# AvalonEnjoyer/pytorch-ViT-paper-replication

Hardware: AMD Instinct MI355X
Metric: images/sec (whole node) ViT-B/16 224px bf16 at 1/2/4/8 MI355X (higher is better)
Workload: dtype bf16; 1 GPU; model=ViT-B/16, global_batch=256, per_gpu_batch=256, seq_len=197, image_size=224, parallelism=dp1, impl=fused, grad_transport=none, optimizer=Adam(wd=0.03 decay group) + clip 1.0 + warmup/linear-decay LR, dropout=0.1 (mlp, embedding)

## Files before the change

### pytorch_vit_paper_replication_amd/_ext.py

```python
from __future__ import annotations

import contextlib
import os

import torch

_C = None
_ERR: BaseException | None = None
_TRIED = False


class StaleExtensionError(RuntimeError):
    """The in-tree ``_C`` was built from other ``csrc/`` sources than the ones in the tree."""


def check_source_hash(so, csrc) -> str:
    from .build import embedded_hash, source_hash

    want = source_hash(csrc)
    have = embedded_hash(so)
    if have != want:
        raise StaleExtensionError(
            f"{so} was built from other sources (binary {have}, csrc/ {want}): rebuild with "
            "`python -m pytorch_vit_paper_replication_amd.build` (or set PVR_AUTOBUILD=1)")
    return want


def load():
    global _C, _ERR, _TRIED
    if _TRIED:
        return _C
    _TRIED = True
    debug = os.environ.get("PVR_DEBUG_KERNELS", "0") == "1"
    try:
        from .build import CSRC, ext_path

        if CSRC.is_dir() and ext_path(debug).exists():
            try:
                check_source_hash(ext_path(debug), CSRC)
            except StaleExtensionError:
                if os.environ.get("PVR_AUTOBUILD", "0") != "1":
                    raise
                from .build import build_extension

                build_extension(debug=debug)
                check_source_hash(ext_path(debug), CSRC)
        if debug:
            from . import _C_debug as mod
        else:
            from . import _C as mod

        _C = mod
    except BaseException as e:
        _ERR = e
        if os.environ.get("PVR_AUTOBUILD", "0") == "1":
            try:
                from .build import build_extension

                build_extension(debug=debug)
                if debug:
                    from . import _C_debug as mod2
                else:
                    from . import _C as mod2

                _C = mod2
                _ERR = None
            except BaseException as e2:
                _ERR = e2
    return _C


def available() -> bool:
    return load() is not None


_DETERMINISTIC_ENV = os.environ.get("PVR_DETERMINISTIC", "0") not in ("", "0")


def deterministic() -> bool:
    m = _C if _TRIED else load()
    on = torch.are_deterministic_algorithms_enabled() or _DETERMINISTIC_ENV
    if m is not None and bool(m.deterministic()) != on:
        m.set_deterministic(on)
    return on


@contextlib.contextmanager
def deterministic_mode(on: bool = True):
    global _DETERMINISTIC_ENV
    old = _DETERMINISTIC_ENV
    _DETERMINISTIC_ENV = on
    try:
        deterministic()
        yield
    finally:
        _DETERMINISTIC_ENV = old
        deterministic()


def ext():
    m = load()
    if m is None:
        raise RuntimeError(
            "pytorch_vit_paper_replication_amd: the gfx950 extension _C is not built or failed to load "
            f"({_ERR!r}). Build it with `python -m pytorch_vit_paper_replication_amd.build`."
        )
    return m


def fallback_allowed() -> bool:
    return os.environ.get("PVR_ALLOW_TORCH_FALLBACK", "0") == "1"


_FORCE_REFERENCE = 0


def fused_disabled() -> bool:
    return _FORCE_REFERENCE > 0 or os.environ.get("PVR_DISABLE_FUSED", "0") == "1"


@contextlib.contextmanager
def reference_path():
    global _FORCE_REFERENCE
    _FORCE_REFERENCE += 1
    try:
        yield
    finally:
        _FORCE_REFERENCE -= 1


def use_fused(t: torch.Tensor) -> bool:
    if not t.is_cuda:
        return False
    if fused_disabled():
        return False
    if available():
        return True
    if fallback_allowed():
        return False
    ext()
    return False


def free_scratch() -> None:
    m = _C if _TRIED else load()
    if m is None:
        return
    if torch.cuda.is_available():
        torch.cuda.synchronize()
    m.free_scratch()
    from .ops import gemm as _gemm

    _gemm._workspaces.clear()
```

### pytorch_vit_paper_replication_amd/csrc/bindings.cpp

```cpp
#include <cstdlib>
#include <algorithm>
#include <map>
#include <torch/extension.h>
#include <c10/hip/HIPStream.h>
#include <hip/hip_runtime.h>

#include "kernels.h"

namespace {

hipStream_t stream() { return c10::hip::getCurrentHIPStream().stream(); }
using ScratchKey = std::pair<int, int64_t>;
ScratchKey scratch_key(int dev) { return std::make_pair(dev, (int64_t)c10::hip::getCurrentHIPStream().id()); }
template <class T>
std::map<ScratchKey, T>& scratch_map() {
  static auto* m = new std::map<ScratchKey, T>();
  return *m;
}
struct SkCounters { torch::Tensor t; };
struct DetWs { torch::Tensor t; };
struct DqWs { torch::Tensor t; };
struct AttnWs { torch::Tensor t; };

int num_cus() {
  static std::map<int, int> cache;
  int dev = 0;
  if (hipGetDevice(&dev) != hipSuccess) return 256;
  auto it = cache.find(dev);
  if (it != cache.end()) return it->second;
  hipDeviceProp_t prop;
  int n = hipGetDeviceProperties(&prop, dev) == hipSuccess && prop.multiProcessorCount > 0 ? prop.multiProcessorCount : 256;
  cache[dev] = n;
  return n;
}

void check(hipError_t e, const char* what) {
  TORCH_CHECK(e == hipSuccess, "pvr kernel '", what, "' failed: ", hipGetErrorString(e));
}

const uint16_t* bf(const torch::Tensor& t, const char* name) {
  TORCH_CHECK(t.is_cuda(), name, " must be a GPU tensor");
  TORCH_CHECK(t.scalar_type() == torch::kBFloat16, name, " must be bfloat16, got ", t.scalar_type());
  return reinterpret_cast<const uint16_t*>(t.data_ptr());
}
uint16_t* bf_mut(torch::Tensor& t, const char* name) { return const_cast<uint16_t*>(bf(t, name)); }
const float* f32(const torch::Tensor& t, const char* name) {
  TORCH_CHECK(t.is_cuda(), name, " must be a GPU tensor");
  TORCH_CHECK(t.scalar_type() == torch::kFloat32, name, " must be float32, got ", t.scalar_type());
  return t.data_ptr<float>();
}
float* f32_mut(torch::Tensor& t, const char* name) { return const_cast<float*>(f32(t, name)); }

template <class T>
T* opt_ptr(const c10::optional<torch::Tensor>& t) {
  return t.has_value() && t->defined() ? reinterpret_cast<T*>(t->data_ptr()) : nullptr;
}

int64_t ld_of(const torch::Tensor& t, const char* name) {
  TORCH_CHECK(t.dim() == 2, name, " must be 2-D");
  TORCH_CHECK(t.stride(1) == 1, name, " must have unit stride in its last dim");
  TORCH_CHECK(t.stride(0) % 8 == 0 || t.size(0) == 1, name, " leading dimension must be a multiple of 8 elements");
  TORCH_CHECK(reinterpret_cast<uintptr_t>(t.data_ptr()) % 16 == 0, name, " must be 16-byte aligned");
  return t.size(0) == 1 ? t.size(1) : t.stride(0);
}

pvr::DropSite drop_args(const c10::optional<torch::Tensor>& seed, int64_t seed_offset, double drop_p, const char* what) {
  pvr::DropSite d;
  d.offset = (uint64_t)seed_offset;
  if (drop_p > 0.0) {
    TORCH_CHECK(seed.has_value() && seed->defined() && seed->is_cuda() && seed->scalar_type() == torch::kInt64 && seed->numel() >= 1,
                what, ": dropout needs an int64 seed tensor on the GPU");
    d.seed = reinterpret_cast<const uint64_t*>(seed->data_ptr());
    d.thr = (uint32_t)llround(drop_p * 65536.0);
    if (d.thr > 65535) d.thr = 65535;
    d.scale = (float)(65536.0 / (65536.0 - d.thr));
  }
  return d;
}
pvr::DropSite drop_path_args(const c10::optional<torch::Tensor>& seed, int64_t seed_offset, double dp_p, int64_t dp_rows,
                             const char* what) {
  TORCH_CHECK(dp_p >= 0.0 && dp_p <= 1.0, what, ": drop_path rate must be in [0, 1]");
  if (dp_p > 0.0) TORCH_CHECK(dp_rows >= 1 && dp_rows < (int64_t(1) << 31), what, ": drop_path needs rows per sample >= 1");
  return drop_args(seed, seed_offset, dp_p, what);
}
void set_drop(pvr::GemmParams& p, const pvr::DropSite& d) {
  if (!d.seed) return;
  p.seed_ptr = d.seed; p.seed_offset = d.offset; p.drop_thr = d.thr; p.drop_scale = d.scale;
}

pvr::Fp8Copy fp8_copy(const c10::optional<torch::Tensor>& q_out, const c10::optional<torch::Tensor>& q_scale,
                      const c10::optional<torch::Tensor>& q_amax, int64_t q_fmt, int64_t rows, int64_t cols, int64_t align,
                      const char* what) {
  pvr::Fp8Copy q;
  q.fmt = (int)q_fmt;
  if (!q_out.has_value() || !q_out->defined()) return q;
  TORCH_CHECK(q_out->is_cuda() && q_out->scalar_type() == torch::kUInt8 && q_out->dim() == 2 && q_out->stride(1) == 1 &&
                  q_out->size(0) >= rows && q_out->size(1) >= cols && q_out->stride(0) % align == 0 &&
                  reinterpret_cast<uintptr_t>(q_out->data_ptr()) % align == 0,
              what, ": q_out must be uint8 [>= ", rows, "][>= ", cols, "] with unit column stride, row stride and base multiples of ", align);
  TORCH_CHECK(q_scale.has_value() && q_scale->defined() && q_amax.has_value() && q_amax->defined() && q_amax->is_cuda() &&
                  q_amax->scalar_type() == torch::kInt32 && (q_fmt == 0 || q_fmt == 1),
              what, ": q_out needs q_scale (f32), q_amax (int32 on the GPU) and q_fmt 0 / 1");
  q.out = q_out->data_ptr<uint8_t>();
  q.ld = q_out->stride(0);
  q.scale = f32(*q_scale, "q_scale");
  q.amax = reinterpret_cast<unsigned*>(q_amax->data_ptr());
  return q;
}

bool g_gemm_tail = true;
struct TailBufs {
  torch::Tensor ws, cnt;
};
void attach_tail(pvr::GemmParams& p, const torch::Tensor& like) {
  if (!g_gemm_tail) return;
  auto& bufs = scratch_map<TailBufs>();
  const auto key = scratch_key((int)like.get_device());
  auto it = bufs.find(key);
  if (it == bufs.end()) {
    const int64_t cus = num_cus();
    TailBufs b;
    b.ws = torch::empty({cus * 65536}, like.options().dtype(torch::kFloat32));
    b.cnt = torch::zeros({cus}, like.options().dtype(torch::kInt32));
    it = bufs.emplace(key, b).first;
  }
  p.tail_ws = it->second.ws.data_ptr<float>();
  p.tail_cnt = reinterpret_cast<unsigned*>(it->second.cnt.data_ptr<int32_t>());
  p.tail_ws_elems = it->second.ws.numel();
  p.tail_cnt_elems = (int)it->second.cnt.numel();
}
void set_gemm_tail(bool on) { g_gemm_tail = on; }

constexpr int g_sk_tiles = 4096;
torch::Tensor& splitk_counters(const torch::Tensor& like) {
  auto& bufs = scratch_map<SkCounters>();
  const auto key = scratch_key((int)like.get_device());
  auto it = bufs.find(key);
  if (it == bufs.end()) it = bufs.emplace(key, SkCounters{torch::zeros({2 * g_sk_tiles + 4}, like.options().dtype(torch::kInt32))}).first;
  return it->second.t;
}
int64_t splitk_timeouts(torch::Tensor like, bool reset) {
  torch::Tensor& c = splitk_counters(like);
  const int64_t v = c[2 * g_sk_tiles].item<int32_t>();
  if (reset) c[2 * g_sk_tiles].zero_();
  return v;
}
constexpr int g_tail_min_kt = 12;

bool g_deterministic = [] {
  const char* e = std::getenv("PVR_DETERMINISTIC");
  return e && std::atoi(e) != 0;
}();
void set_deterministic(bool on) { g_deterministic = on; }
bool deterministic() { return g_deterministic; }
float* det_scratch(int64_t numel, const torch::TensorOptions& opts) {
  DetWs& d = scratch_map<DetWs>()[scratch_key((int)opts.device().index())];
  if (!d.t.defined() || d.t.numel() < numel) d.t = torch::empty({numel}, opts.dtype(torch::kFloat32));
  return d.t.data_ptr<float>();
}

void gemm(torch::Tensor A, bool a_kcontig, torch::Tensor B, bool b_kcontig, torch::Tensor C, int64_t M, int64_t N, int64_t K,
          int64_t epi, c10::optional<torch::Tensor> bias, c10::optional<torch::Tensor> resid, c10::optional<torch::Tensor> addend,
          int64_t addend_period, c10::optional<torch::Tensor> aux, int64_t row_group, int64_t row_stride_group,
          int64_t row_offset, c10::optional<torch::Tensor> seed, int64_t seed_offset, double drop_p, int64_t k_split,
          int64_t tile_cfg, c10::optional<torch::Tensor> dbg, c10::optional<torch::Tensor> colsum,
          int64_t epi_staged, int64_t tail_limit, c10::optional<torch::Tensor> reduce_out, bool reduce_acc,
          int64_t drop_row_mul, c10::optional<torch::Tensor> dp_seed, int64_t dp_offset, double dp_p, int64_t dp_rows) {
  pvr::GemmParams p{};
  TORCH_CHECK(drop_row_mul >= 0 && (drop_row_mul == 0 || (tile_cfg == 0 && row_group == 0)) && M * std::max<int64_t>(drop_row_mul, 1) < (int64_t(1) << 31),
              "gemm: drop_row_mul (mask of every drop_row_mul-th row of a larger tensor) needs tile 0 and no row remap");
  p.drop_row_mul = (int)drop_row_mul;
  p.epi_staged = (int)epi_staged;
  if (colsum.has_value() && colsum->defined()) p.colsum = f32_mut(*colsum, "colsum");
  if (dbg.has_value() && dbg->defined()) p.dbg = reinterpret_cast<uint64_t*>(dbg->data_ptr());
  p.drop_scale = 1.f;
  p.M = (int)M; p.N = (int)N; p.K = (int)K;
  p.A = bf(A, "A"); p.lda = ld_of(A, "A"); p.a_kcontig = a_kcontig;
  p.B = bf(B, "B"); p.ldb = ld_of(B, "B"); p.b_kcontig = b_kcontig;
  TORCH_CHECK(N % 8 == 0, "gemm: N must be a multiple of 8");
  if (a_kcontig) TORCH_CHECK(K % 64 == 0, "gemm: K must be a multiple of 64 for a k-contiguous A");
  if (b_kcontig) TORCH_CHECK(K % 64 == 0, "gemm: K must be a multiple of 64 for a k-contiguous B");
  if (a_kcontig) {
    TORCH_CHECK(A.size(0) >= M && A.size(1) >= K, "gemm: A too small");
  } else {
    TORCH_CHECK(A.size(0) >= K && A.size(1) >= M, "gemm: A too small");
  }
  if (b_kcontig) {
    TORCH_CHECK(B.size(0) >= N && B.size(1) >= K, "gemm: B too small");
  } else {
    TORCH_CHECK(B.size(0) >= K && B.size(1) >= N, "gemm: B too small");
  }
  const bool f32out = epi >= 3;
  TORCH_CHECK(C.is_cuda() && C.scalar_type() == (f32out ? torch::kFloat32 : torch::kBFloat16), "gemm: C dtype mismatch for epilogue");
  if (C.dim() == 3) {
    TORCH_CHECK(epi == 4 && tile_cfg == 14, "gemm: a 3-D C is the split-K workspace of EPI_F32_STORE / tile 14");
    TORCH_CHECK(C.stride(2) == 1 && C.size(1) >= M && C.size(2) >= N, "gemm: workspace shape");
    const int64_t ks = k_split > 0 ? ((k_split + 63) / 64) * 64 : ((K + 63) / 64) * 64;
    TORCH_CHECK(C.size(0) >= (K + ks - 1) / ks, "gemm: workspace has fewer slices than K splits");
    p.C = C.data_ptr(); p.ldc = C.stride(1); p.split_stride = C.stride(0);
  } else {
    p.C = C.data_ptr(); p.ldc = ld_of(C, "C");
  }
  if (bias.has_value() && bias->defined()) { TORCH_CHECK(bias->numel() >= N && bias->is_contiguous(), "bias"); p.bias = f32(*bias, "bias"); }
  if (resid.has_value() && resid->defined()) { p.resid = bf(*resid, "resid"); p.ld_resid = ld_of(*resid, "resid"); }
  if (addend.has_value() && addend->defined()) { p.addend = f32(*addend, "addend"); p.addend_period = (int)addend_period; TORCH_CHECK(addend_period > 0, "addend_period"); }
  if (aux.has_value() && aux->defined()) { p.aux = const_cast<uint16_t*>(bf(*aux, "aux")); p.ld_aux = ld_of(*aux, "aux"); }
  if (epi == 2) TORCH_CHECK(p.aux != nullptr, "gemm: the dGELU epilogue needs aux");
  p.row_group = (int)row_group; p.row_stride_group = (int)row_stride_group; p.row_offset = (int)row_offset;
  set_drop(p, drop_args(seed, seed_offset, drop_p, "gemm"));
  p.k_split_len = k_split > 0 ? (int)(((k_split + 63) / 64) * 64) : (int)(((K + 63) / 64) * 64);
  if (dp_p > 0.0) {
    const pvr::DropSite dp = drop_path_args(dp_seed, dp_offset, dp_p, dp_rows, "gemm: drop_path");
    TORCH_CHECK(epi == 0 && p.resid != nullptr, "gemm: drop_path needs the residual epilogue (EPI_BF16 with resid)");
    TORCH_CHECK(a_kcontig && b_kcontig && row_group == 0 && p.addend == nullptr && p.k_split_len >= K,
                "gemm: drop_path does not combine with row_group / addend / split-K / transposed operands");
    TORCH_CHECK(tile_cfg == 0 || tile_cfg == 6 || tile_cfg == 12 || tile_cfg == 13,
                "gemm: drop_path runs on tiles 0, 6, 12 and 13 (not the wave-specialised tile 15 or the split-K tile 14)");
    TORCH_CHECK(p.seed_ptr == nullptr || p.seed_ptr == dp.seed, "gemm: drop_path and dropout must share the seed tensor");
    TORCH_CHECK(M / dp_rows + 1 < (int64_t(1) << 31), "gemm: drop_path sample index");
    p.seed_ptr = dp.seed;
    p.dp_thr = dp.thr; p.dp_scale = dp.scale; p.dp_seed_offset = dp.offset; p.dp_rows = (int)dp_rows;
  }
  p.epi = (int)epi;
  p.tile_cfg = (int)tile_cfg;
  if (epi <= 2 && p.k_split_len >= K && tail_limit >= 0) {
    attach_tail(p, C);
    p.tail_max_units = (int)tail_limit;
    p.tail_min_kt = g_tail_min_kt;
  }
  if (reduce_out.has_value() && reduce_out->defined()) {
    const torch::Tensor& o = *reduce_out;
    TORCH_CHECK(C.dim() == 3 && epi == 4 && tile_cfg == 14, "gemm: reduce_out needs the split-K workspace form");
    TORCH_CHECK(o.is_cuda() && o.scalar_type() == torch::kFloat32 && o.dim() == 2 && o.stride(1) == 1 && o.size(0) >= M && o.size(1) >= N &&
                    o.stride(0) % 4 == 0 && reinterpret_cast<uintptr_t>(o.data_ptr()) % 16 == 0,
                "gemm: reduce_out must be a 16-B aligned fp32 [M, N] tensor with unit column stride");
    const int64_t splits = (K + p.k_split_len - 1) / p.k_split_len;
    const int64_t tiles = ((M + 255) / 256) * ((N + 255) / 256);
    TORCH_CHECK(N % 4 == 0 && tiles <= g_sk_tiles && tiles * splits <= num_cus(), "gemm: reduce_out: too many workgroups to be co-resident");
    TORCH_CHECK(p.split_stride * 4 * (2 * splits + 16) < (int64_t(1) << 32) && M * p.ldc * 4 < (int64_t(1) << 31),
                "gemm: reduce_out: workspace too large for 32-bit buffer offsets");
    torch::Tensor& cnt = splitk_counters(o);
    p.sk_out = o.data_ptr<float>();
    p.sk_ldo = o.stride(0);
    p.sk_acc = reduce_acc ? 1 : 0;
    p.sk_cnt = reinterpret_cast<unsigned*>(cnt.data_ptr<int32_t>());
    p.sk_cnt_tiles = g_sk_tiles;
  }
  check(pvr_gemm(&p, stream()), "gemm");
}

std::vector<torch::Tensor> layernorm_fwd(torch::Tensor x, torch::Tensor w, torch::Tensor b, double eps, int64_t rows,
                                         int64_t x_row_stride) {
  const int64_t D = w.numel();
  auto y = torch::empty({rows, D}, x.options());
  auto mean = torch::empty({rows}, x.options().dtype(torch::kFloat32));
  auto rstd = torch::empty({rows}, x.options().dtype(torch::kFloat32));
  TORCH_CHECK(x.stride(-1) == 1, "layernorm: x last dim must be contiguous");
  check(pvr_layernorm_fwd(bf(x, "x"), x_row_stride, f32(w, "w"), f32(b, "b"), bf_mut(y, "y"), D, f32_mut(mean, "mean"),
                          f32_mut(rstd, "rstd"), (int)rows, (int)D, (float)eps, stream()),
        "layernorm_fwd");
  return {y, mean, rstd};
}

std::vector<torch::Tensor> layernorm_fwd_q8(torch::Tensor x, torch::Tensor w, torch::Tensor b, double eps, int64_t rows,
                                            int64_t x_row_stride, torch::Tensor q_out, torch::Tensor q_scale, torch::Tensor q_amax,
                                            bool skip_y) {
  const int64_t D = w.numel();
  auto y = torch::empty({rows, D}, x.options());
  auto mean = torch::empty({rows}, x.options().dtype(torch::kFloat32));
  auto rstd = torch::empty({rows}, x.options().dtype(torch::kFloat32));
  TORCH_CHECK(x.stride(-1) == 1, "layernorm: x last dim must be contiguous");
  TORCH_CHECK(q_out.defined(), "layernorm_fwd_q8: q_out is required");
  const pvr::Fp8Copy q = fp8_copy(q_out, q_scale, q_amax, 0, rows, D, 8, "layernorm_fwd_q8");
  check(pvr_layernorm_fwd_q8(bf(x, "x"), x_row_stride, f32(w, "w"), f32(b, "b"), skip_y ? nullptr : bf_mut(y, "y"), D, q,
                             f32_mut(mean, "mean"), f32_mut(rstd, "rstd"), (int)rows, (int)D, (float)eps, stream()),
        "layernorm_fwd_q8");
  return {y, mean, rstd};
}

void layernorm_bwd(torch::Tensor dy, int64_t dy_stride, torch::Tensor x, int64_t x_stride, torch::Tensor mean, torch::Tensor rstd,
                   torch::Tensor w, c10::optional<torch::Tensor> dres, int64_t dres_stride, torch::Tensor dx, int64_t dx_stride,
                   c10::optional<torch::Tensor> dw, c10::optional<torch::Tensor> db, int64_t rows,
                   c10::optional<torch::Tensor> dsum, c10::optional<torch::Tensor> dz, c10::optional<torch::Tensor> seed,
                   int64_t seed_offset, double drop_p, c10::optional<torch::Tensor> q_out,
                   c10::optional<torch::Tensor> q_scale, c10::optional<torch::Tensor> q_amax, bool dz_nostore,
                   int64_t q_fmt, int64_t dres_every, c10::optional<torch::Tensor> dp_seed, int64_t dp_offset, double dp_p,
                   int64_t dp_rows) {
  const int64_t D = w.numel();
  pvr::LnBwdParams p{};
  TORCH_CHECK(dres_every >= 0, "layernorm_bwd: dres_every >= 0");
  if (dres_every > 1) {
    TORCH_CHECK(dres.has_value() && dres->defined() && dres->numel() >= ((rows + dres_every - 1) / dres_every - 1) * dres_stride + D &&
                    !(q_out.has_value() && q_out->defined()),
                "layernorm_bwd: dres_every needs a compact dres [ceil(rows / dres_every)][D] and no fp8 copy");
  }
  p.dres_every = (int)dres_every;
  p.dy = bf(dy, "dy"); p.dy_stride = dy_stride;
  p.x = bf(x, "x"); p.x_stride = x_stride;
  p.mean = f32(mean, "mean"); p.rstd = f32(rstd, "rstd"); p.w = f32(w, "w");
  p.dres = opt_ptr<const uint16_t>(dres); p.dres_stride = dres_stride;
  p.dx = bf_mut(dx, "dx"); p.dx_stride = dx_stride;
  p.dw = opt_ptr<float>(dw); p.db = opt_ptr<float>(db); p.dsum = opt_ptr<float>(dsum);
  const bool has_dz = dz.has_value() && dz->defined();
  if (has_dz) {
    TORCH_CHECK(drop_p > 0.0 || dp_p > 0.0, "layernorm_bwd: dz is the dropout / drop_path backward, it needs drop_p > 0 or a drop_path rate > 0");
    p.dz = const_cast<uint16_t*>(bf(*dz, "dz"));
    p.dz_stride = ld_of(*dz, "dz");
  }
  p.drop = drop_args(seed, seed_offset, has_dz ? drop_p : 0.0, "layernorm_bwd");
  if (dp_p > 0.0) {
    TORCH_CHECK(has_dz, "layernorm_bwd: drop_path scales the dz output, it needs dz");
    TORCH_CHECK(!(q_out.has_value() && q_out->defined()), "layernorm_bwd: drop_path does not combine with the fp8 copy (q_out)");
    p.dpath = drop_path_args(dp_seed, dp_offset, dp_p, dp_rows, "layernorm_bwd: drop_path");
    p.dp_rows = (int)dp_rows;
  }
  p.dz_nostore = dz_nostore ? 1 : 0;
  p.q = fp8_copy(q_out, q_scale, q_amax, q_fmt, rows, D, 8, "layernorm_bwd");
  p.rows = (int)rows; p.D = (int)D;
  if (g_deterministic && (p.dw || p.db || p.dsum))
    p.part = det_scratch((int64_t)pvr_layernorm_bwd_blocks((int)rows, (int)D) * 3 * D, x.options());
  check(pvr_layernorm_bwd(&p, stream()), "layernorm_bwd");
}

void splitk_reduce(torch::Tensor ws, int64_t S, torch::Tensor out, bool accumulate) {
  TORCH_CHECK(ws.dim() == 3 && ws.size(0) >= S && S >= 1, "splitk_reduce: ws must be [S, rows, cols]");
  TORCH_CHECK(out.is_contiguous() && ws.stride(2) == 1 && ws.stride(1) == ws.size(2), "splitk_reduce: layouts");
  const int64_t rows = ws.size(1), wcols = ws.size(2);
  TORCH_CHECK(out.numel() % rows == 0, "splitk_reduce: out must hold [rows, ocols]");
  const int64_t ocols = out.numel() / rows;
  TORCH_CHECK(ocols <= wcols && ocols % 4 == 0 && wcols % 4 == 0, "splitk_reduce: out columns must be a 4-aligned prefix of ws columns");
  check(pvr_splitk_reduce(f32(ws, "ws"), (int)S, ws.stride(0), f32_mut(out, "out"), out.numel(), (int)ocols, (int)wcols,
                          accumulate ? 1 : 0, stream()),
        "splitk_reduce");
}

void pad_cols_bf16(torch::Tensor src, torch::Tensor dst) {
  TORCH_CHECK(src.is_contiguous() && dst.is_contiguous() && src.dim() == 2 && dst.dim() == 2 && src.size(0) == dst.size(0) &&
                  src.size(1) <= dst.size(1) && src.size(1) % 4 == 0 && dst.size(1) % 4 == 0,
              "pad_cols_bf16: src [rows, cols], dst [rows, ld >= cols], contiguous, 4-aligned");
  check(pvr_pad_cols_bf16(bf(src, "src"), (int)src.size(0), (int)src.size(1), bf_mut(dst, "dst"), (int)dst.size(1), stream()),
        "pad_cols_bf16");
}

void splitk_epilogue(torch::Tensor ws, int64_t S, torch::Tensor out, c10::optional<torch::Tensor> bias,
                     c10::optional<torch::Tensor> resid, bool gelu) {
  TORCH_CHECK(ws.dim() == 3 && ws.size(0) >= S && S >= 1 && ws.stride(2) == 1 && ws.stride(1) == ws.size(2),
              "splitk_epilogue: ws must be [S, M, N] with contiguous rows");
  const int64_t M = ws.size(1), N = ws.size(2);
  TORCH_CHECK(out.dim() == 2 && out.size(0) == M && out.size(1) == N && N % 4 == 0, "splitk_epilogue: out shape");
  const int64_t ldc = ld_of(out, "out");
  const float* bp = nullptr;
  if (bias.has_value() && bias->defined()) {
    TORCH_CHECK(bias->numel() >= N && bias->is_contiguous(), "splitk_epilogue: bias");
    bp = f32(*bias, "bias");
  }
  const uint16_t* rp = nullptr;
  int64_t ldr = 0;
  if (resid.has_value() && resid->defined()) {
    TORCH_CHECK(resid->dim() == 2 && resid->size(0) >= M && resid->size(1) >= N, "splitk_epilogue: resid must cover [M, N]");
    rp = bf(*resid, "resid");
    ldr = ld_of(*resid, "resid");
  }
  check(pvr_splitk_epilogue(f32(ws, "ws"), (int)S, ws.stride(0), (int)M, (int)N, bp, rp, ldr, gelu ? 1 : 0, bf_mut(out, "out"), ldc,
                            stream()),
        "splitk_epilogue");
}

void cast_f32_bf16(torch::Tensor in, torch::Tensor out) {
  TORCH_CHECK(in.is_contiguous() && out.is_contiguous() && in.numel() == out.numel(), "cast: shape/contiguity");
  TORCH_CHECK(in.device() == out.device() && reinterpret_cast<uintptr_t>(in.data_ptr()) % 16 == 0 &&
                  reinterpret_cast<uintptr_t>(out.data_ptr()) % 8 == 0,
              "cast: in (16-byte aligned) and out (8-byte aligned) on one GPU");
  check(pvr_cast_f32_bf16(f32(in, "in"), bf_mut(out, "out"), in.numel(), stream()), "cast_f32_bf16");
}

void transpose_batched(torch::Tensor src, torch::Tensor dst, torch::Tensor meta, int64_t total_tiles) {
  TORCH_CHECK(meta.scalar_type() == torch::kInt64 && meta.is_cuda() && meta.dim() == 2 && meta.size(1) == 5, "meta");
  check(pvr_transpose_batched(bf(src, "src"), bf_mut(dst, "dst"), meta.data_ptr<int64_t>(), (int)meta.size(0), (int)total_tiles,
                              stream()),
        "transpose_batched");
}

void colsum(torch::Tensor dy, int64_t rows, int64_t N, c10::optional<torch::Tensor> db, c10::optional<torch::Tensor> dz,
            c10::optional<torch::Tensor> seed, int64_t seed_offset, double drop_p, c10::optional<torch::Tensor> q_out,
            c10::optional<torch::Tensor> q_scale, c10::optional<torch::Tensor> q_amax, int64_t q_fmt, int64_t row_mul,
            c10::optional<torch::Tensor> dp_seed, int64_t dp_offset, double dp_p, int64_t dp_rows) {
  TORCH_CHECK(row_mul >= 1 && rows * row_mul < (int64_t(1) << 31), "colsum: row_mul >= 1 and rows * row_mul < 2^31");
  const pvr::DropSite d = drop_args(seed, seed_offset, drop_p, "colsum");
  pvr::DropSite dp;
  if (dp_p > 0.0) {
    TORCH_CHECK(!(q_out.has_value() && q_out->defined()), "colsum: drop_path does not combine with the fp8 copy (q_out)");
    dp = drop_path_args(dp_seed, dp_offset, dp_p, dp_rows, "colsum: drop_path");
  }
  int64_t ldz = 0;
  uint16_t* dzp = nullptr;
  if (dz.has_value() && dz->defined()) { dzp = const_cast<uint16_t*>(bf(*dz, "dz")); ldz = ld_of(*dz, "dz"); }
  const pvr::Fp8Copy q = fp8_copy(q_out, q_scale, q_amax, q_fmt, rows, N, 8, "colsum");
  check(pvr_colsum(bf(dy, "dy"), ld_of(dy, "dy"), (int)rows, (int)N, opt_ptr<float>(db), dzp, ldz, d, q,
                   g_deterministic && opt_ptr<float>(db) ? det_scratch((int64_t)pvr_colsum_part_rows((int)rows) * N, dy.options()) : nullptr,
                   (int)row_mul, dp, (int)std::max<int64_t>(dp_rows, 1), stream()),
        "colsum");
}

torch::Tensor drop_path_scale(torch::Tensor seed, int64_t site_offset, double p, int64_t B) {
  TORCH_CHECK(B >= 0 && B < (int64_t(1) << 31), "drop_path_scale: B");
  auto out = torch::ones({B}, seed.options().dtype(torch::kFloat32));
  if (p <= 0.0 || B == 0) return out;
  const pvr::DropSite dp = drop_path_args(seed, site_offset, p, 1, "drop_path_scale");
  check(pvr_drop_path_scale(dp, out.data_ptr<float>(), (int)B, stream()), "drop_path_scale");
  return out;
}

const pvr::MixRow* mix_rows(const c10::optional<torch::Tensor>& mix, const c10::optional<torch::Tensor>& host, int64_t B, int64_t H,
                            int64_t W, const torch::Tensor& img, const char* what) {
  if (!mix.has_value() || !mix->defined()) {
    TORCH_CHECK(!host.has_value() || !host->defined(), what, ": mix_host without mix");
    return nullptr;
  }
  TORCH_CHECK(mix->is_cuda() && mix->device() == img.device(), what, ": mix must be on the image's device");
  TORCH_CHECK(mix->scalar_type() == torch::kInt32 && mix->dim() == 2 && mix->size(0) == B && mix->size(1) == 8 && mix->is_contiguous(),
              what, ": mix must be contiguous int32 [", B, ", 8]");
  TORCH_CHECK(reinterpret_cast<uintptr_t>(mix->data_ptr()) % 16 == 0, what, ": mix must be 16-byte aligned");
  torch::Tensor h;
  if (host.has_value() && host->defined()) {
    TORCH_CHECK(!host->is_cuda() && host->scalar_type() == torch::kInt32 && host->dim() == 2 && host->size(0) == B &&
                    host->size(1) == 8 && host->is_contiguous(),
                what, ": mix_host must be a contiguous CPU int32 [", B, ", 8] tensor");
    h = *host;
  } else {
    h = mix->cpu();
  }
  const auto* rows = reinterpret_cast<const pvr::MixRow*>(h.data_ptr());
  for (int64_t b = 0; b < B; ++b) {
    const pvr::MixRow& r = rows[b];
// ... 676 lines not shown
}

void fp8_transpose(torch::Tensor x8, torch::Tensor yt) {
  TORCH_CHECK(x8.is_cuda() && x8.scalar_type() == torch::kUInt8 && x8.dim() == 2 && x8.stride(1) == 1 && x8.stride(0) % 16 == 0 &&
                  x8.size(1) % 16 == 0 && reinterpret_cast<uintptr_t>(x8.data_ptr()) % 16 == 0,
              "fp8_transpose: x8 uint8 [rows][cols], cols and row stride multiples of 16, 16-byte aligned");
  TORCH_CHECK(yt.is_cuda() && yt.scalar_type() == torch::kUInt8 && yt.dim() == 2 && yt.size(0) == x8.size(1) &&
                  yt.size(1) >= x8.size(0) && yt.stride(1) == 1 && yt.stride(0) % 64 == 0 && yt.size(1) == yt.stride(0) &&
                  reinterpret_cast<uintptr_t>(yt.data_ptr()) % 16 == 0,
              "fp8_transpose: yT uint8 [cols][>= rows], row stride a multiple of 64");
  check(pvr_fp8_transpose(x8.data_ptr<uint8_t>(), x8.stride(0), yt.data_ptr<uint8_t>(), yt.stride(0), (int)x8.size(0), (int)x8.size(1),
                          stream()),
        "fp8_transpose");
}

void gemm_fp8_wgrad_mn(torch::Tensor dy8, torch::Tensor x8, torch::Tensor ws, int64_t N, int64_t K, int64_t T, torch::Tensor scale_a,
                       torch::Tensor scale_b, int64_t ksplit, int64_t fmt_a) {
  TORCH_CHECK((fmt_a == 0 || fmt_a == 1), "gemm_fp8_wgrad_mn: fmt_a 0 (e4m3) / 1 (e5m2)");
  TORCH_CHECK(dy8.dim() == 2 && x8.dim() == 2 && dy8.size(0) >= T && x8.size(0) >= T && dy8.size(1) >= N && x8.size(1) >= K &&
                  dy8.stride(1) == 1 && x8.stride(1) == 1,
              "gemm_fp8_wgrad_mn: dy8 [T][N], x8 [T][K] row-major");
  TORCH_CHECK(N % 16 == 0 && K % 16 == 0 && dy8.stride(0) % 16 == 0 && x8.stride(0) % 16 == 0 && ksplit % 128 == 0 &&
                  reinterpret_cast<uintptr_t>(dy8.data_ptr()) % 16 == 0 && reinterpret_cast<uintptr_t>(x8.data_ptr()) % 16 == 0,
              "gemm_fp8_wgrad_mn: 16-byte rows and bases, ksplit a multiple of 128");
  TORCH_CHECK(T * std::max(dy8.stride(0), x8.stride(0)) < (1ll << 31), "gemm_fp8_wgrad_mn: 31-bit operand offsets");
  TORCH_CHECK(ws.is_cuda() && ws.scalar_type() == torch::kFloat32 && ws.dim() == 3 && ws.stride(2) == 1 && ws.size(1) >= N &&
                  ws.size(2) >= K && ws.size(0) >= (T + ksplit - 1) / ksplit,
              "gemm_fp8_wgrad_mn: workspace [splits][N][K] f32");
  pvr::GemmParams p{};
  p.drop_scale = 1.f;
  p.M = (int)N; p.N = (int)K; p.K = (int)T;
  p.A = reinterpret_cast<const uint16_t*>(u8(dy8, "dy8")); p.lda = dy8.stride(0); p.a_kcontig = 0;
  p.B = reinterpret_cast<const uint16_t*>(u8(x8, "x8")); p.ldb = x8.stride(0); p.b_kcontig = 0;
  p.C = ws.data_ptr(); p.ldc = ws.stride(1); p.split_stride = ws.stride(0);
  p.scale_a = f32(scale_a, "scale_a"); p.scale_b = f32(scale_b, "scale_b");
  p.elem8 = 1; p.fmt_a = (int)fmt_a; p.fmt_b = 0;
  p.k_split_len = (int)ksplit;
  p.epi = 4;
  p.tile_cfg = 14;
  check(pvr_gemm(&p, stream()), "gemm_fp8_wgrad_mn");
}

void gemm_fp8_wgrad(torch::Tensor A8, torch::Tensor B8, torch::Tensor ws, int64_t N, int64_t K, int64_t Tp, torch::Tensor scale_a,
                    torch::Tensor scale_b, int64_t ksplit, int64_t fmt_a) {
  TORCH_CHECK((fmt_a == 0 || fmt_a == 1), "gemm_fp8_wgrad: fmt_a 0 (e4m3) / 1 (e5m2)");
  pvr::GemmParams p{};
  p.drop_scale = 1.f;
  p.M = (int)N; p.N = (int)K; p.K = (int)Tp;
  p.A = reinterpret_cast<const uint16_t*>(u8(A8, "A8")); p.lda = A8.stride(0); p.a_kcontig = 1;
  p.B = reinterpret_cast<const uint16_t*>(u8(B8, "B8")); p.ldb = B8.stride(0); p.b_kcontig = 1;
  TORCH_CHECK(A8.size(0) >= N && A8.size(1) >= Tp && B8.size(0) >= K && B8.size(1) >= Tp, "gemm_fp8_wgrad: operand too small");
  TORCH_CHECK(Tp % 128 == 0 && ksplit % 128 == 0 && K % 8 == 0, "gemm_fp8_wgrad: Tp, ksplit multiples of 128");
  TORCH_CHECK(ws.is_cuda() && ws.scalar_type() == torch::kFloat32 && ws.dim() == 3 && ws.stride(2) == 1 && ws.size(1) >= N &&
                  ws.size(2) >= K && ws.size(0) >= (Tp + ksplit - 1) / ksplit,
              "gemm_fp8_wgrad: workspace [splits][N][K] f32");
  p.C = ws.data_ptr(); p.ldc = ws.stride(1); p.split_stride = ws.stride(0);
  p.scale_a = f32(scale_a, "scale_a"); p.scale_b = f32(scale_b, "scale_b");
  p.elem8 = 1; p.fmt_a = (int)fmt_a; p.fmt_b = 0;
  p.k_split_len = (int)ksplit;
  p.epi = 4;
  p.tile_cfg = 14;
  check(pvr_gemm(&p, stream()), "gemm_fp8_wgrad");
}

void fp8_quant(torch::Tensor x, c10::optional<torch::Tensor> y, c10::optional<torch::Tensor> qscale, torch::Tensor amax, int64_t fmt) {
  const uint16_t* xp = bf(x, "x");
  const int64_t ldx = ld_of(x, "x");
  uint8_t* yp = nullptr;
  int64_t ldy = 0;
  if (y.has_value() && y->defined()) {
    yp = const_cast<uint8_t*>(u8(*y, "y"));
    ldy = y->stride(0);
    TORCH_CHECK(y->size(0) == x.size(0) && y->size(1) == x.size(1), "fp8_quant: shape mismatch");
  }
  TORCH_CHECK(amax.is_cuda() && amax.scalar_type() == torch::kInt32 && amax.numel() >= 1, "fp8_quant: amax int32");
  const float* qs = nullptr;
  if (qscale.has_value() && qscale->defined()) qs = f32(*qscale, "qscale");
  TORCH_CHECK(yp == nullptr || qs != nullptr, "fp8_quant: y needs qscale");
  check(pvr_fp8_quant(xp, ldx, yp, ldy, x.size(0), (int)x.size(1), qs, reinterpret_cast<unsigned*>(amax.data_ptr()), (int)fmt, stream()),
        "fp8_quant");
}

torch::Tensor fp8_dequant(torch::Tensor x, c10::optional<torch::Tensor> dscale, int64_t fmt) {
  TORCH_CHECK(x.is_cuda() && x.scalar_type() == torch::kUInt8 && x.is_contiguous(), "fp8_dequant: contiguous uint8");
  auto y = torch::empty(x.sizes(), x.options().dtype(torch::kFloat32));
  const float* ds = nullptr;
  if (dscale.has_value() && dscale->defined()) ds = f32(*dscale, "dscale");
  check(pvr_fp8_dequant(x.data_ptr<uint8_t>(), y.data_ptr<float>(), x.numel(), ds, (int)fmt, stream()), "fp8_dequant");
  return y;
}

void fp8_quant_multi(torch::Tensor segs, int64_t nchunks, c10::optional<torch::Tensor> qscale, torch::Tensor amax, int64_t fmt,
                     bool amax_only) {
  TORCH_CHECK(segs.is_cuda() && segs.scalar_type() == torch::kInt64 && segs.dim() == 2 && segs.size(1) == 5 && segs.is_contiguous(),
              "fp8_quant_multi: segs int64 [n][5]");
  TORCH_CHECK(amax.is_cuda() && amax.scalar_type() == torch::kInt32, "fp8_quant_multi: amax int32");
  const float* qs = qscale.has_value() && qscale->defined() ? f32(*qscale, "qscale") : nullptr;
  TORCH_CHECK(amax_only || qs != nullptr, "fp8_quant_multi: quantizing needs qscale");
  check(pvr_fp8_quant_multi(segs.data_ptr<int64_t>(), (int)segs.size(0), nchunks, qs, reinterpret_cast<unsigned*>(amax.data_ptr()),
                            (int)fmt, amax_only ? 1 : 0, stream()),
        "fp8_quant_multi");
}

void fp8_scale_update(torch::Tensor hist, torch::Tensor amax, torch::Tensor qscale, torch::Tensor dscale, torch::Tensor fmax, int64_t s0,
                      int64_t s1, double margin_mul) {
  TORCH_CHECK(hist.dim() == 2 && hist.is_contiguous(), "hist [n][H]");
  TORCH_CHECK(amax.scalar_type() == torch::kInt32, "amax int32");
  TORCH_CHECK(s0 >= 0 && s1 <= hist.size(0), "slot range");
  check(pvr_fp8_scale_update(f32_mut(hist, "hist"), (int)hist.size(1), reinterpret_cast<unsigned*>(amax.data_ptr()), f32_mut(qscale, "qscale"),
                             f32_mut(dscale, "dscale"), f32(fmax, "fmax"), (int)s0, (int)s1, (float)margin_mul, stream()),
        "fp8_scale_update");
}

std::vector<torch::Tensor> attn_fwd(torch::Tensor qkv, int64_t B, int64_t N, int64_t H, double scale, c10::optional<torch::Tensor> seed,
                                    int64_t seed_offset, double drop_p, c10::optional<torch::Tensor> q_out,
                                    c10::optional<torch::Tensor> q_scale, c10::optional<torch::Tensor> q_amax, bool q_only) {
  const int64_t D = qkv.size(1) / 3;
  auto out = torch::empty({B * N, D}, qkv.options());
  auto lse = torch::empty({B * H, N}, qkv.options().dtype(torch::kFloat32));
  TORCH_CHECK(!q_only || (q_out.has_value() && q_out->defined()), "attn_fwd: q_only needs q_out");
  TORCH_CHECK(qkv.size(0) == B * N, "attn_fwd: qkv rows != B*N");
  const pvr::DropSite d = drop_args(seed, seed_offset, drop_p, "attn_fwd");
  const pvr::Fp8Copy q8 = fp8_copy(q_out, q_scale, q_amax, 0, B * N, D, 4, "attn_fwd");
  check(pvr_attn_fwd(bf(qkv, "qkv"), ld_of(qkv, "qkv"), bf_mut(out, "out"), D, f32_mut(lse, "lse"), (int)B, (int)N, (int)H, (int)D,
                     (float)scale, d, q8, q_only ? 1 : 0, stream()),
        "attn_fwd");
  return {out, lse};
}

void attn_dbias_reduce(torch::Tensor part, int64_t B, int64_t H, torch::Tensor dbias) {
  TORCH_CHECK(dbias.is_cuda() && dbias.scalar_type() == torch::kFloat32 && dbias.is_contiguous() && dbias.numel() % (3 * H) == 0,
              "attn_dbias_reduce: f32 [3D] bias gradient");
  const int64_t DH = dbias.numel() / (3 * H);
  TORCH_CHECK(part.is_cuda() && part.scalar_type() == torch::kFloat32 && part.is_contiguous() && part.numel() % (B * H * 3 * DH) == 0,
              "attn_dbias_reduce: f32 [B*H][R][3 * head dim] partials");
  const int64_t NQ = part.numel() / (B * H * 3 * DH);
  auto ws = torch::empty({(int64_t)pvr_attn_dbias_splits((int)B, (int)NQ) * H * 2 * DH}, part.options());
  check(pvr_attn_dbias_reduce(part.data_ptr<float>(), ws.data_ptr<float>(), dbias.data_ptr<float>(), (int)B, (int)H, (int)NQ,
                              (int)(DH * H), stream()),
        "attn_dbias_reduce");
}

torch::Tensor dq_workspace(int64_t numel, const torch::TensorOptions& opts, bool drop = false) {
  DqWs& d = scratch_map<DqWs>()[scratch_key((int)opts.device().index())];
  if (drop) {
    d.t = torch::Tensor();
    return torch::Tensor();
  }
  if (!d.t.defined() || d.t.numel() < numel) d.t = torch::zeros({numel}, opts.dtype(torch::kFloat32));
  return d.t;
}

torch::Tensor attn_scratch(int64_t numel, const torch::TensorOptions& opts) {
  AttnWs& d = scratch_map<AttnWs>()[scratch_key((int)opts.device().index())];
  if (!d.t.defined() || d.t.numel() < numel) d.t = torch::empty({numel}, opts.dtype(torch::kFloat32));
  return d.t;
}

void free_scratch() {
  scratch_map<TailBufs>().clear();
  scratch_map<SkCounters>().clear();
  scratch_map<DetWs>().clear();
  scratch_map<DqWs>().clear();
  scratch_map<AttnWs>().clear();
}

int64_t attn_bwd_bias_rows(int64_t B, int64_t N, int64_t H, int64_t D, bool drop) {
  return pvr_attn_bwd_part_rows((int)B, (int)N, (int)H, (int)D, 3 * D, D, D, 3 * D, drop ? 1 : 0);
}

bool attn_bwd_q8_ok(int64_t B, int64_t N, int64_t H, int64_t D, bool drop) {
  return pvr_attn_bwd_q8_ok((int)N, drop ? 1 : 0) && !pvr_attn_bwd_uses_pipe((int)B, (int)N, (int)H, (int)D, 3 * D, D, D, 3 * D, drop ? 1 : 0);
}

torch::Tensor attn_bwd(torch::Tensor dout, torch::Tensor qkv, torch::Tensor out, torch::Tensor lse, int64_t B, int64_t N, int64_t H,
                       double scale, c10::optional<torch::Tensor> dbias, c10::optional<torch::Tensor> dbias_part_out,
                       c10::optional<torch::Tensor> seed, int64_t seed_offset, double drop_p, c10::optional<torch::Tensor> q_out,
                       c10::optional<torch::Tensor> q_scale, c10::optional<torch::Tensor> q_amax, bool q_only,
                       int64_t q_fmt) {
  const int64_t D = qkv.size(1) / 3;
  auto dqkv = torch::empty_like(qkv);
  torch::Tensor dq_acc;
  int dq_rezero = 0;
  const pvr::DropSite drop = drop_args(seed, seed_offset, drop_p, "attn_bwd");
  const int has_drop = drop.seed ? 1 : 0;
  const int64_t dh = D / H;
  torch::Tensor dbias_part, old_part;
  const bool want_db = dbias.has_value() && dbias->defined();
  const int64_t lds[4] = {ld_of(qkv, "qkv"), ld_of(dout, "dout"), ld_of(out, "out"), ld_of(dqkv, "dqkv")};
  const int prow = pvr_attn_bwd_part_rows((int)B, (int)N, (int)H, (int)D, lds[0], lds[1], lds[2], lds[3], has_drop);
  const bool parts = prow > 0;
  const bool pipe = pvr_attn_bwd_uses_pipe((int)B, (int)N, (int)H, (int)D, lds[0], lds[1], lds[2], lds[3], has_drop) != 0;
  const bool part_out = dbias_part_out.has_value() && dbias_part_out->defined();
  if (part_out) {
    TORCH_CHECK(parts && !want_db, "dbias_part: shapes with attn_bwd_bias_rows > 0 only, and not together with dbias");
    TORCH_CHECK(dbias_part_out->is_cuda() && dbias_part_out->scalar_type() == torch::kFloat32 && dbias_part_out->is_contiguous() &&
                    dbias_part_out->numel() == B * H * prow * 3 * dh,
                "dbias_part [B*H][attn_bwd_bias_rows][3 * head dim] f32");
    dbias_part = *dbias_part_out;
  }
  if (want_db) {
    TORCH_CHECK(dbias->numel() == 3 * D && dbias->scalar_type() == torch::kFloat32 && dbias->is_contiguous(), "dbias [3D] f32");
    if (parts)
      dbias_part = torch::empty({B * H, (int64_t)prow, 3 * dh}, qkv.options().dtype(torch::kFloat32));
    else if (2 * (dh / 16) <= 2 * pvr_attn_bwd_waves((int)N))
      old_part = torch::empty({B * pvr_attn_bwd_key_blocks((int)N), 3 * D}, qkv.options().dtype(torch::kFloat32));
  }
  const int old_db = old_part.defined() ? 1 : 0;
  if (pvr_attn_bwd_needs_dq_acc((int)N, (int)dh, old_db, has_drop, g_deterministic ? 1 : 0)) {
    dq_acc = dq_workspace(B * N * D, qkv.options());
    dq_rezero = dq_acc.defined() ? 1 : 0;
    if (!dq_acc.defined()) dq_acc = torch::zeros({B * N, D}, qkv.options().dtype(torch::kFloat32));
  }
  const pvr::Fp8Copy q8 = fp8_copy(q_out, q_scale, q_amax, q_fmt, B * N, 3 * D, 4, "attn_bwd");
  if (q8.out)
    TORCH_CHECK(pvr_attn_bwd_q8_ok((int)N, has_drop) && !old_db && !pipe, "attn_bwd: no e5m2 dQKV copy for this shape (see attn_bwd_q8_ok)");
  auto ws = attn_scratch(pvr_attn_bwd_ws_floats((int)B, (int)N, (int)H, (int)D, old_db, has_drop, g_deterministic ? 1 : 0), qkv.options());
  pvr::AttnBwdParams p{};
  p.qkv = bf(qkv, "qkv"); p.ld = lds[0];
  p.out = bf(out, "out"); p.ld_o = lds[2];
  p.dout = bf(dout, "dout"); p.ld_do = lds[1];
  p.dqkv = bf_mut(dqkv, "dqkv"); p.ld_dq = lds[3];
  p.lse = f32(lse, "lse"); p.ws = ws.data_ptr<float>();
  p.dq_acc = dq_acc.defined() ? dq_acc.data_ptr<float>() : nullptr; p.dq_rezero = dq_rezero;
  p.dbias = pipe && dbias_part.defined() ? dbias_part.data_ptr<float>() : old_db ? old_part.data_ptr<float>() : nullptr;
  p.bpart = !pipe && dbias_part.defined() ? dbias_part.data_ptr<float>() : nullptr;
  p.B = (int)B; p.N = (int)N; p.H = (int)H; p.D = (int)D; p.scale = (float)scale;
  p.drop = drop; p.q8 = q8; p.q8_only = q_only && q8.out ? 1 : 0;
  const hipError_t err = pvr_attn_bwd(&p, stream());
  if (err != hipSuccess && dq_rezero) dq_workspace(0, qkv.options(), true);
  check(err, "attn_bwd");
  if (want_db) {
    if (parts)
      attn_dbias_reduce(dbias_part, B, H, *dbias);
    else if (old_db)
      dbias->add_(old_part.sum(0));
    else
      dbias->add_(dqkv.sum(0, false, torch::kFloat32));
  }
  return dqkv;
}

std::vector<torch::Tensor> attn_cls_fwd(torch::Tensor qkv, int64_t B, int64_t N, int64_t H, double scale) {
  TORCH_CHECK(qkv.dim() == 2 && qkv.size(0) == B * N && qkv.size(1) % 3 == 0 && H > 0, "attn_cls_fwd: qkv [B*N][3D]");
  const int64_t D = qkv.size(1) / 3;
  TORCH_CHECK(D % H == 0 && pvr_attn_cls_ok((int)N, (int)(D / H)), "attn_cls_fwd: unsupported N / head dim (attn_cls_ok)");
  auto out = torch::empty({B, D}, qkv.options());
  auto lse = torch::empty({B * H}, qkv.options().dtype(torch::kFloat32));
  check(pvr_attn_cls_fwd(bf(qkv, "qkv"), ld_of(qkv, "qkv"), bf_mut(out, "out"), D, f32_mut(lse, "lse"), (int)B, (int)N, (int)H, (int)D,
                         (float)scale, stream()),
        "attn_cls_fwd");
  return {out, lse};
}

std::vector<torch::Tensor> attn_cls_bwd(torch::Tensor dout, torch::Tensor qkv, torch::Tensor out, torch::Tensor lse, int64_t B, int64_t N,
                                        int64_t H, double scale) {
  TORCH_CHECK(qkv.dim() == 2 && qkv.size(0) == B * N && qkv.size(1) % 3 == 0 && H > 0, "attn_cls_bwd: qkv [B*N][3D]");
  const int64_t D = qkv.size(1) / 3;
  TORCH_CHECK(D % H == 0 && pvr_attn_cls_ok((int)N, (int)(D / H)), "attn_cls_bwd: unsupported N / head dim (attn_cls_ok)");
  TORCH_CHECK(dout.dim() == 2 && dout.size(0) == B && dout.size(1) == D && out.dim() == 2 && out.size(0) == B && out.size(1) == D &&
                  lse.numel() == B * H && lse.is_contiguous(),
              "attn_cls_bwd: dout / out [B][D], lse [B*H]");
  auto dqkv = torch::empty({B * N, 3 * D}, qkv.options());
  auto dq0 = torch::empty({B, D}, qkv.options().dtype(torch::kFloat32));
  check(pvr_attn_cls_bwd(bf(qkv, "qkv"), ld_of(qkv, "qkv"), bf(out, "out"), ld_of(out, "out"), bf(dout, "dout"), ld_of(dout, "dout"),
                         f32(lse, "lse"), bf_mut(dqkv, "dqkv"), 3 * D, f32_mut(dq0, "dq0"), (int)B, (int)N, (int)H, (int)D, (float)scale,
                         stream()),
        "attn_cls_bwd");
  return {dqkv, dq0};
}

void attn_cls_dbias(torch::Tensor dq0, torch::Tensor dout, torch::Tensor dbias) {
  TORCH_CHECK(dq0.dim() == 2 && dq0.is_contiguous() && dout.dim() == 2 && dout.size(0) == dq0.size(0) && dout.size(1) == dq0.size(1) &&
                  dbias.is_contiguous() && dbias.numel() == 3 * dq0.size(1),
              "attn_cls_dbias: dq0 f32 [B][D] contiguous, dout bf16 [B][D], dbias f32 [3D]");
  check(pvr_attn_cls_dbias(f32(dq0, "dq0"), bf(dout, "dout"), ld_of(dout, "dout"), f32_mut(dbias, "dbias"), (int)dq0.size(0),
                           (int)dq0.size(1), stream()),
        "attn_cls_dbias");
}

}

extern "C" const char* pvr_src_hash(void);

PYBIND11_MODULE(TORCH_EXTENSION_NAME, m) {
  m.doc() = "MI355X (gfx950) HIP kernels for pytorch_vit_paper_replication_amd";
  m.def("source_hash", []() { return std::string(pvr_src_hash()); },
        "content hash of the csrc/ sources this binary was built from (build.source_hash())");
  m.def("gemm_tail_split", [](int64_t M, int64_t N, int64_t K, int64_t elem_bytes, int64_t max_units) {
    return pvr_gemm_tail_split((int)M, (int)N, (int)K, (int)elem_bytes, (int)max_units); },
    py::arg("M"), py::arg("N"), py::arg("K"), py::arg("elem_bytes"), py::arg("max_units") = 0,
    "K-parts of the split tail round this GEMM shape gets (0: none)");
  m.def("set_attn_dbg", [](torch::Tensor t) { pvr_set_attn_dbg(t.defined() && t.numel() ? t.data_ptr() : nullptr); },
        "diagnostic builds (-DPVR_ATTN_STAMPS): int64 buffer for the attention backward's phase stamps "
        "[workgroup * waves + wave][8] (scripts/attn_stamps.py); a no-op otherwise");
  m.def("set_attn_prep_xcd", &pvr_set_attn_prep_xcd, "attention backward pre-pass: XCD-contiguous (batch, head) pairs (1) or round-robin (0, default); A/B");
  m.def("set_ln_fwd_q8_grid", &pvr_set_ln_fwd_q8_grid, "LayerNorm forward with the e4m3 copy: grid cap in workgroups per CU (A/B)");
  m.def("set_attn_fwd_head_qf", &pvr_set_attn_fwd_head_qf, "whole-head attention forward (dh 64, N <= 256): 16-query fragments per wave (1 = default, 2 = half the LDS reads with 7 waves; A/B)");
  m.def("set_attn_fwd_qg", &pvr_set_attn_fwd_qg, "tiled attention forward: 16-query groups per wave (0 = auto by query padding, 1 = round-3 form, 2 = forced; A/B)");
  m.def("set_fp8_persistent", &pvr_set_fp8_persistent, "fp8 fwd/dgrad GEMMs on the persistent ping-pong: 1 when the epilogue has no per-row input (default), 0 never (A/B)");
  m.def("set_deterministic", &set_deterministic, "deterministic reductions (partial rows + ordered sum) instead of float atomics");
  m.def("deterministic", &deterministic);
  m.def("set_gemm_tail", &set_gemm_tail, "split-K tail of the last dispatch round on (True, default) / off (A/B)");
  m.def("gemm", &gemm,py::arg("A"), py::arg("a_kcontig"), py::arg("B"), py::arg("b_kcontig"), py::arg("C"),
        py::arg("M"), py::arg("N"), py::arg("K"), py::arg("epi"), py::arg("bias"), py::arg("resid"), py::arg("addend"),
        py::arg("addend_period"), py::arg("aux"), py::arg("row_group"), py::arg("row_stride_group"),
        py::arg("row_offset"), py::arg("seed"), py::arg("seed_offset"), py::arg("drop_p"), py::arg("k_split"),
        py::arg("tile_cfg"), py::arg("dbg") = py::none(), py::arg("colsum") = py::none(),
        py::arg("epi_staged") = 0, py::arg("tail_limit") = 0, py::arg("reduce_out") = py::none(), py::arg("reduce_acc") = true,
        py::arg("drop_row_mul") = 0, py::arg("dp_seed") = py::none(), py::arg("dp_offset") = 0, py::arg("dp_p") = 0.0,
        py::arg("dp_rows") = 1);
  m.def("drop_path_scale", &drop_path_scale, py::arg("seed"), py::arg("site_offset"), py::arg("p"), py::arg("B"));
  m.def("splitk_timeouts", &splitk_timeouts, py::arg("like"), py::arg("reset") = false);
  m.def("num_cus", &num_cus);
  m.def("layernorm_fwd", &layernorm_fwd);
  m.def("free_scratch", &free_scratch);
  m.def("layernorm_fwd_q8", &layernorm_fwd_q8);
  m.def("layernorm_bwd", &layernorm_bwd, py::arg("dy"), py::arg("dy_stride"), py::arg("x"), py::arg("x_stride"),
        py::arg("mean"), py::arg("rstd"), py::arg("w"), py::arg("dres"), py::arg("dres_stride"), py::arg("dx"),
        py::arg("dx_stride"), py::arg("dw"), py::arg("db"), py::arg("rows"), py::arg("dsum") = py::none(),
        py::arg("dz") = py::none(), py::arg("seed") = py::none(), py::arg("seed_offset") = 0, py::arg("drop_p") = 0.0,
        py::arg("q_out") = py::none(), py::arg("q_scale") = py::none(), py::arg("q_amax") = py::none(),
        py::arg("dz_nostore") = false, py::arg("q_fmt") = 1, py::arg("dres_every") = 0, py::arg("dp_seed") = py::none(),
        py::arg("dp_offset") = 0, py::arg("dp_p") = 0.0, py::arg("dp_rows") = 1);
  m.def("cast_f32_bf16", &cast_f32_bf16);
  m.def("splitk_epilogue", &splitk_epilogue);
  m.def("attn_bwd_bias_rows", &attn_bwd_bias_rows, py::arg("B"), py::arg("N"), py::arg("H"), py::arg("D"), py::arg("drop") = false);
  m.def("attn_dbias_reduce", &attn_dbias_reduce);
  m.def("splitk_reduce", &splitk_reduce);
  m.def("pad_cols_bf16", &pad_cols_bf16);
  m.def("transpose_batched", &transpose_batched);
  m.def("colsum", &colsum, py::arg("dy"), py::arg("rows"), py::arg("N"), py::arg("db"), py::arg("dz"), py::arg("seed"),
        py::arg("seed_offset"), py::arg("drop_p"), py::arg("q_out") = py::none(), py::arg("q_scale") = py::none(),
        py::arg("q_amax") = py::none(), py::arg("q_fmt") = 1, py::arg("row_mul") = 1, py::arg("dp_seed") = py::none(),
        py::arg("dp_offset") = 0, py::arg("dp_p") = 0.0, py::arg("dp_rows") = 1);
  m.def("im2col", &im2col, py::arg("img"), py::arg("out"), py::arg("P"), py::arg("Kp"), py::arg("mix") = py::none(),
        py::arg("mix_host") = py::none(), py::arg("keep") = py::none(), py::arg("erase") = py::none(),
        py::arg("erase_host") = py::none(), py::arg("erase_mode") = "const", py::arg("erase_value") = std::vector<double>{0.0},
        py::arg("erase_seed") = py::none(), py::arg("erase_offset") = 0);
  m.def("im2col_u8", &im2col_u8, py::arg("img"), py::arg("out"), py::arg("mean"), py::arg("std"), py::arg("geom"), py::arg("H"),
        py::arg("W"), py::arg("P"), py::arg("Kp"), py::arg("mix") = py::none(), py::arg("mix_host") = py::none(),
        py::arg("keep") = py::none(), py::arg("erase") = py::none(), py::arg("erase_host") = py::none(),
        py::arg("erase_mode") = "const", py::arg("erase_value") = std::vector<double>{0.0}, py::arg("erase_seed") = py::none(),
        py::arg("erase_offset") = 0);
  m.def("color_u8", &color_u8, py::arg("img"), py::arg("plan"), py::arg("plan_host") = py::none());
  m.def("erase_noise", &erase_noise, py::arg("seed"), py::arg("site_offset"), py::arg("B"), py::arg("C"), py::arg("H"), py::arg("W"));
  m.def("patch_keep_table", &patch_keep_table, py::arg("seed"), py::arg("site_offset"), py::arg("B"), py::arg("n_p"), py::arg("n_keep"));
  m.def("pos_gather", &pos_gather, py::arg("pos"), py::arg("keep"));
  m.def("cls_rows", &cls_rows);
  m.def("patch_bwd", &patch_bwd, py::arg("dE"), py::arg("B"), py::arg("ntok"), py::arg("D"), py::arg("dpos"), py::arg("dcls"),
        py::arg("dconv"), py::arg("dbias"), py::arg("seed"), py::arg("seed_offset"), py::arg("drop_p"), py::arg("inv") = py::none(),
        py::arg("n_keep") = 0);
  m.def("xent", &xent, py::arg("logits"), py::arg("labels"), py::arg("dlogits"), py::arg("correct"), py::arg("grad_scale"),
        py::arg("mean") = py::none());
  m.def("xent_soft", &xent_soft, py::arg("logits"), py::arg("ya"), py::arg("yb"), py::arg("lam"), py::arg("eps"),
        py::arg("dlogits"), py::arg("correct"), py::arg("grad_scale"), py::arg("mean") = py::none());
  m.def("grad_norm", &grad_norm);
  m.def("norm_partial_blocks", []() { return pvr_norm_partial_blocks(); });
  m.def("adam", &adam, py::arg("p"), py::arg("g"), py::arg("m"), py::arg("v"), py::arg("shadow"), py::arg("seg_start"),
        py::arg("seg_group"), py::arg("groups"), py::arg("clip"), py::arg("skip_nonfinite"), py::arg("ema") = py::none(),
        py::arg("ema_pair") = py::none());
  m.def("adam_t", &adam_t, py::arg("p"), py::arg("g"), py::arg("m"), py::arg("v"), py::arg("shadow"), py::arg("shadow_t"),
        py::arg("tmeta"), py::arg("ntiles"), py::arg("fmeta"), py::arg("flat4"), py::arg("groups"), py::arg("clip"),
        py::arg("skip_nonfinite"), py::arg("ema") = py::none(), py::arg("ema_pair") = py::none());
  m.def("lamb_chunk", []() { return (int)pvr::LAMB_CHUNK; });
  m.def("lamb_moments", &lamb_moments, py::arg("p"), py::arg("g"), py::arg("m"), py::arg("v"), py::arg("chunks"), py::arg("seg_group"),
        py::arg("partial"), py::arg("groups"), py::arg("clip"), py::arg("skip_nonfinite"));
  m.def("lamb_ratio", &lamb_ratio, py::arg("partial"), py::arg("seg_chunks"), py::arg("seg_group"), py::arg("trust"), py::arg("groups"),
        py::arg("clip"), py::arg("skip_nonfinite"));
  m.def("lamb_update", &lamb_update, py::arg("p"), py::arg("m"), py::arg("v"), py::arg("shadow"), py::arg("trust"), py::arg("groups"),
        py::arg("clip"), py::arg("skip_nonfinite"), py::arg("seg_start") = py::none(), py::arg("seg_group") = py::none(),
        py::arg("shadow_t") = py::none(), py::arg("tmeta") = py::none(), py::arg("ntiles") = 0, py::arg("fmeta") = py::none(),
        py::arg("flat4") = 0, py::arg("ema") = py::none(), py::arg("ema_pair") = py::none());
  m.def("scale_by_clip", &scale_by_clip);
  m.def("head_fwd", &head_fwd);
  m.def("head_bwd", &head_bwd, py::arg("dlogits"), py::arg("xhat"), py::arg("rstd"), py::arg("gamma"), py::arg("beta"), py::arg("W"),
        py::arg("B"), py::arg("N"), py::arg("dW") = py::none(), py::arg("db") = py::none(), py::arg("dgamma") = py::none(),
        py::arg("dbeta") = py::none());
  m.def("scale_by", &scale_by);
  m.def("metrics_accum", &metrics_accum);
  m.def("rng_next", &rng_next);
  m.def("zero_f32", &zero_f32);
  m.def("gemm_fp8", &gemm_fp8, py::arg("A"), py::arg("fmt_a"), py::arg("B"), py::arg("fmt_b"), py::arg("C"), py::arg("M"),
        py::arg("N"), py::arg("K"), py::arg("epi"), py::arg("scale_a"), py::arg("scale_b"), py::arg("bias") = py::none(),
        py::arg("resid") = py::none(), py::arg("aux") = py::none(), py::arg("seed") = py::none(), py::arg("seed_offset") = 0,
        py::arg("drop_p") = 0.0, py::arg("colsum") = py::none(), py::arg("q_out") = py::none(), py::arg("q_scale") = py::none(),
        py::arg("q_amax") = py::none(), py::arg("q_fmt") = 0, py::arg("c_skip") = false, py::arg("tail_limit") = 0);
  m.def("fp8_transpose", &fp8_transpose);
  m.def("gemm_fp8_wgrad_mn", &gemm_fp8_wgrad_mn, py::arg("dy8"), py::arg("x8"), py::arg("ws"), py::arg("N"), py::arg("K"),
        py::arg("T"), py::arg("scale_a"), py::arg("scale_b"), py::arg("ksplit"), py::arg("fmt_a") = 1);
  m.def("fp8_quant", &fp8_quant, py::arg("x"), py::arg("y"), py::arg("qscale"), py::arg("amax"), py::arg("fmt"));
  m.def("fp8_dequant", &fp8_dequant, py::arg("x"), py::arg("dscale") = py::none(), py::arg("fmt") = 0);
  m.def("fp8_scale_update", &fp8_scale_update);
  m.def("fp8_quant_t", &fp8_quant_t);
  m.def("gemm_fp8_wgrad", &gemm_fp8_wgrad, py::arg("A8"), py::arg("B8"), py::arg("ws"), py::arg("N"), py::arg("K"), py::arg("Tp"),
        py::arg("scale_a"), py::arg("scale_b"), py::arg("ksplit"), py::arg("fmt_a") = 1);
  m.def("fp8_quant_multi", &fp8_quant_multi, py::arg("segs"), py::arg("nchunks"), py::arg("qscale"), py::arg("amax"), py::arg("fmt"),
        py::arg("amax_only"));
  m.def("attn_fwd", &attn_fwd, py::arg("qkv"), py::arg("B"), py::arg("N"), py::arg("H"), py::arg("scale"),
        py::arg("seed") = py::none(), py::arg("seed_offset") = 0, py::arg("drop_p") = 0.0, py::arg("q_out") = py::none(),
        py::arg("q_scale") = py::none(), py::arg("q_amax") = py::none(), py::arg("q_only") = false);
  m.def("attn_bwd", &attn_bwd, py::arg("dout"), py::arg("qkv"), py::arg("out"), py::arg("lse"), py::arg("B"), py::arg("N"),
        py::arg("H"), py::arg("scale"), py::arg("dbias") = py::none(), py::arg("dbias_part") = py::none(),
        py::arg("seed") = py::none(), py::arg("seed_offset") = 0, py::arg("drop_p") = 0.0, py::arg("q_out") = py::none(),
        py::arg("q_scale") = py::none(), py::arg("q_amax") = py::none(), py::arg("q_only") = false,
        py::arg("q_fmt") = 1);
  m.def("attn_cls_ok", [](int64_t N, int64_t dh) { return pvr_attn_cls_ok((int)N, (int)dh) != 0; },
        "the class-token attention kernels take this token count and head dim");
  m.def("attn_cls_fwd", &attn_cls_fwd, py::arg("qkv"), py::arg("B"), py::arg("N"), py::arg("H"), py::arg("scale"));
  m.def("attn_cls_bwd", &attn_cls_bwd, py::arg("dout"), py::arg("qkv"), py::arg("out"), py::arg("lse"), py::arg("B"), py::arg("N"),
        py::arg("H"), py::arg("scale"));
  m.def("attn_cls_dbias", &attn_cls_dbias);
  m.def("attn_bwd_q8_ok", &attn_bwd_q8_ok, "attn_bwd can write dQKV's e5m2 copy for this shape");
  m.def("arch", []() { return std::string("gfx950"); });
}
```

### pytorch_vit_paper_replication_amd/csrc/gemm.hip

```cpp
#include "common.h"
#include "kernels.h"
#include <type_traits>

namespace pvr {

enum GemmEpi : int {
  EPI_BF16 = 0,
  EPI_GELU = 1,
  EPI_DGELU = 2,
  EPI_F32_ATOMIC = 3,
  EPI_F32_STORE = 4,
  EPI_BF16_DP = 5,
};
constexpr bool epi_bf16(int e) { return e == EPI_BF16 || e == EPI_BF16_DP; }

struct DpRowScale {
  uint32_t key, b0, r0;
  int row0;
  float fkeep;
  PVR_DEV void init(const GemmParams& p, int first_row) {
    key = rng_key(*p.seed_ptr + p.dp_seed_offset);
    fkeep = p.drop_scale * p.dp_scale;
    row0 = __builtin_amdgcn_readfirstlane(first_row);
    b0 = (uint32_t)row0 / (uint32_t)p.dp_rows;
    r0 = (uint32_t)row0 - b0 * (uint32_t)p.dp_rows;
  }
  PVR_DEV float factor(const GemmParams& p, int row) const {
    const uint32_t d = (uint32_t)p.dp_rows;
    uint32_t b;
    if (d >= 128u) {
      const uint32_t r = r0 + (uint32_t)(row - row0);
      b = b0 + (r >= d ? 1u : 0u) + (r >= 2u * d ? 1u : 0u);
    } else {
      b = (uint32_t)row / d;
    }
    return rng_keep_32(key, b, p.dp_thr) ? fkeep : 0.f;
  }
};



namespace {

PVR_DEV void stamp(const GemmParams& p, int slot) {
#ifdef PVR_GEMM_PHASE_STAMPS
  return;
#endif
  if (p.dbg && threadIdx.x == 0) {
    const int b = blockIdx.x + gridDim.x * blockIdx.z;
    p.dbg[(int64_t)b * 8 + slot] = __builtin_amdgcn_s_memtime();
  }
}

constexpr int TK = 64;

#ifndef PVR_PP_PRE
#define PVR_PP_PRE 1
#endif

PVR_DEV int swz_k(int row) { return (row >> 1) & 7; }
PVR_DEV int swz_mn(int row) { return ((row & 3) | (((row >> 3) & 1) << 2)) << 1; }
PVR_DEV int swz8(int row) { return ((row >> 1) & 3) | (((row >> 5) & 1) << 2); }

template <int R, bool KC, int NW>
PVR_DEV void stage_tile(__amdgpu_buffer_rsrc_t rs, char* lds, int64_t ld, int k0, int wave, int lane) {
  if constexpr (KC) {
    constexpr int NI = R / 8;
#pragma unroll
    for (int i = 0; i < NI / NW; ++i) {
      const int s = wave + NW * i;
      const int row = s * 8 + (lane >> 3);
      const int c = (lane & 7) ^ swz_k(row);
      const uint32_t voff = (uint32_t)(row * ld * 2 + (int64_t)(k0 + c * 8) * 2);
      dma16(rs, to_lds(lds + s * 1024), voff);
    }
  } else {
    constexpr int CPR = R / 8, RPI = 64 / CPR, NI = TK / RPI;
#pragma unroll
    for (int i = 0; i < NI / NW; ++i) {
      const int s = wave + NW * i;
      const int row = s * RPI + lane / CPR;
      const int pc = lane % CPR;
      const int c = (pc & ~15) | ((pc & 15) ^ swz_mn(row));
      const uint32_t voff = (uint32_t)((int64_t)(k0 + row) * ld * 2 + c * 16);
      dma16(rs, to_lds(lds + s * 1024), voff);
    }
  }
}

template <int R, bool KC>
PVR_DEV v8s read_frag(const char* lds, int r0, int ks, int lane) {
  if constexpr (KC) {
    const int row = r0 + (lane & 15);
    const int c = ks * 4 + (lane >> 4);
    return ds_read_b128(lds + row * 128 + ((c ^ swz_k(row)) << 4));
  } else {
    const int g = lane >> 4, q = (lane >> 2) & 3, p = lane & 3;
    const int c = (r0 >> 3) + (p >> 1);
    const int kr0 = ks * 32 + 8 * g + q;
    const int kr1 = kr0 + 4;
    const int pc0 = (c & ~15) | ((c & 15) ^ swz_mn(kr0));
    const int pc1 = (c & ~15) | ((c & 15) ^ swz_mn(kr1));
    v4s lo = ds_read_tr(lds + kr0 * (R * 2) + pc0 * 16 + 8 * (p & 1));
    v4s hi = ds_read_tr(lds + kr1 * (R * 2) + pc1 * 16 + 8 * (p & 1));
    return cat44(lo, hi);
  }
}

template <int R>
PVR_DEV void read_frag_mn_async(const char* lds, int r0, int ks, int lane, v4s& lo, v4s& hi) {
  const int g = lane >> 4, q = (lane >> 2) & 3, p = lane & 3;
  const int c = (r0 >> 3) + (p >> 1);
  const int kr0 = ks * 32 + 8 * g + q;
  const int kr1 = kr0 + 4;
  const int pc0 = (c & ~15) | ((c & 15) ^ swz_mn(kr0));
  const int pc1 = (c & ~15) | ((c & 15) ^ swz_mn(kr1));
  lo = ds_read_tr_async(lds + kr0 * (R * 2) + pc0 * 16 + 8 * (p & 1));
  hi = ds_read_tr_async(lds + kr1 * (R * 2) + pc1 * 16 + 8 * (p & 1));
}

PVR_DEV uint32_t rsrc_bytes(int64_t extent_elems, int64_t base_elems) {
  int64_t b = (extent_elems - base_elems) * 2;
  if (b < 0) b = 0;
  if (b > 0xFFFFFFFFll) b = 0xFFFFFFFFll;
  return (uint32_t)b;
}

template <int FN, int EPI>
struct RowIn {
  uint2 r[FN];
  float4 a[FN];
};

template <int FN, int EPI>
PVR_DEV void load_row(const GemmParams& p, int m, int64_t orow, int nb, int g, RowIn<FN, EPI>& in) {
  if (m >= p.M) return;
#pragma unroll
  for (int j = 0; j < FN; ++j) {
    const int n = nb + 16 * j + 4 * g;
    if (n >= p.N) continue;
    if constexpr (epi_bf16(EPI)) {
      if (p.resid) in.r[j] = *(const uint2*)(p.resid + (int64_t)m * p.ld_resid + n);
      if (p.addend) in.a[j] = *(const float4*)(p.addend + (orow % p.addend_period) * p.N + n);
    } else if constexpr (EPI == EPI_DGELU) {
      in.r[j] = *(const uint2*)(p.aux + (int64_t)m * p.ld_aux + n);
    }
  }
}

PVR_DEV int64_t out_row(const GemmParams& p, int m) {
  return p.row_group ? (int64_t)(m / p.row_group) * p.row_stride_group + p.row_offset + m % p.row_group : (int64_t)m;
}

template <int FM, int FN, bool SWAP, int EPI>
PVR_DEV void epilogue(const GemmParams& p, v4f (&acc)[FM][FN], int mb, int nb, int lane) {
  const int g = lane >> 4, li = lane & 15;
  if constexpr (SWAP) {
    const uint64_t seed = (p.drop_thr ? *p.seed_ptr : 0ull) + p.seed_offset;
    const float deq = p.scale_a ? (*p.scale_a) * (*p.scale_b) : 1.f;
    DpRowScale dps{};
    if constexpr (EPI == EPI_BF16_DP) dps.init(p, mb);
    float4 bias[FN];
#pragma unroll
    for (int j = 0; j < FN; ++j) {
      bias[j] = make_float4(0.f, 0.f, 0.f, 0.f);
      if constexpr (epi_bf16(EPI) || EPI == EPI_GELU) {
        const int n = nb + 16 * j + 4 * g;
        if (p.bias && n < p.N) bias[j] = *(const float4*)(p.bias + n);
      }
    }
    float csum[FN][4];
#pragma unroll
    for (int j = 0; j < FN; ++j) csum[j][0] = csum[j][1] = csum[j][2] = csum[j][3] = 0.f;
    RowIn<FN, EPI> cur, nxt;
    load_row<FN, EPI>(p, mb + li, out_row(p, mb + li), nb, g, cur);
#pragma unroll
    for (int i = 0; i < FM; ++i) {
      const int m = mb + 16 * i + li;
      const int64_t orow = out_row(p, m);
      if (i + 1 < FM) load_row<FN, EPI>(p, m + 16, out_row(p, m + 16), nb, g, nxt);
      if (m < p.M) {
        float rf = 1.f;
        if constexpr (EPI == EPI_BF16_DP) rf = dps.factor(p, m);
#pragma unroll
        for (int j = 0; j < FN; ++j) {
          const int n = nb + 16 * j + 4 * g;
          if (n >= p.N) continue;
          float v[4] = {acc[i][j][0] * deq, acc[i][j][1] * deq, acc[i][j][2] * deq, acc[i][j][3] * deq};
          bool keep[4] = {true, true, true, true};
          if constexpr (epi_bf16(EPI) || EPI == EPI_GELU) {
            if (p.drop_thr) {
              const uint64_t idx = (uint64_t)(p.drop_row_mul ? (int64_t)m * p.drop_row_mul : orow) * p.N + n;
              rng_keep2(seed, idx, p.drop_thr, keep[0], keep[1]);
              rng_keep2(seed, idx + 2, p.drop_thr, keep[2], keep[3]);
            }
          }
          if constexpr (epi_bf16(EPI) || EPI == EPI_GELU) {
            v[0] += bias[j].x; v[1] += bias[j].y; v[2] += bias[j].z; v[3] += bias[j].w;
          }
          if constexpr (epi_bf16(EPI)) {
            if (p.addend) {
              v[0] += cur.a[j].x; v[1] += cur.a[j].y; v[2] += cur.a[j].z; v[3] += cur.a[j].w;
            }
            if constexpr (EPI == EPI_BF16_DP) {
              const bool rk = rf != 0.f;
              const float zero = rk ? 0.f : -0.f;
#pragma unroll
              for (int r = 0; r < 4; ++r) v[r] = keep[r] && rk ? v[r] * rf : zero;
            } else if (p.drop_thr) {
#pragma unroll
              for (int r = 0; r < 4; ++r) v[r] = keep[r] ? v[r] * p.drop_scale : 0.f;
            }
            if (p.resid) {
              const uint2 rr = cur.r[j];
              v[0] += bf2f(rr.x & 0xFFFF); v[1] += bf2f(rr.x >> 16);
              v[2] += bf2f(rr.y & 0xFFFF); v[3] += bf2f(rr.y >> 16);
            }
            uint2 o; o.x = pack2bf(v[0], v[1]); o.y = pack2bf(v[2], v[3]);
            *(uint2*)((uint16_t*)p.C + orow * p.ldc + n) = o;
          } else if constexpr (EPI == EPI_GELU) {
            float gp[4];
#pragma unroll
            for (int r = 0; r < 4; ++r) {
              float gv, gd;
              gelu_and_grad(v[r], gv, gd);
              const float sc = keep[r] ? p.drop_scale : 0.f;
              v[r] = gv * sc;
              gp[r] = gd * sc;
            }
            if (p.aux) {
              uint2 a; a.x = pack2bf(gp[0], gp[1]); a.y = pack2bf(gp[2], gp[3]);
              *(uint2*)(p.aux + (int64_t)m * p.ld_aux + n) = a;
            }
            uint2 o; o.x = pack2bf(v[0], v[1]); o.y = pack2bf(v[2], v[3]);
            *(uint2*)((uint16_t*)p.C + orow * p.ldc + n) = o;
          } else if constexpr (EPI == EPI_DGELU) {
            const uint2 gg = cur.r[j];
            v[0] *= bf2f(gg.x & 0xFFFF); v[1] *= bf2f(gg.x >> 16);
            v[2] *= bf2f(gg.y & 0xFFFF); v[3] *= bf2f(gg.y >> 16);
            csum[j][0] += v[0]; csum[j][1] += v[1]; csum[j][2] += v[2]; csum[j][3] += v[3];
            uint2 o; o.x = pack2bf(v[0], v[1]); o.y = pack2bf(v[2], v[3]);
            *(uint2*)((uint16_t*)p.C + orow * p.ldc + n) = o;
          } else if constexpr (EPI == EPI_F32_STORE) {
            *(float4*)((float*)p.C + orow * p.ldc + n) = make_float4(v[0], v[1], v[2], v[3]);
          } else {
#pragma unroll
            for (int r = 0; r < 4; ++r) atomicAdd((float*)p.C + orow * p.ldc + n + r, v[r]);
          }
        }
      }
      cur = nxt;
    }
    if constexpr (EPI == EPI_DGELU) {
      if (p.colsum) {
#pragma unroll
        for (int j = 0; j < FN; ++j)
#pragma unroll
          for (int r = 0; r < 4; ++r) {
            float c = csum[j][r];
            c += __shfl_xor(c, 1, 64);
            c += __shfl_xor(c, 2, 64);
            c += __shfl_xor(c, 4, 64);
            c += __shfl_xor(c, 8, 64);
            csum[j][r] = c;
          }
        if (li == 0) {
#pragma unroll
          for (int j = 0; j < FN; ++j) {
            const int n = nb + 16 * j + 4 * g;
            if (n < p.N)
#pragma unroll
              for (int r = 0; r < 4; ++r) atomicAdd(p.colsum + n + r, csum[j][r]);
          }
        }
      }
    }
  } else {
#pragma unroll
    for (int i = 0; i < FM; ++i)
#pragma unroll
      for (int j = 0; j < FN; ++j) {
        const int n = nb + 16 * j + li;
        if (n >= p.N) continue;
#pragma unroll
        for (int r = 0; r < 4; ++r) {
          const int m = mb + 16 * i + 4 * g + r;
          if (m >= p.M) continue;
          float* dst = (float*)p.C + (int64_t)m * p.ldc + n;
          if constexpr (EPI == EPI_F32_ATOMIC)
            atomicAdd(dst, acc[i][j][r]);
          else
            *dst = acc[i][j][r];
        }
      }
  }
}

template <int BM, int BN, int WM, int WN, bool AK, bool BKC, bool SWAP, int EPI>
__global__ void __launch_bounds__(WM* WN * 64) gemm_kernel(GemmParams p) {
  constexpr int NW = WM * WN;
  constexpr int A_BYTES = BM * TK * 2, B_BYTES = BN * TK * 2, STAGE = A_BYTES + B_BYTES;
  constexpr int WTM = BM / WM, WTN = BN / WN, FM = WTM / 16, FN = WTN / 16;
  extern __shared__ __attribute__((aligned(16))) char smem[];

// ... 286 lines not shown
    char* dst = smem + s * STAGE_BYTES;
    stage32<BM, AK, NW>(pick_rsrc(s < nk, ars, nul), dst, p.lda, s * BK32, wave, lane);
    stage32<BN, BKC, NW>(pick_rsrc(s < nk, brs, nul), dst + A_BYTES, p.ldb, s * BK32, wave, lane);
  }
  wait_barrier<INFL>();
  v8s a0[FM], b0[FN], a1[FM], b1[FN];
  load_frags<FM, FN, BM, BN, AK, BKC>(smem, wm, wn, lane, a0, b0);
  wait_barrier_lds<INFL>();
  stamp(p, 1);

  int kt = 0;
  for (; kt + 1 < nk; kt += 2) {
    v3_stage<BM, BN, WM, WN, AK, BKC, SWAP>(acc, a0, b0, a1, b1, smem + ((kt + 1) % STAGES) * STAGE_BYTES,
                                    smem + (kt % STAGES) * STAGE_BYTES, pick_rsrc(kt + STAGES < nk, ars, nul),
                                    pick_rsrc(kt + STAGES < nk, brs, nul), p.lda, p.ldb, (kt + STAGES) * BK32, wave, lane,
                                    wm, wn);
    wait_barrier_lds<INFL>();
    v3_stage<BM, BN, WM, WN, AK, BKC, SWAP>(acc, a1, b1, a0, b0, smem + ((kt + 2) % STAGES) * STAGE_BYTES,
                                    smem + ((kt + 1) % STAGES) * STAGE_BYTES, pick_rsrc(kt + 1 + STAGES < nk, ars, nul),
                                    pick_rsrc(kt + 1 + STAGES < nk, brs, nul), p.lda, p.ldb, (kt + 1 + STAGES) * BK32, wave,
                                    lane, wm, wn);
    wait_barrier_lds<INFL>();
  }
  if (kt < nk) mfma_block<FM, FN, SWAP>(acc, a0, b0);
  asm volatile("s_waitcnt vmcnt(0)" ::: "memory");
  stamp(p, 2);
  epilogue<FM, FN, SWAP, EPI>(p, acc, m0 + wm * (16 * FM), n0 + wn * (16 * FN), lane);
  if (p.dbg) asm volatile("s_waitcnt vmcnt(0)" ::: "memory");
  stamp(p, 3);
}

template <int BM, int BN, int WM, int WN, int STAGES, int WPE, bool AK, bool BKC, bool SWAP, int EPI>
hipError_t launch_v3(const GemmParams& p, hipStream_t s) {
  constexpr int SMEM = STAGES * (BM + BN) * BK32 * 2;
  auto kern = gemm_v3_kernel<BM, BN, WM, WN, STAGES, WPE, AK, BKC, SWAP, EPI>;
  static bool attr_set = false;
  if (!attr_set) {
    hipError_t e = hipFuncSetAttribute((const void*)kern, hipFuncAttributeMaxDynamicSharedMemorySize, SMEM);
    if (e != hipSuccess) return e;
    attr_set = true;
  }
  const int ntm = (p.M + BM - 1) / BM, ntn = (p.N + BN - 1) / BN;
  const int nsplit = (p.K + p.k_split_len - 1) / p.k_split_len;
  hipLaunchKernelGGL(kern, dim3(ntm * ntn, 1, nsplit), dim3(WM * WN * 64), SMEM, s, p);
  return hipGetLastError();
}

constexpr int PP_BK = 64;
constexpr int PP_BUF = 2 * 256 * 128;

template <int W, bool AK, bool BKC, int ES>
PVR_DEV void pp_issue(__amdgpu_buffer_rsrc_t ars, __amdgpu_buffer_rsrc_t brs, __amdgpu_buffer_rsrc_t nul, char* smem,
                      int64_t lda, int64_t ldb, int t, int nk, int wave, int lane) {
  static_assert(ES == 2 || ES == 1, "bf16 or fp8 operands");
  char* buf = smem + (t & 1) * PP_BUF;
  const int k0 = t * PP_BK;
  const int kb = t * 128;
  const bool live = t < nk;
#pragma unroll
  for (int x = 0; x < 2; ++x) {
    const int d = wave + 8 * x;
    if constexpr (W == 0 || W == 3) {
      constexpr int hh = W == 3;
      if constexpr (AK) {
        const int rowb = (2 * (d >> 3) + hh) * 64 + (d & 7) * 8;
        const int row = rowb + (lane >> 3);
        const int c = (lane & 7) ^ swz_k(row);
        dma16(live ? ars : nul, to_lds(buf + rowb * 128), (uint32_t)(row * lda * ES + kb + c * 16));
      } else if constexpr (ES == 1) {
        const int kr = 8 * d + (lane >> 3), cl = (lane & 7) ^ swz8(kr);
        const int m = (cl >> 2) * 128 + hh * 64 + (cl & 3) * 16;
        dma16(live ? ars : nul, to_lds(buf + hh * 16384 + d * 1024), (uint32_t)((int64_t)(t * 128 + kr) * lda + m));
      } else {
        const int kr = 4 * d + (lane >> 4);
        const int cl = (lane & 15) ^ swz_mn(kr);
        const int m = (cl >> 3) * 128 + hh * 64 + (cl & 7) * 8;
        dma16(live ? ars : nul, to_lds(buf + hh * 16384 + d * 1024), (uint32_t)(((int64_t)(k0 + kr) * lda + m) * 2));
      }
    } else {
      constexpr int hh = W == 2;
      if constexpr (BKC) {
        const int rowb = (2 * (d >> 2) + hh) * 32 + (d & 3) * 8;
        const int row = rowb + (lane >> 3);
        const int c = (lane & 7) ^ swz_k(row);
        dma16(live ? brs : nul, to_lds(buf + 256 * 128 + rowb * 128), (uint32_t)(row * ldb * ES + kb + c * 16));
      } else if constexpr (ES == 1) {
        const int kr = 8 * d + (lane >> 3), cl = (lane & 7) ^ swz8(kr);
        const int n = (cl >> 1) * 64 + hh * 32 + (cl & 1) * 16;
        dma16(live ? brs : nul, to_lds(buf + 256 * 128 + hh * 16384 + d * 1024), (uint32_t)((int64_t)(t * 128 + kr) * ldb + n));
      } else {
        const int kr = 4 * d + (lane >> 4);
        const int cl = (lane & 15) ^ swz_mn(kr);
        const int n = (cl >> 2) * 64 + hh * 32 + (cl & 3) * 8;
        dma16(live ? brs : nul, to_lds(buf + 256 * 128 + hh * 16384 + d * 1024), (uint32_t)(((int64_t)(k0 + kr) * ldb + n) * 2));
      }
    }
  }
}

PVR_DEV void pp_barrier() {
  asm volatile("" ::: "memory");
  __builtin_amdgcn_s_barrier();
  asm volatile("" ::: "memory");
}

PVR_DEV v8s frag_fp8(const char* img, int r0, int h, int lane) {
  const int row = r0 + (lane & 15);
  const int c = (lane >> 4) + 4 * h;
  return ds_read_b128(img + row * 128 + ((c ^ swz_k(row)) << 4));
}

typedef uint32_t v2u8 __attribute__((ext_vector_type(2)));
PVR_DEV void read_frag_mn8_async(const char* img, int c0, int lane, v2u8 (&r)[4]) {
  const int g = lane >> 4, i = lane & 15;
  const int row = 32 * g + (i >> 1);
  const uint32_t a = (uint32_t)(uintptr_t)(const __attribute__((address_space(3))) char*)(
      img + row * 128 + ((((c0 >> 4) ^ swz8(row)) << 4) | 8 * (i & 1)));
  asm volatile("ds_read_b64_tr_b8 %0, %1" : "=v"(r[0]) : "v"(a));
  asm volatile("ds_read_b64_tr_b8 %0, %1 offset:1024" : "=v"(r[1]) : "v"(a));
  asm volatile("ds_read_b64_tr_b8 %0, %1 offset:2048" : "=v"(r[2]) : "v"(a));
  asm volatile("ds_read_b64_tr_b8 %0, %1 offset:3072" : "=v"(r[3]) : "v"(a));
}
PVR_DEV v8s cat8_fp8(v2u8 lo, v2u8 hi) {
  typedef uint32_t v4u_ __attribute__((ext_vector_type(4)));
  return __builtin_bit_cast(v8s, (v4u_){lo.x, lo.y, hi.x, hi.y});
}

template <int FA, int FB>
PVR_DEV v4f mfma_fp8(const v8s& a0, const v8s& a1, const v8s& b0, const v8s& b1, v4f c) {
  typedef int v8i __attribute__((ext_vector_type(8)));
  typedef int v4i __attribute__((ext_vector_type(4)));
  const v4i x0 = __builtin_bit_cast(v4i, a0), x1 = __builtin_bit_cast(v4i, a1);
  const v4i y0 = __builtin_bit_cast(v4i, b0), y1 = __builtin_bit_cast(v4i, b1);
  const v8i a = {x0[0], x0[1], x0[2], x0[3], x1[0], x1[1], x1[2], x1[3]};
  const v8i b = {y0[0], y0[1], y0[2], y0[3], y1[0], y1[1], y1[2], y1[3]};
  return __builtin_amdgcn_mfma_scale_f32_16x16x128_f8f6f4(a, b, c, FA, FB, 0, 127, 0, 127);
}

struct PpStamps {
#ifdef PVR_GEMM_PHASE_STAMPS
  uint64_t acc[8] = {0, 0, 0, 0, 0, 0, 0, 0};
  uint64_t last = 0;
  uint64_t t0 = 0;
#endif
  PVR_DEV void at(int k, int pt) {
#if defined(PVR_GEMM_PHASE_STAMPS) && !defined(PVR_GEMM_PHASE_BY_TYPE)
    const uint64_t t = __builtin_amdgcn_s_memtime();
#ifdef PVR_GEMM_PHASE_ONLY_TYPE
    if (pt == PVR_GEMM_PHASE_ONLY_TYPE) acc[k] += t - last;
#else
    (void)pt;
    acc[k] += t - last;
#endif
    last = t;
#else
    (void)k;
    (void)pt;
#endif
  }
  PVR_DEV void type_mark(int pt, int what) {
#if defined(PVR_GEMM_PHASE_STAMPS) && defined(PVR_GEMM_PHASE_BY_TYPE)
    const uint64_t t = __builtin_amdgcn_s_memtime();
    if (what == 0) t0 = t;
    else if (what == 1) acc[4 + pt] += t - t0;
    else acc[pt] += t - t0;
#else
    (void)pt;
    (void)what;
#endif
  }
  PVR_DEV void begin() {
#ifdef PVR_GEMM_PHASE_STAMPS
    last = __builtin_amdgcn_s_memtime();
#endif
  }
};

template <int QM, int QN, int RD_A, int RD_B, int KIND, bool AK, bool BKC, bool SWAP, int ES = 2, int FA = 0, int FB = 0, int PR = 0>
PVR_DEV void pp_phase(v4f (&acc)[8][4], v8s (&af)[4][2], v8s (&bf)[2][2][2], v8s (&pre)[4], const char* buf, const char* nbuf,
                      __amdgpu_buffer_rsrc_t ars, __amdgpu_buffer_rsrc_t brs, __amdgpu_buffer_rsrc_t nul, char* smem, int64_t lda,
                      int64_t ldb, int t_issue, int nk, int wave, int lane, int wm, int wn, PpStamps& pst) {
  static_assert(PR == 0 || (AK && ES == 2), "A0 read-ahead: bf16 k-contiguous A only");
  constexpr int PT_ = QM == 0 ? QN : 3 - QN;
  pst.type_mark(PT_, 0);

  v4s alo[4][2], ahi[4][2], blo[2][2], bhi[2][2];
  constexpr bool MN8A = ES == 1 && !AK, MN8B = ES == 1 && !BKC;
  v2u8 a8r[MN8A ? 4 : 1][4], b8r[MN8B ? 2 : 1][4];
  if constexpr (RD_A && MN8A) {
#pragma unroll
    for (int ii = 0; ii < 4; ++ii) read_frag_mn8_async(buf + QM * 16384, wm * 64 + 16 * ii, lane, a8r[ii]);
  } else if constexpr (RD_A) {
#pragma unroll
    for (int ii = 0; ii < 4; ++ii)
#pragma unroll
      for (int ks = 0; ks < 2; ++ks) {
        if constexpr (ES == 1)
          af[ii][ks] = frag_fp8(buf, wm * 128 + QM * 64 + 16 * ii, ks, lane);
        else if constexpr (AK && PR == 1)
          af[ii][ks] = ks == 0 ? pre[ii] : read_frag<256, true>(buf, wm * 128 + QM * 64 + 16 * ii, ks, lane);
        else if constexpr (AK)
          af[ii][ks] = read_frag<256, true>(buf, wm * 128 + QM * 64 + 16 * ii, ks, lane);
        else
          read_frag_mn_async<128>(buf + QM * 16384, wm * 64 + 16 * ii, ks, lane, alo[ii][ks], ahi[ii][ks]);
      }
  }
  if constexpr (PR == 2) {
#pragma unroll
    for (int ii = 0; ii < 4; ++ii) pre[ii] = read_frag<256, true>(nbuf, wm * 128 + 16 * ii, 0, lane);
  }
  if constexpr (RD_B && MN8B) {
#pragma unroll
    for (int jj = 0; jj < 2; ++jj) read_frag_mn8_async(buf + 256 * 128 + QN * 16384, wn * 32 + 16 * jj, lane, b8r[jj]);
  } else if constexpr (RD_B) {
#pragma unroll
    for (int jj = 0; jj < 2; ++jj)
#pragma unroll
      for (int ks = 0; ks < 2; ++ks) {
        if constexpr (ES == 1)
          bf[QN][jj][ks] = frag_fp8(buf + 256 * 128, wn * 64 + QN * 32 + 16 * jj, ks, lane);
        else if constexpr (BKC)
          bf[QN][jj][ks] = read_frag<256, true>(buf + 256 * 128, wn * 64 + QN * 32 + 16 * jj, ks, lane);
        else
          read_frag_mn_async<128>(buf + 256 * 128 + QN * 16384, wn * 32 + 16 * jj, ks, lane, blo[jj][ks], bhi[jj][ks]);
      }
  }
  pst.at(0, PT_);
  pp_issue<KIND, AK, BKC, ES>(ars, brs, nul, smem, lda, ldb, t_issue, nk, wave, lane);
  pst.at(1, PT_);
  asm volatile("s_waitcnt vmcnt(8)" ::: "memory");
  pst.type_mark(PT_, 1);
  pst.at(2, PT_);
  pp_barrier();
  pst.at(3, PT_);
  if constexpr (AK && BKC)
    asm volatile("s_waitcnt lgkmcnt(0)" ::: "memory");
  else
    lds_wait();
  if constexpr (RD_A && MN8A) {
#pragma unroll
    for (int ii = 0; ii < 4; ++ii) {
      af[ii][0] = cat8_fp8(a8r[ii][0], a8r[ii][1]);
      af[ii][1] = cat8_fp8(a8r[ii][2], a8r[ii][3]);
    }
  }
  if constexpr (RD_B && MN8B) {
#pragma unroll
    for (int jj = 0; jj < 2; ++jj) {
      bf[QN][jj][0] = cat8_fp8(b8r[jj][0], b8r[jj][1]);
      bf[QN][jj][1] = cat8_fp8(b8r[jj][2], b8r[jj][3]);
    }
  }
  if constexpr (RD_A && !AK && ES == 2) {
#pragma unroll
    for (int ii = 0; ii < 4; ++ii)
#pragma unroll
      for (int ks = 0; ks < 2; ++ks) af[ii][ks] = cat44(alo[ii][ks], ahi[ii][ks]);
  }
  if constexpr (RD_B && !BKC && ES == 2) {
#pragma unroll
    for (int jj = 0; jj < 2; ++jj)
#pragma unroll
      for (int ks = 0; ks < 2; ++ks) bf[QN][jj][ks] = cat44(blo[jj][ks], bhi[jj][ks]);
  }
  pst.at(4, PT_);
  __builtin_amdgcn_s_setprio(1);
  if constexpr (ES == 1) {
#pragma unroll
    for (int ii = 0; ii < 4; ++ii)
#pragma unroll
      for (int jj = 0; jj < 2; ++jj) {
        v4f& c = acc[QM * 4 + ii][QN * 2 + jj];
        if constexpr (SWAP)
          c = mfma_fp8<FB, FA>(bf[QN][jj][0], bf[QN][jj][1], af[ii][0], af[ii][1], c);
        else
          c = mfma_fp8<FA, FB>(af[ii][0], af[ii][1], bf[QN][jj][0], bf[QN][jj][1], c);
      }
    __builtin_amdgcn_s_setprio(0);
    pst.at(5, PT_);
    pp_barrier();
    pst.at(6, PT_);
    pst.type_mark(PT_, 2);
    return;
  }
#pragma unroll
  for (int ks = 0; ks < 2; ++ks)
#pragma unroll
    for (int ii = 0; ii < 4; ++ii)
#pragma unroll
      for (int jj = 0; jj < 2; ++jj) {
        v4f& c = acc[QM * 4 + ii][QN * 2 + jj];
        if constexpr (SWAP)
          c = mfma16(bf[QN][jj][ks], af[ii][ks], c);
        else
          c = mfma16(af[ii][ks], bf[QN][jj][ks], c);
      }
  __builtin_amdgcn_s_setprio(0);
  pst.at(5, PT_);
  pp_barrier();
  pst.at(6, PT_);
  pst.type_mark(PT_, 2);
}

__host__ __device__ inline bool direct_ok(const GemmParams& p) {
  const int64_t l1 = p.ldc > p.ld_resid ? p.ldc : p.ld_resid;
  const int64_t ld = l1 > p.ld_aux ? l1 : p.ld_aux;
  return !p.addend && !p.row_group && (p.N & 7) == 0 && (int64_t)p.M * ld * 2 < (1ll << 31);
}

template <int EPI, bool RES, bool SCALED = false>
PVR_DEV void epilogue_direct(const GemmParams& p, v4f (&acc)[8][4], char* smem, int mb, int nb, int wm, int wn, int lane) {
  typedef uint32_t v4u __attribute__((ext_vector_type(4)));
  typedef uint32_t v2u_q __attribute__((ext_vector_type(2)));
  const int li = lane & 15, g = lane >> 4;
  const float deq = SCALED ? (*p.scale_a) * (*p.scale_b) : 1.f;
  const int rows = max(0, min(128, p.M - mb));
  const uint32_t OOB = 0x80000000u;
  const __amdgpu_buffer_rsrc_t crs =
      make_rsrc((const uint16_t*)p.C + (int64_t)mb * p.ldc, rows && !p.c_skip ? (uint32_t)(((int64_t)(rows - 1) * p.ldc + p.N) * 2) : 0);
  __amdgpu_buffer_rsrc_t xrs = crs;
  int64_t ldx = p.ldc;
  if constexpr (epi_bf16(EPI) && RES) {
    xrs = make_rsrc(p.resid + (int64_t)mb * p.ld_resid, rows ? (uint32_t)(((int64_t)(rows - 1) * p.ld_resid + p.N) * 2) : 0);
    ldx = p.ld_resid;
  } else if constexpr (EPI == EPI_GELU || EPI == EPI_DGELU) {
    const bool has = p.aux != nullptr;
    xrs = make_rsrc(has ? p.aux + (int64_t)mb * p.ld_aux : p.aux, has && rows ? (uint32_t)(((int64_t)(rows - 1) * p.ld_aux + p.N) * 2) : 0);
    ldx = p.ld_aux;
  }
  const __amdgpu_buffer_rsrc_t brs = make_rsrc(p.bias, p.bias ? (uint32_t)p.N * 4 : 0);
  int c0[2];
  uint32_t vc[2], vx[2];
  float bias[2][8];
#pragma unroll
  for (int jp = 0; jp < 2; ++jp) {
    c0[jp] = nb + 32 * jp + ((g & 1) << 4) + ((g & 2) << 2);
    const bool okc = c0[jp] < p.N;
    vc[jp] = okc ? (uint32_t)((li * p.ldc + c0[jp]) * 2) : OOB;
    vx[jp] = okc ? (uint32_t)((li * ldx + c0[jp]) * 2) : OOB;
#pragma unroll
    for (int e = 0; e < 8; ++e) bias[jp][e] = 0.f;
    if constexpr (epi_bf16(EPI) || EPI == EPI_GELU) {
      const uint32_t vb = okc ? (uint32_t)(c0[jp] * 4) : OOB;
      const v4f b0 = __builtin_bit_cast(v4f, __builtin_amdgcn_raw_buffer_load_b128(brs, vb, 0, 0));
      const v4f b1 = __builtin_bit_cast(v4f, __builtin_amdgcn_raw_buffer_load_b128(brs, vb + 16, 0, 0));
#pragma unroll
      for (int e = 0; e < 4; ++e) { bias[jp][e] = b0[e]; bias[jp][4 + e] = b1[e]; }
    }
  }
  const uint64_t seed = (p.drop_thr ? *p.seed_ptr : 0ull) + p.seed_offset;
  const uint32_t key = p.drop_thr ? rng_key(seed) : 0u;
  const bool idx32 = (uint64_t)p.M * (uint64_t)p.N + 8 <= 0xFFFFFFFFull;
  DpRowScale dps{};
  if constexpr (EPI == EPI_BF16_DP) dps.init(p, mb);
  float csum[2][8];
#pragma unroll
  for (int jp = 0; jp < 2; ++jp)
#pragma unroll
    for (int e = 0; e < 8; ++e) csum[jp][e] = 0.f;
  constexpr bool HAS_IN = (epi_bf16(EPI) && RES) || EPI == EPI_DGELU;
  constexpr int RING = 4;
  constexpr bool QOK = SCALED && (EPI == EPI_GELU || EPI == EPI_DGELU);
  const bool qon = QOK && p.q_out != nullptr;
  const __amdgpu_buffer_rsrc_t qrs = make_rsrc(qon ? p.q_out + (int64_t)mb * p.ld_q : p.q_out,
                                               qon && rows ? (uint32_t)((int64_t)(rows - 1) * p.ld_q + p.N) : 0u);
  const float qsc = qon ? *p.q_scale : 1.f;
  float qam = 0.f;
  v4u xring[HAS_IN ? RING : 1][2];
  if constexpr (HAS_IN) {
#pragma unroll
    for (int i = 0; i < RING; ++i)
#pragma unroll
      for (int jp = 0; jp < 2; ++jp)
        xring[i][jp] = __builtin_amdgcn_raw_buffer_load_b128(xrs, vx[jp] + (uint32_t)(i * 16 * (int)ldx * 2), 0, 0);
  }
#pragma unroll
  for (int i = 0; i < 8; ++i) {
    if (i == 1) stamp(p, 4);
    const uint32_t so_c = (uint32_t)(i * 16 * (int)p.ldc * 2), so_x = (uint32_t)(i * 16 * (int)ldx * 2);
    const int m = mb + 16 * i + li;
    float rf = 1.f;
    if constexpr (EPI == EPI_BF16_DP) rf = dps.factor(p, m);
#pragma unroll
    for (int jp = 0; jp < 2; ++jp) {
      v4u xin = {0u, 0u, 0u, 0u};
      if constexpr (HAS_IN) {
        xin = xring[i % RING][jp];
        if (i + RING < 8)
          xring[i % RING][jp] = __builtin_amdgcn_raw_buffer_load_b128(xrs, vx[jp] + (uint32_t)((i + RING) * 16 * (int)ldx * 2), 0, 0);
      }
      float v[8];
#pragma unroll
      for (int r = 0; r < 4; ++r) {
        float a = acc[i][2 * jp][r], b = acc[i][2 * jp + 1][r];
        asm volatile("s_nop 1\n\tv_permlane16_swap_b32 %0, %1" : "+v"(a), "+v"(b));
        v[r] = SCALED ? a * deq : a;
        v[4 + r] = SCALED ? b * deq : b;
      }
      bool keep[8] = {true, true, true, true, true, true, true, true};
      if constexpr (epi_bf16(EPI) || EPI == EPI_GELU) {
#pragma unroll
        for (int e = 0; e < 8; ++e) v[e] += bias[jp][e];
        if (p.drop_thr) {
          const uint64_t idx = (uint64_t)m * p.N + c0[jp];
          if (idx32) {
            bool k0[4], k1[4];
            rng_keep4_32(key, (uint32_t)idx, p.drop_thr, k0);
            rng_keep4_32(key, (uint32_t)idx + 4, p.drop_thr, k1);
#pragma unroll
            for (int e = 0; e < 4; ++e) { keep[e] = k0[e]; keep[4 + e] = k1[e]; }
          } else {
#pragma unroll
            for (int e = 0; e < 8; e += 2) rng_keep2(seed, idx + e, p.drop_thr, keep[e], keep[e + 1]);
          }
        }
      }
      v4u out;
      if constexpr (epi_bf16(EPI)) {
        if constexpr (EPI == EPI_BF16_DP) {
          const bool rk = rf != 0.f;
          const float zero = rk ? 0.f : -0.f;
#pragma unroll
          for (int e = 0; e < 8; ++e) v[e] = keep[e] && rk ? v[e] * rf : zero;
        } else if (p.drop_thr) {
#pragma unroll
          for (int e = 0; e < 8; ++e) v[e] = keep[e] ? v[e] * p.drop_scale : 0.f;
        }
        if constexpr (RES) {
#pragma unroll
          for (int q = 0; q < 4; ++q) {
            v[2 * q] += bf2f(xin[q] & 0xFFFF);
            v[2 * q + 1] += bf2f(xin[q] >> 16);
          }
        }
#pragma unroll
        for (int q = 0; q < 4; ++q) out[q] = pack2bf(v[2 * q], v[2 * q + 1]);
      } else if constexpr (EPI == EPI_GELU) {
        v4u ax;
#pragma unroll
        for (int q = 0; q < 4; ++q) {
          const v2f s2 = {keep[2 * q] ? p.drop_scale : 0.f, keep[2 * q + 1] ? p.drop_scale : 0.f};
          v2f g2, d2;
          gelu_and_grad2((v2f){v[2 * q], v[2 * q + 1]}, g2, d2);
          g2 *= s2;
          d2 *= s2;
          ax[q] = pack2bf(d2.x, d2.y);
          v[2 * q] = g2.x;
          v[2 * q + 1] = g2.y;
        }
        if (!p.c_skip) {
#pragma unroll
          for (int q = 0; q < 4; ++q) out[q] = pack2bf(v[2 * q], v[2 * q + 1]);
        } else {
          out = v4u{0u, 0u, 0u, 0u};
        }
        __builtin_amdgcn_raw_buffer_store_b128(ax, xrs, vx[jp] + so_x, 0, 0);
      } else {
#pragma unroll
        for (int q = 0; q < 4; ++q) {
          v[2 * q] *= bf2f(xin[q] & 0xFFFF);
          v[2 * q + 1] *= bf2f(xin[q] >> 16);
        }
#pragma unroll
        for (int e = 0; e < 8; ++e) csum[jp][e] += v[e];
        if (!p.c_skip) {
#pragma unroll
          for (int q = 0; q < 4; ++q) out[q] = pack2bf(v[2 * q], v[2 * q + 1]);
        } else {
          out = v4u{0u, 0u, 0u, 0u};
        }
      }
      __builtin_amdgcn_raw_buffer_store_b128(out, crs, vc[jp] + so_c, 0, 0);
      if constexpr (QOK) {
        if (qon) {
          const uint32_t vq = c0[jp] < p.N ? (uint32_t)((int64_t)(16 * i + li) * p.ld_q + c0[jp]) : OOB;
          float vm = 0.f;
#pragma unroll
          for (int e = 0; e < 8; ++e) vm = nan_max(vm, fabsf(v[e]));
          qam = nan_max(qam, vm);
          const uint2 q8 = p.q_fmt ? pack8_fp8_fast<1>(v, qsc, vm) : pack8_fp8_fast<0>(v, qsc, vm);
          __builtin_amdgcn_raw_buffer_store_b64((v2u_q){q8.x, q8.y}, qrs, vq, 0, 0);
        }
      }
    }
  }
  stamp(p, 5);
  if constexpr (EPI == EPI_DGELU) {
    {
#pragma unroll
      for (int jp = 0; jp < 2; ++jp)
#pragma unroll
        for (int e = 0; e < 8; ++e) csum[jp][e] = row16_sum(csum[jp][e]);
      float* red = (float*)smem;
      if (li == 0) {
#pragma unroll
        for (int e = 0; e < 8; ++e) {
          const float give = wm == 0 ? csum[1][e] : csum[0][e];
          red[(1 - wm) * 128 + wn * 32 + (c0[1 - wm] - nb - 32 * (1 - wm)) + e] = give;
        }
      }
      asm volatile("s_waitcnt lgkmcnt(0)" ::: "memory");
      __builtin_amdgcn_s_barrier();
      asm volatile("" ::: "memory");
      const __amdgpu_buffer_rsrc_t srs = make_rsrc(p.colsum, p.colsum ? (uint32_t)p.N * 4 : 0);
      if (li == 0) {
        const int jp = wm;
        const uint32_t vo = c0[jp] < p.N ? (uint32_t)c0[jp] * 4 : OOB;
#pragma unroll
        for (int e = 0; e < 8; ++e) {
          const float mine = wm == 0 ? csum[0][e] : csum[1][e];
          __builtin_amdgcn_raw_ptr_buffer_atomic_fadd_f32(mine + red[jp * 128 + wn * 32 + (c0[jp] - nb - 32 * jp) + e], srs, vo + 4 * e, 0, 0);
        }
      }
    }
  }
  if constexpr (QOK) {
    if (qon) {
      qam = wave_max_nan(qam);
      float* qred = (float*)(smem + 2048);
      const int w = (int)(threadIdx.x >> 6);
      if (lane == 0) qred[w] = qam;
      asm volatile("s_waitcnt lgkmcnt(0)" ::: "memory");
      __builtin_amdgcn_s_barrier();
      asm volatile("" ::: "memory");
      if (threadIdx.x == 0) {
        float b = qred[0];
#pragma unroll
        for (int k = 1; k < 8; ++k) b = nan_max(b, qred[k]);
        if (!(b <= 0.f)) atomicMax(p.q_amax, __float_as_uint(b));
      }
    }
  }
}

constexpr int CPOL_SC1 = 16;

template <int EPI, int RP = 128, bool RES = false>
PVR_DEV void epilogue_staged(const GemmParams& p, v4f (&acc)[8][4], char* smem, int m0, int n0, int wm, int wn, int lane) {
  static_assert(RP == 128 || RP == 64 || RP == 32, "rows per pass");
  const int tid = threadIdx.x;
  const int g = lane >> 4, li = lane & 15;
  const int cq = tid & 63;
  const int n = n0 + 4 * cq;
  const bool ncol = n < p.N;
  float4 bias = make_float4(0.f, 0.f, 0.f, 0.f);
  if constexpr (epi_bf16(EPI) || EPI == EPI_GELU) {
    if (p.bias && ncol) bias = *(const float4*)(p.bias + n);
  }
  const uint64_t seed = (p.drop_thr ? *p.seed_ptr : 0ull) + p.seed_offset;
  const uint32_t key = p.drop_thr ? rng_key(seed) : 0u;
  const bool idx32 = (uint64_t)p.M * (uint64_t)p.N + 4 <= 0xFFFFFFFFull;
  const float deq = p.scale_a ? (*p.scale_a) * (*p.scale_b) : 1.f;
  DpRowScale dps{};
  if constexpr (EPI == EPI_BF16_DP) dps.init(p, m0);
  float csum[4] = {0.f, 0.f, 0.f, 0.f};
  constexpr int NPASS = 256 / RP, FPP = RP / 16;
#pragma unroll
  for (int half = 0; half < NPASS; ++half) {
    if constexpr (EPI == EPI_F32_ATOMIC) {
      __syncthreads();
      if (wm == (half * RP) / 128) {
        const int i0 = ((half * RP) % 128) / 16;
#pragma unroll
        for (int ii = 0; ii < FPP; ++ii)
#pragma unroll
          for (int j = 0; j < 4; ++j) {
            const int r = 16 * ii + li;
            const int ch = wn * 16 + 4 * j + g;
            *(v4f*)(smem + r * 1024 + ((ch ^ (r & 63)) << 4)) = acc[i0 + ii][j];
          }
      }
      __syncthreads();
      const int c = tid & 255;
      const bool okc = n0 + c < p.N;
#pragma unroll 8
      for (int k = 0; k < RP / 2; ++k) {
        const int r = (tid >> 8) + 2 * k;
        const int m = m0 + half * RP + r;
        const float a = *(const float*)(smem + r * 1024 + (((c >> 2) ^ (r & 63)) << 4) + 4 * (c & 3));
        if (okc && m < p.M) atomicAdd((float*)p.C + (int64_t)m * p.ldc + n0 + c, a * deq);
      }
      continue;
    }
    __syncthreads();
    if (wm == (half * RP) / 128) {
      const int i0 = ((half * RP) % 128) / 16;
#pragma unroll
      for (int ii = 0; ii < FPP; ++ii)
#pragma unroll
        for (int j = 0; j < 4; ++j) {
          const int r = 16 * ii + li;
          const int ch = wn * 16 + 4 * j + g;
          *(v4f*)(smem + r * 1024 + ((ch ^ (r & 63)) << 4)) = acc[i0 + ii][j];
        }
    }
    __syncthreads();
    constexpr int RPT = RP / 8;
    constexpr bool HAS_IN = EPI == EPI_DGELU || (epi_bf16(EPI) && RES);
    const int mrow0 = m0 + half * RP + (tid >> 6);
    const int nn = ncol ? n : 0;
    const bool rows_in = m0 + half * RP + RP <= p.M;
    uint2 pin[HAS_IN ? RPT : 1];
    if constexpr (HAS_IN) {
      const uint16_t* src = EPI == EPI_DGELU ? p.aux : p.resid;
      const int64_t lsrc = EPI == EPI_DGELU ? p.ld_aux : p.ld_resid;
      const uint16_t* s0 = src + (int64_t)mrow0 * lsrc + nn;
      if (rows_in) {
#pragma unroll
        for (int k = 0; k < RPT; ++k) pin[k] = *(const uint2*)(s0 + (int64_t)k * (8 * lsrc));
      } else {
#pragma unroll
        for (int k = 0; k < RPT; ++k) pin[k] = *(const uint2*)(src + (int64_t)min(mrow0 + 8 * k, p.M - 1) * lsrc + nn);
      }
    }
    const uint64_t idx0 = (uint64_t)mrow0 * p.N + n, idx_step = 8ull * p.N;
    uint16_t* c0 = (uint16_t*)p.C + (int64_t)mrow0 * p.ldc + n;
    uint16_t* x0 = EPI == EPI_GELU && p.aux ? p.aux + (int64_t)mrow0 * p.ld_aux + n : nullptr;
#pragma unroll
    for (int k = 0; k < RPT; ++k) {
      const int r = (tid >> 6) + 8 * k;
      const int m = mrow0 + 8 * k;
      const v4f a = *(const v4f*)(smem + r * 1024 + ((cq ^ (r & 63)) << 4));
      const bool ok = m < p.M && ncol;
      float v[4] = {a[0] * deq, a[1] * deq, a[2] * deq, a[3] * deq};
      if constexpr (epi_bf16(EPI) || EPI == EPI_GELU) {
        v[0] += bias.x; v[1] += bias.y; v[2] += bias.z; v[3] += bias.w;
        bool keep[4] = {true, true, true, true};
        if (p.drop_thr) {
          const uint64_t idx = idx0 + (uint64_t)k * idx_step;
          if (EPI == EPI_GELU && idx32) {
            rng_keep4_32(key, (uint32_t)idx, p.drop_thr, keep);
          } else {
            rng_keep2(seed, idx, p.drop_thr, keep[0], keep[1]);
            rng_keep2(seed, idx + 2, p.drop_thr, keep[2], keep[3]);
          }
        }
        if constexpr (epi_bf16(EPI)) {
          if constexpr (EPI == EPI_BF16_DP) {
            const float rf = dps.factor(p, m);
            const bool rk = rf != 0.f;
            const float zero = rk ? 0.f : -0.f;
#pragma unroll
            for (int q = 0; q < 4; ++q) v[q] = keep[q] && rk ? v[q] * rf : zero;
          } else if (p.drop_thr) {
#pragma unroll
            for (int q = 0; q < 4; ++q) v[q] = keep[q] ? v[q] * p.drop_scale : 0.f;
          }
          if constexpr (RES) {
            const uint2 rr = pin[k];
            v[0] += bf2f(rr.x & 0xFFFF); v[1] += bf2f(rr.x >> 16);
            v[2] += bf2f(rr.y & 0xFFFF); v[3] += bf2f(rr.y >> 16);
          }
        } else {
          const v2f s01 = {keep[0] ? p.drop_scale : 0.f, keep[1] ? p.drop_scale : 0.f};
          const v2f s23 = {keep[2] ? p.drop_scale : 0.f, keep[3] ? p.drop_scale : 0.f};
          v2f g01, d01, g23, d23;
          gelu_and_grad2((v2f){v[0], v[1]}, g01, d01);
          gelu_and_grad2((v2f){v[2], v[3]}, g23, d23);
          g01 *= s01; g23 *= s23; d01 *= s01; d23 *= s23;
          v[0] = g01.x; v[1] = g01.y; v[2] = g23.x; v[3] = g23.y;
          uint2 ax; ax.x = pack2bf(d01.x, d01.y); ax.y = pack2bf(d23.x, d23.y);
          if (ok && p.aux) *(uint2*)(x0 + (int64_t)k * (8 * p.ld_aux)) = ax;
        }
      } else if constexpr (EPI == EPI_DGELU) {
        const uint2 gg = pin[k];
        v[0] *= bf2f(gg.x & 0xFFFF); v[1] *= bf2f(gg.x >> 16);
        v[2] *= bf2f(gg.y & 0xFFFF); v[3] *= bf2f(gg.y >> 16);
        if (ok) {
          csum[0] += v[0]; csum[1] += v[1]; csum[2] += v[2]; csum[3] += v[3];
        }
      }
      if constexpr (EPI == EPI_F32_STORE) {
        if (p.sk_out) {
          typedef uint32_t v4u_t __attribute__((ext_vector_type(4)));
          const __amdgpu_buffer_rsrc_t srs = make_rsrc((float*)p.C + (int64_t)blockIdx.z * p.split_stride, (uint32_t)(p.split_stride * 4));
          if (ok)
            __builtin_amdgcn_raw_buffer_store_b128(__builtin_bit_cast(v4u_t, make_float4(v[0], v[1], v[2], v[3])), srs,
                                                   (uint32_t)(((int64_t)m * p.ldc + n) * 4), 0, CPOL_SC1);
        } else if (ok) {
          *(float4*)((float*)p.C + (int64_t)blockIdx.z * p.split_stride + (int64_t)m * p.ldc + n) = make_float4(v[0], v[1], v[2], v[3]);
        }
      } else {
        uint2 o; o.x = pack2bf(v[0], v[1]); o.y = pack2bf(v[2], v[3]);
        if (ok) *(uint2*)(c0 + (int64_t)k * (8 * p.ldc)) = o;
      }
    }
  }
  if constexpr (EPI == EPI_DGELU) {
    if (p.colsum) {
      __syncthreads();
      float* red = (float*)smem;
      *(float4*)(red + (tid >> 6) * 256 + 4 * cq) = make_float4(csum[0], csum[1], csum[2], csum[3]);
      __syncthreads();
      if (tid < 256 && n0 + tid < p.N) {
        float t = 0.f;
#pragma unroll
        for (int w = 0; w < 8; ++w) t += red[w * 256 + tid];
        atomicAdd(p.colsum + n0 + tid, t);
      }
    }
  }
}


template <int S>
PVR_DEV void tail_sum(v4f (&acc)[8][4], __amdgpu_buffer_rsrc_t rs, int tid) {
  constexpr int SLAB_BYTES = 256 * 256 * 4;
#pragma unroll
  for (int i = 0; i < 8; ++i)
#pragma unroll
    for (int j = 0; j < 4; ++j) {
      const uint32_t off = (uint32_t)(((i * 4 + j) * 512 + tid) * 16);
      v4f s = __builtin_bit_cast(v4f, __builtin_amdgcn_raw_buffer_load_b128(rs, off, 0, CPOL_SC1));
#pragma unroll
      for (int q = 1; q < S; ++q)
        s += __builtin_bit_cast(v4f, __builtin_amdgcn_raw_buffer_load_b128(rs, off, q * SLAB_BYTES, CPOL_SC1));
      acc[i][j] = s;
    }
}

PVR_DEV bool tail_gather(const GemmParams& p, v4f (&acc)[8][4], char* smem, int tloc, int tpart) {
  typedef uint32_t v4u_t __attribute__((ext_vector_type(4)));
  constexpr int SLAB = 256 * 256;
  const int tid = threadIdx.x;
  const int S = p.tail_split;
  float* base = p.tail_ws + (int64_t)tloc * S * SLAB;
  const __amdgpu_buffer_rsrc_t rs = make_rsrc(base, (uint32_t)S * SLAB * 4);
#pragma unroll
  for (int i = 0; i < 8; ++i)
#pragma unroll
    for (int j = 0; j < 4; ++j)
      __builtin_amdgcn_raw_buffer_store_b128(__builtin_bit_cast(v4u_t, acc[i][j]), rs, (uint32_t)(((i * 4 + j) * 512 + tid) * 16),
                                             tpart * SLAB * 4, CPOL_SC1);
  asm volatile("s_waitcnt vmcnt(0)" ::: "memory");
  __syncthreads();
  unsigned* flag = (unsigned*)smem;
  if (tid == 0) {
    const unsigned old = __hip_atomic_fetch_add(p.tail_cnt + tloc, 1u, __ATOMIC_RELAXED, __HIP_MEMORY_SCOPE_AGENT);
    const unsigned last = old == (unsigned)(S - 1) ? 1u : 0u;
    if (last) __hip_atomic_store(p.tail_cnt + tloc, 0u, __ATOMIC_RELAXED, __HIP_MEMORY_SCOPE_AGENT);
    *(volatile unsigned*)flag = last;
  }
  __syncthreads();
  const unsigned last = *(volatile unsigned*)flag;
  if (!last) return false;
  switch (S) {
    case 2: tail_sum<2>(acc, rs, tid); break;
    case 3: tail_sum<3>(acc, rs, tid); break;
    default: tail_sum<4>(acc, rs, tid); break;
  }
  __syncthreads();
  return true;
}

template <int RPT, int U>
PVR_DEV void splitk_rows(const GemmParams& p, __amdgpu_buffer_rsrc_t wrs, int S, int rb, int nrow, int n0, int tid) {
  const int n = n0 + 4 * (tid & 63);
  const uint32_t far = (uint32_t)(p.split_stride * 4 * S);
  uint32_t off[RPT];
  v4f a[RPT];
#pragma unroll
  for (int i = 0; i < RPT; ++i) {
    const int r = (tid >> 6) + 8 * i, m = rb + r;
    off[i] = r < nrow && m < p.M && n < p.N ? (uint32_t)(((int64_t)m * p.ldc + n) * 4) : far;
    a[i] = v4f{0.f, 0.f, 0.f, 0.f};
  }
  for (int q0 = 0; q0 < S; q0 += U) {
    v4f l[U][RPT];
#pragma unroll
    for (int u = 0; u < U; ++u)
#pragma unroll
      for (int i = 0; i < RPT; ++i)
        l[u][i] = __builtin_bit_cast(v4f, __builtin_amdgcn_raw_buffer_load_b128(wrs, off[i], (uint32_t)((q0 + u) * p.split_stride * 4), CPOL_SC1));
#pragma unroll
    for (int u = 0; u < U; ++u)
#pragma unroll
      for (int i = 0; i < RPT; ++i) a[i] += l[u][i];
  }
#pragma unroll
  for (int i = 0; i < RPT; ++i) {
    if (off[i] == far) continue;
    const int m = rb + (tid >> 6) + 8 * i;
    float4* dst = (float4*)(p.sk_out + (int64_t)m * p.sk_ldo + n);
    const v4f prev = p.sk_acc ? __builtin_bit_cast(v4f, *dst) : v4f{0.f, 0.f, 0.f, 0.f};
    *dst = __builtin_bit_cast(float4, prev + a[i]);
  }
}

PVR_DEV void splitk_fixup(const GemmParams& p, char* smem, int tile, int m0, int n0) {
  typedef uint32_t v4u_t __attribute__((ext_vector_type(4)));
  const int S = gridDim.z, z = blockIdx.z, tid = threadIdx.x;
  unsigned* arrive = p.sk_cnt + 2 * tile;
  unsigned* done = arrive + 1;
  asm volatile("s_waitcnt vmcnt(0)" ::: "memory");
  __syncthreads();
  if (tid == 0) {
    __hip_atomic_fetch_add(arrive, 1u, __ATOMIC_RELAXED, __HIP_MEMORY_SCOPE_AGENT);
    unsigned spins = 0;
    while (__hip_atomic_load(arrive, __ATOMIC_RELAXED, __HIP_MEMORY_SCOPE_AGENT) < (unsigned)S) {
      __builtin_amdgcn_s_sleep(4);
      if (++spins == (1u << 24)) {
        __hip_atomic_fetch_add(p.sk_cnt + 2 * p.sk_cnt_tiles, 1u, __ATOMIC_RELAXED, __HIP_MEMORY_SCOPE_AGENT);
        break;
      }
    }
  }
  __syncthreads();
  __builtin_amdgcn_fence(__ATOMIC_ACQUIRE, "wavefront");
  const __amdgpu_buffer_rsrc_t wrs = make_rsrc(p.C, (uint32_t)(p.split_stride * 4 * S));
  const int r0 = 256 * z / S, nrow = 256 * (z + 1) / S - r0;
  const int rpt = (nrow + 7) / 8;
  if (rpt <= 1) splitk_rows<1, 16>(p, wrs, S, m0 + r0, nrow, n0, tid);
  else if (rpt <= 2) splitk_rows<2, 8>(p, wrs, S, m0 + r0, nrow, n0, tid);
  else if (rpt <= 4) splitk_rows<4, 4>(p, wrs, S, m0 + r0, nrow, n0, tid);
  else if (rpt <= 8) splitk_rows<8, 2>(p, wrs, S, m0 + r0, nrow, n0, tid);
  else splitk_rows<16, 1>(p, wrs, S, m0 + r0, nrow, n0, tid);
  asm volatile("s_waitcnt vmcnt(0)" ::: "memory");
  __syncthreads();
  if (tid == 0) {
    const unsigned old = __hip_atomic_fetch_add(done, 1u, __ATOMIC_RELAXED, __HIP_MEMORY_SCOPE_AGENT);
    if (old == (unsigned)(S - 1)) {
      __hip_atomic_store(arrive, 0u, __ATOMIC_RELAXED, __HIP_MEMORY_SCOPE_AGENT);
      __hip_atomic_store(done, 0u, __ATOMIC_RELAXED, __HIP_MEMORY_SCOPE_AGENT);
    }
  }
  (void)smem;
}

template <bool AK, bool BKC, bool SWAP, int EPI, int ES = 2, int FA = 0, int FB = 0>
__global__ void __launch_bounds__(512, 2) gemm_pp_kernel(GemmParams p) {
  extern __shared__ __attribute__((aligned(16))) char smem[];
  const int lane = threadIdx.x & 63;
  const int wave = __builtin_amdgcn_readfirstlane(threadIdx.x >> 6);
  const int wm = wave >> 2, wn = wave & 3;

  const int ntm = (p.M + 255) / 256, ntn = (p.N + 255) / 256;
  constexpr int BKE = 128 / ES;
  PVR_ASSERT(blockDim.x == 512);
  PVR_ASSERT(ES == 2 || (p.K % 128 == 0 && p.scale_a && p.scale_b));
  int tt, kbeg, kend, tloc = 0, tpart = -1;
  const TailPlan tp{p.tail_from, p.tail_split};
  PVR_ASSERT((int)blockIdx.x < tail_grid(tp, ntm * ntn));
  const TailUnit tu = tail_unit_c(tp, ntm * ntn, (int)blockIdx.x);
  tt = tu.tile;
  if (tu.part >= 0) {
    tpart = tu.part;
    tloc = tt - p.tail_from;
    const int nkt = p.K / BKE;
    kbeg = tail_kbeg(tpart, p.tail_split, nkt) * BKE;
    kend = tail_kbeg(tpart + 1, p.tail_split, nkt) * BKE;
  } else {
    kbeg = blockIdx.z * p.k_split_len;
    kend = min(p.K, kbeg + p.k_split_len);
  }
  const int m0 = (tt / ntn) * 256, n0 = (tt % ntn) * 256;
  const int nk = (kend - kbeg + BKE - 1) / BKE;
  PVR_ASSERT(!(AK || BKC) || (p.K % BKE == 0 && kbeg % BKE == 0));

  const void* abase;
  uint32_t abytes;
  if constexpr (ES == 1 && !AK) {
    const uint8_t* a8 = (const uint8_t*)p.A;
    abase = a8 + (int64_t)kbeg * p.lda + m0;
    abytes = rsrc_bytes((int64_t)(kend - 1) * p.lda + p.M, (int64_t)kbeg * p.lda + m0) / 2;
  } else if constexpr (ES == 1) {
    const uint8_t* a8 = (const uint8_t*)p.A;
    abase = a8 + (int64_t)m0 * p.lda + kbeg;
    abytes = rsrc_bytes((int64_t)(p.M - 1) * p.lda + p.K, (int64_t)m0 * p.lda + kbeg) / 2;
  } else if constexpr (AK) {
    abase = p.A + (int64_t)m0 * p.lda + kbeg;
    abytes = rsrc_bytes((int64_t)(p.M - 1) * p.lda + p.K, (int64_t)m0 * p.lda + kbeg);
  } else {
    abase = p.A + (int64_t)kbeg * p.lda + m0;
    abytes = rsrc_bytes((int64_t)(kend - 1) * p.lda + p.M, (int64_t)kbeg * p.lda + m0);
  }
  const void* bbase;
  uint32_t bbytes;
  if constexpr (ES == 1 && !BKC) {
    const uint8_t* b8 = (const uint8_t*)p.B;
    bbase = b8 + (int64_t)kbeg * p.ldb + n0;
    bbytes = rsrc_bytes((int64_t)(kend - 1) * p.ldb + p.N, (int64_t)kbeg * p.ldb + n0) / 2;
  } else if constexpr (ES == 1) {
    const uint8_t* b8 = (const uint8_t*)p.B;
    bbase = b8 + (int64_t)n0 * p.ldb + kbeg;
    bbytes = rsrc_bytes((int64_t)(p.N - 1) * p.ldb + p.K, (int64_t)n0 * p.ldb + kbeg) / 2;
  } else if constexpr (BKC) {
    bbase = p.B + (int64_t)n0 * p.ldb + kbeg;
    bbytes = rsrc_bytes((int64_t)(p.N - 1) * p.ldb + p.K, (int64_t)n0 * p.ldb + kbeg);
  } else {
    bbase = p.B + (int64_t)kbeg * p.ldb + n0;
    bbytes = rsrc_bytes((int64_t)(kend - 1) * p.ldb + p.N, (int64_t)kbeg * p.ldb + n0);
  }
  const __amdgpu_buffer_rsrc_t ars = make_rsrc(abase, abytes);
  const __amdgpu_buffer_rsrc_t brs = make_rsrc(bbase, bbytes);
  const __amdgpu_buffer_rsrc_t nul = make_rsrc(abase, 0);

  v4f acc[8][4];
#pragma unroll
  for (int i = 0; i < 8; ++i)
#pragma unroll
    for (int j = 0; j < 4; ++j) acc[i][j] = v4f{0.f, 0.f, 0.f, 0.f};
  v8s af[4][2], bf[2][2][2];
  PpStamps pst;

  stamp(p, 0);
  pp_issue<0, AK, BKC, ES>(ars, brs, nul, smem, p.lda, p.ldb, 0, nk, wave, lane);
  pp_issue<1, AK, BKC, ES>(ars, brs, nul, smem, p.lda, p.ldb, 0, nk, wave, lane);
  pp_issue<2, AK, BKC, ES>(ars, brs, nul, smem, p.lda, p.ldb, 0, nk, wave, lane);
  pp_issue<3, AK, BKC, ES>(ars, brs, nul, smem, p.lda, p.ldb, 0, nk, wave, lane);
  pp_issue<0, AK, BKC, ES>(ars, brs, nul, smem, p.lda, p.ldb, 1, nk, wave, lane);
  pp_issue<1, AK, BKC, ES>(ars, brs, nul, smem, p.lda, p.ldb, 1, nk, wave, lane);
  asm volatile("s_waitcnt vmcnt(8)" ::: "memory");
  pp_barrier();
  if (wm == 1) pp_barrier();
  stamp(p, 1);
  pst.begin();
#ifdef PVR_GEMM_PHASE_STAMPS
  const uint64_t pst0 = pst.last;
#endif

  constexpr int PRE = (PVR_PP_PRE && AK && ES == 2) ? 1 : 0;
  v8s pre[4];
  if constexpr (PRE) {
#pragma unroll
    for (int ii = 0; ii < 4; ++ii) pre[ii] = read_frag<256, true>(smem, wm * 128 + 16 * ii, 0, lane);
  }
  for (int t = 0; t < nk; ++t) {
    const char* buf = smem + (t & 1) * PP_BUF;
    const char* nbuf = smem + ((t + 1) & 1) * PP_BUF;
    pp_phase<0, 0, 1, 1, 2, AK, BKC, SWAP, ES, FA, FB, PRE>(acc, af, bf, pre, buf, nbuf, ars, brs, nul, smem, p.lda, p.ldb, t + 1, nk, wave, lane, wm, wn, pst);
    pp_phase<0, 1, 0, 1, 3, AK, BKC, SWAP, ES, FA, FB>(acc, af, bf, pre, buf, nbuf, ars, brs, nul, smem, p.lda, p.ldb, t + 1, nk, wave, lane, wm, wn, pst);
    pp_phase<1, 1, 1, 0, 0, AK, BKC, SWAP, ES, FA, FB>(acc, af, bf, pre, buf, nbuf, ars, brs, nul, smem, p.lda, p.ldb, t + 2, nk, wave, lane, wm, wn, pst);
    pp_phase<1, 0, 0, 0, 1, AK, BKC, SWAP, ES, FA, FB, 2 * PRE>(acc, af, bf, pre, buf, nbuf, ars, brs, nul, smem, p.lda, p.ldb, t + 2, nk, wave, lane, wm, wn, pst);
  }
  asm volatile("s_waitcnt vmcnt(0)" ::: "memory");
  if (wm == 0) pp_barrier();
  stamp(p, 2);
#ifdef PVR_GEMM_PHASE_STAMPS
  pst.acc[7] = __builtin_amdgcn_s_memtime() - pst0;
  if (p.dbg && lane == 0) {
    const int64_t b = blockIdx.x + (int64_t)gridDim.x * blockIdx.z;
#pragma unroll
    for (int k = 0; k < 8; ++k) p.dbg[(b * 8 + wave) * 8 + k] = pst.acc[k];
  }
#endif
  if constexpr (epi_bf16(EPI) || EPI == EPI_GELU || EPI == EPI_DGELU) {
    if (tpart >= 0 && !tail_gather(p, acc, smem, tloc, tpart)) return;
  }
  if constexpr (SWAP && (EPI == EPI_F32_ATOMIC || EPI == EPI_F32_STORE)) {
    if ((p.N & 3) == 0 && !p.row_group)
      epilogue_staged<EPI, 128, false>(p, acc, smem, m0, n0, wm, wn, lane);
    else
      epilogue<8, 4, SWAP, EPI>(p, acc, m0 + wm * 128, n0 + wn * 64, lane);
    if constexpr (EPI == EPI_F32_STORE) {
      if (p.sk_out) splitk_fixup(p, smem, tt, m0, n0);
    }
  } else if constexpr (SWAP && (epi_bf16(EPI) || EPI == EPI_GELU || EPI == EPI_DGELU)) {
    if (!p.epi_staged && direct_ok(p)) {
      if (EPI == EPI_BF16_DP || (epi_bf16(EPI) && p.resid))
        epilogue_direct<EPI, epi_bf16(EPI), ES == 1>(p, acc, smem, m0 + wm * 128, n0 + wn * 64, wm, wn, lane);
      else
        epilogue_direct<EPI, false, ES == 1>(p, acc, smem, m0 + wm * 128, n0 + wn * 64, wm, wn, lane);
    } else if (EPI == EPI_BF16_DP || (!p.addend && !p.row_group && (p.N & 3) == 0)) {
      if (EPI == EPI_BF16_DP || (epi_bf16(EPI) && p.resid))
        epilogue_staged<EPI, 128, epi_bf16(EPI)>(p, acc, smem, m0, n0, wm, wn, lane);
      else
        epilogue_staged<EPI, 128, false>(p, acc, smem, m0, n0, wm, wn, lane);
    }
    else
      epilogue<8, 4, SWAP, EPI>(p, acc, m0 + wm * 128, n0 + wn * 64, lane);
  } else {
    epilogue<8, 4, SWAP, EPI>(p, acc, m0 + wm * 128, n0 + wn * 64, lane);
  }
  if (p.dbg) asm volatile("s_waitcnt vmcnt(0)" ::: "memory");
  stamp(p, 3);
}

int device_cus() {
  static int cache[64] = {0};
  int dev = 0;
  if (hipGetDevice(&dev) != hipSuccess || dev < 0 || dev >= 64) return 256;
  if (!cache[dev]) {
    hipDeviceProp_t prop;
    const int n = hipGetDeviceProperties(&prop, dev) == hipSuccess ? prop.multiProcessorCount : 0;
    cache[dev] = n > 0 ? n : 256;
  }
  return cache[dev];
}

void plan_tail(GemmParams& q, int ntiles, int bke) {
  q.tail_from = 0;
  q.tail_split = 0;
  if (!q.tail_ws || !q.tail_cnt) return;
  const TailPlan t = plan_tail_c(ntiles, q.K / bke, device_cus(), q.tail_ws_elems, q.tail_cnt_elems, q.tail_max_units,
                                    q.tail_min_kt > 0 ? q.tail_min_kt : 12);
  q.tail_from = t.from;
  q.tail_split = t.split;
}

template <bool AK, bool BKC, bool SWAP, int EPI, int ES = 2, int FA = 0, int FB = 0>
hipError_t launch_pp(const GemmParams& p, hipStream_t s) {
  constexpr int SMEM = 2 * PP_BUF;
  auto kern = gemm_pp_kernel<AK, BKC, SWAP, EPI, ES, FA, FB>;
  static bool attr_set = false;
  if (!attr_set) {
    hipError_t e = hipFuncSetAttribute((const void*)kern, hipFuncAttributeMaxDynamicSharedMemorySize, SMEM);
    if (e != hipSuccess) return e;
    attr_set = true;
  }
  const int ntm = (p.M + 255) / 256, ntn = (p.N + 255) / 256;
  const int nsplit = (p.K + p.k_split_len - 1) / p.k_split_len;
  GemmParams q = p;
  q.tail_from = q.tail_split = 0;
  int grid = ntm * ntn;
  if constexpr (AK && BKC && (epi_bf16(EPI) || EPI == EPI_GELU || EPI == EPI_DGELU)) {
    if (nsplit == 1) {
      plan_tail(q, ntm * ntn, 128 / ES);
      grid = tail_grid(TailPlan{q.tail_from, q.tail_split}, ntm * ntn);
    }
  }
  hipLaunchKernelGGL(kern, dim3(grid, 1, nsplit), dim3(512), SMEM, s, q);
  return hipGetLastError();
}

template <int ES = 2>
PVR_DEV void ppp_issue_kind(int kind, __amdgpu_buffer_rsrc_t ars, __amdgpu_buffer_rsrc_t brs, char* buf, int64_t lda, int64_t ldb,
                            int kb, int wave, int lane) {
#pragma unroll
  for (int x = 0; x < 2; ++x) {
    const int d = wave + 8 * x;
    if (kind == 0 || kind == 3) {
      const int hh = kind == 3;
      const int rowb = (2 * (d >> 3) + hh) * 64 + (d & 7) * 8;
      const int row = rowb + (lane >> 3);
      const int c = (lane & 7) ^ swz_k(row);
      dma16(ars, to_lds(buf + rowb * 128), (uint32_t)(row * lda * ES + kb + c * 16));
    } else {
      const int hh = kind == 2;
      const int rowb = (2 * (d >> 2) + hh) * 32 + (d & 3) * 8;
      const int row = rowb + (lane >> 3);
      const int c = (lane & 7) ^ swz_k(row);
      dma16(brs, to_lds(buf + 256 * 128 + rowb * 128), (uint32_t)(row * ldb * ES + kb + c * 16));
    }
  }
}

struct PppTile {
  int m0, n0;
  __amdgpu_buffer_rsrc_t ars, brs;
};

template <int ES = 2>
PVR_DEV PppTile ppp_tile(const GemmParams& p, int v, int ntiles, int ntn) {
  PppTile t;
  if (v >= ntiles) {
    t.m0 = t.n0 = 0;
    t.ars = make_rsrc(p.A, 0);
    t.brs = make_rsrc(p.B, 0);
    return t;
  }
  const int tt = xcd_remap(v, ntiles);
  t.m0 = (tt / ntn) * 256;
  t.n0 = (tt % ntn) * 256;
  if constexpr (ES == 1) {
    t.ars = make_rsrc((const uint8_t*)p.A + (int64_t)t.m0 * p.lda, rsrc_bytes((int64_t)(p.M - 1) * p.lda + p.K, (int64_t)t.m0 * p.lda) / 2);
    t.brs = make_rsrc((const uint8_t*)p.B + (int64_t)t.n0 * p.ldb, rsrc_bytes((int64_t)(p.N - 1) * p.ldb + p.K, (int64_t)t.n0 * p.ldb) / 2);
  } else {
    t.ars = make_rsrc(p.A + (int64_t)t.m0 * p.lda, rsrc_bytes((int64_t)(p.M - 1) * p.lda + p.K, (int64_t)t.m0 * p.lda));
    t.brs = make_rsrc(p.B + (int64_t)t.n0 * p.ldb, rsrc_bytes((int64_t)(p.N - 1) * p.ldb + p.K, (int64_t)t.n0 * p.ldb));
  }
  return t;
}

template <int QM, int QN, int RD_A, int RD_B, bool SWAP, int VM = 8, int ES = 2, int FA = 0, int FB = 0, int PR = 0>
PVR_DEV void ppp_phase(v4f (&acc)[8][4], v8s (&af)[4][2], v8s (&bf)[2][2][2], v8s (&pre)[4], const char* buf, char* smem,
                       const PppTile& cur, const PppTile& nxt, int G_issue, int kind, int tile_first_G, int nk, const GemmParams& p,
                       int wave, int lane, int wm, int wn) {
  static_assert(PR == 0 || ES == 2, "A0 read-ahead: bf16 only");
  if constexpr (RD_A) {
#pragma unroll
    for (int ii = 0; ii < 4; ++ii)
#pragma unroll
      for (int ks = 0; ks < 2; ++ks)
        af[ii][ks] = ES == 1 ? frag_fp8(buf, wm * 128 + QM * 64 + 16 * ii, ks, lane)
                     : (PR == 1 && ks == 0) ? pre[ii]
                                            : read_frag<256, true>(buf, wm * 128 + QM * 64 + 16 * ii, ks, lane);
  }
  if constexpr (PR == 2) {
    const char* nbuf = smem + (((buf - smem) / PP_BUF) ^ 1) * PP_BUF;
#pragma unroll
    for (int ii = 0; ii < 4; ++ii) pre[ii] = read_frag<256, true>(nbuf, wm * 128 + 16 * ii, 0, lane);
  }
  if constexpr (RD_B) {
#pragma unroll
    for (int jj = 0; jj < 2; ++jj)
#pragma unroll
      for (int ks = 0; ks < 2; ++ks)
        bf[QN][jj][ks] = ES == 1 ? frag_fp8(buf + 256 * 128, wn * 64 + QN * 32 + 16 * jj, ks, lane)
                                 : read_frag<256, true>(buf + 256 * 128, wn * 64 + QN * 32 + 16 * jj, ks, lane);
  }
  {
    const int rel = G_issue - tile_first_G;
    const bool same = rel < nk;
    const PppTile& t = same ? cur : nxt;
    const int kt = same ? rel : rel - nk;
    ppp_issue_kind<ES>(kind, t.ars, t.brs, smem + (G_issue & 1) * PP_BUF, p.lda, p.ldb, kt * 128, wave, lane);
  }
  asm volatile("s_waitcnt vmcnt(%0)" ::"n"(VM) : "memory");
  pp_barrier();
  asm volatile("s_waitcnt lgkmcnt(0)" ::: "memory");
  __builtin_amdgcn_s_setprio(1);
  if constexpr (ES == 1) {
#pragma unroll
    for (int ii = 0; ii < 4; ++ii)
#pragma unroll
      for (int jj = 0; jj < 2; ++jj) {
        v4f& c = acc[QM * 4 + ii][QN * 2 + jj];
        if constexpr (SWAP)
          c = mfma_fp8<FB, FA>(bf[QN][jj][0], bf[QN][jj][1], af[ii][0], af[ii][1], c);
        else
          c = mfma_fp8<FA, FB>(af[ii][0], af[ii][1], bf[QN][jj][0], bf[QN][jj][1], c);
      }
    __builtin_amdgcn_s_setprio(0);
    pp_barrier();
    return;
  }
#pragma unroll
  for (int ks = 0; ks < 2; ++ks)
#pragma unroll
    for (int ii = 0; ii < 4; ++ii)
#pragma unroll
      for (int jj = 0; jj < 2; ++jj) {
        v4f& c = acc[QM * 4 + ii][QN * 2 + jj];
        if constexpr (SWAP)
          c = mfma16(bf[QN][jj][ks], af[ii][ks], c);
        else
          c = mfma16(af[ii][ks], bf[QN][jj][ks], c);
      }
  __builtin_amdgcn_s_setprio(0);
  pp_barrier();
}

template <bool SWAP, int EPI, bool DIRECT, int ES = 2, int FA = 0, int FB = 0>
__global__ void __launch_bounds__(512, 2) gemm_ppp_kernel(GemmParams p) {
  static_assert(ES == 2 || DIRECT, "fp8 persistent GEMM: register-direct epilogue");
  constexpr int INFL = !DIRECT ? 0 : epi_bf16(EPI) ? 16 : EPI == EPI_GELU ? 32 : 24;
  extern __shared__ __attribute__((aligned(16))) char smem[];
  const int lane = threadIdx.x & 63;
  const int wave = __builtin_amdgcn_readfirstlane(threadIdx.x >> 6);
  const int wm = wave >> 2, wn = wave & 3;
  const int ntm = (p.M + 255) / 256, ntn = (p.N + 255) / 256, ntiles = ntm * ntn;
  const int nk = p.K / (128 / ES);
  int v = blockIdx.x;
  if (v >= ntiles) return;

  PppTile cur = ppp_tile<ES>(p, v, ntiles, ntn);
  PppTile nxt = ppp_tile<ES>(p, v + gridDim.x, ntiles, ntn);
  ppp_issue_kind<ES>(0, cur.ars, cur.brs, smem, p.lda, p.ldb, 0, wave, lane);
  ppp_issue_kind<ES>(1, cur.ars, cur.brs, smem, p.lda, p.ldb, 0, wave, lane);
  ppp_issue_kind<ES>(2, cur.ars, cur.brs, smem, p.lda, p.ldb, 0, wave, lane);
  ppp_issue_kind<ES>(3, cur.ars, cur.brs, smem, p.lda, p.ldb, 0, wave, lane);
  ppp_issue_kind<ES>(0, cur.ars, cur.brs, smem + PP_BUF, p.lda, p.ldb, 128, wave, lane);
  ppp_issue_kind<ES>(1, cur.ars, cur.brs, smem + PP_BUF, p.lda, p.ldb, 128, wave, lane);
  asm volatile("s_waitcnt vmcnt(8)" ::: "memory");
  pp_barrier();
  constexpr int PRE = (PVR_PP_PRE && ES == 2) ? 1 : 0;
  v8s pre[4];
  if constexpr (PRE) {
#pragma unroll
    for (int ii = 0; ii < 4; ++ii) pre[ii] = read_frag<256, true>(smem, wm * 128 + 16 * ii, 0, lane);
  }

  const bool dstamp = p.dbg != nullptr;
  const uint64_t ts0 = dstamp ? __builtin_amdgcn_s_memtime() : 0;
  uint64_t ts_loop = 0, ts_epi = 0, ts_a = 0;
  int ntile_done = 0;
  int G0 = 0;
  for (;;) {
    if (dstamp) ts_a = __builtin_amdgcn_s_memtime();
    v4f acc[8][4];
#pragma unroll
    for (int i = 0; i < 8; ++i)
#pragma unroll
      for (int j = 0; j < 4; ++j) acc[i][j] = v4f{0.f, 0.f, 0.f, 0.f};
    v8s af[4][2], bf[2][2][2];
    if (wm == 1) pp_barrier();
    int kt = 0;
    if constexpr (INFL > 0) {
      if (G0 > 0) {
        const char* buf = smem + (G0 & 1) * PP_BUF;
        ppp_phase<0, 0, 1, 1, SWAP, 8 + INFL, ES, FA, FB, PRE>(acc, af, bf, pre, buf, smem, cur, nxt, G0 + 1, 2, G0, nk, p, wave, lane, wm, wn);
        ppp_phase<0, 1, 0, 1, SWAP, 8 + INFL, ES, FA, FB>(acc, af, bf, pre, buf, smem, cur, nxt, G0 + 1, 3, G0, nk, p, wave, lane, wm, wn);
        ppp_phase<1, 1, 1, 0, SWAP, 8 + INFL, ES, FA, FB>(acc, af, bf, pre, buf, smem, cur, nxt, G0 + 2, 0, G0, nk, p, wave, lane, wm, wn);
        ppp_phase<1, 0, 0, 0, SWAP, 8 + INFL, ES, FA, FB, 2 * PRE>(acc, af, bf, pre, buf, smem, cur, nxt, G0 + 2, 1, G0, nk, p, wave, lane, wm, wn);
        kt = 1;
      }
    }
    for (; kt < nk; ++kt) {
      const int G = G0 + kt;
      const char* buf = smem + (G & 1) * PP_BUF;
      ppp_phase<0, 0, 1, 1, SWAP, 8, ES, FA, FB, PRE>(acc, af, bf, pre, buf, smem, cur, nxt, G + 1, 2, G0, nk, p, wave, lane, wm, wn);
      ppp_phase<0, 1, 0, 1, SWAP, 8, ES, FA, FB>(acc, af, bf, pre, buf, smem, cur, nxt, G + 1, 3, G0, nk, p, wave, lane, wm, wn);
      ppp_phase<1, 1, 1, 0, SWAP, 8, ES, FA, FB>(acc, af, bf, pre, buf, smem, cur, nxt, G + 2, 0, G0, nk, p, wave, lane, wm, wn);
      ppp_phase<1, 0, 0, 0, SWAP, 8, ES, FA, FB, 2 * PRE>(acc, af, bf, pre, buf, smem, cur, nxt, G + 2, 1, G0, nk, p, wave, lane, wm, wn);
    }
    if (wm == 0) pp_barrier();
    uint64_t ts_b = 0;
    if (dstamp) {
      ts_b = __builtin_amdgcn_s_memtime();
      ts_loop += ts_b - ts_a;
    }
    if constexpr (DIRECT) {
      if (EPI == EPI_BF16_DP || (epi_bf16(EPI) && p.resid))
        epilogue_direct<EPI, epi_bf16(EPI), ES == 1>(p, acc, smem + 2 * PP_BUF, cur.m0 + wm * 128, cur.n0 + wn * 64, wm, wn, lane);
      else
        epilogue_direct<EPI, false, ES == 1>(p, acc, smem + 2 * PP_BUF, cur.m0 + wm * 128, cur.n0 + wn * 64, wm, wn, lane);
    } else if constexpr (ES == 2) {
      if (EPI == EPI_BF16_DP || (epi_bf16(EPI) && p.resid))
        epilogue_staged<EPI, 32, epi_bf16(EPI)>(p, acc, smem + 2 * PP_BUF, cur.m0, cur.n0, wm, wn, lane);
      else
        epilogue_staged<EPI, 32, false>(p, acc, smem + 2 * PP_BUF, cur.m0, cur.n0, wm, wn, lane);
    }
    if (dstamp) {
      ts_epi += __builtin_amdgcn_s_memtime() - ts_b;
      ++ntile_done;
    }
    v += gridDim.x;
    if (v >= ntiles) break;
    G0 += nk;
    cur = nxt;
    nxt = ppp_tile<ES>(p, v + gridDim.x, ntiles, ntn);
    if constexpr (INFL == 0) {
      asm volatile("s_waitcnt vmcnt(0)" ::: "memory");
      __syncthreads();
    }
  }
  asm volatile("s_waitcnt vmcnt(0)" ::: "memory");
  if (dstamp && threadIdx.x == 0) {
    uint64_t* d = p.dbg + (int64_t)blockIdx.x * 8;
    d[0] = __builtin_amdgcn_s_memtime() - ts0;
    d[1] = ts_loop;
    d[2] = ts_epi;
    d[3] = (uint64_t)ntile_done;
  }
}

template <bool SWAP, int EPI, int ES = 2, int FA = 0, int FB = 0>
hipError_t launch_ppp(const GemmParams& p, hipStream_t s) {
  constexpr int SMEM = 2 * PP_BUF + 32 * 1024;
  auto kd = gemm_ppp_kernel<SWAP, EPI, true, ES, FA, FB>;
  auto ks = gemm_ppp_kernel<SWAP, EPI, ES == 1, ES, FA, FB>;
  static bool attr_set = false;
  if (!attr_set) {
    hipError_t e = hipFuncSetAttribute((const void*)kd, hipFuncAttributeMaxDynamicSharedMemorySize, SMEM);
    if (e == hipSuccess) e = hipFuncSetAttribute((const void*)ks, hipFuncAttributeMaxDynamicSharedMemorySize, SMEM);
    if (e != hipSuccess) return e;
    attr_set = true;
  }
  const bool direct = !p.epi_staged && direct_ok(p);
  if (ES == 1 && !direct) return hipErrorInvalidValue;
  auto kern = direct ? kd : ks;
  const int ntiles = ((p.M + 255) / 256) * ((p.N + 255) / 256);
  const int cus = device_cus();
  const int grid = ntiles < cus ? ntiles : cus;
  hipLaunchKernelGGL(kern, dim3(grid), dim3(512), SMEM, s, p);
  return hipGetLastError();
}

template <bool AK, bool BKC, bool SWAP, int EPI>
hipError_t launch_tile(const GemmParams& p, hipStream_t s) {
  switch (p.tile_cfg) {
    case 6: return launch_v3<256, 256, 2, 4, 4, 2, AK, BKC, SWAP, EPI>(p, s);
    case 13:
      if constexpr (AK && BKC && SWAP && (epi_bf16(EPI) || EPI == EPI_GELU || EPI == EPI_DGELU)) {
        if (p.K % PP_BK == 0 && p.K >= 2 * PP_BK && p.k_split_len >= p.K && !p.addend && !p.row_group && (p.N & 3) == 0)
          return launch_ppp<SWAP, EPI>(p, s);
      }
      [[fallthrough]];
    case 12:
      if constexpr (AK || !BKC) {
        if ((!AK || (p.K % PP_BK == 0 && p.k_split_len % PP_BK == 0)) && (AK || p.k_split_len % PP_BK == 0))
          return launch_pp<AK, BKC, SWAP, EPI>(p, s);
      }
      return launch_v3<256, 256, 2, 4, 4, 2, AK, BKC, SWAP, EPI>(p, s);
    default: return launch_cfg<128, 128, 2, 2, AK, BKC, SWAP, EPI>(p, s);
  }
}

}

}

extern "C" int pvr_gemm_tail_split(int M, int N, int K, int elem_bytes, int max_units) {
  pvr::GemmParams q{};
  q.K = K;
  q.tail_max_units = max_units;
  q.tail_ws = reinterpret_cast<float*>(16);
  q.tail_cnt = reinterpret_cast<unsigned*>(16);
  q.tail_ws_elems = (int64_t)pvr::device_cus() * 65536;
  q.tail_cnt_elems = pvr::device_cus();
  pvr::plan_tail(q, ((M + 255) / 256) * ((N + 255) / 256), elem_bytes == 1 ? 128 : 64);
  return q.tail_split;
}

static int g_fp8_persistent = 1;
extern "C" void pvr_set_fp8_persistent(int mode) { g_fp8_persistent = mode ? 1 : 0; }

extern "C" int pvr_gemm_ws_takes(const pvr::GemmParams* pp) { return pvr_gemm_ws_ok(pp, pvr::device_cus()); }

extern "C" hipError_t pvr_gemm(const pvr::GemmParams* pp, hipStream_t s) {
  using namespace pvr;
  const GemmParams& p = *pp;
  if (p.M <= 0 || p.N <= 0 || p.K <= 0) return hipSuccess;
  if (p.drop_row_mul && (p.drop_row_mul < 0 || p.tile_cfg != 0 || p.row_group || p.elem8)) return hipErrorInvalidValue;
  if (p.epi < EPI_BF16 || p.epi > EPI_F32_STORE) return hipErrorInvalidValue;
  if (p.dp_thr) {
    const bool tile_ok = p.tile_cfg == 0 || p.tile_cfg == 6 || p.tile_cfg == 12 || p.tile_cfg == 13;
    if (p.epi != EPI_BF16 || !p.resid || !p.seed_ptr || p.dp_rows < 1 || p.dp_thr > 65535u || p.elem8 || p.row_group || p.addend ||
        (p.N & 7) || !tile_ok || !p.a_kcontig || !p.b_kcontig || p.k_split_len < p.K)
      return hipErrorInvalidValue;
    return launch_tile<true, true, true, EPI_BF16_DP>(p, s);
  }
  if (p.tile_cfg == 15) {
    if (pvr_gemm_ws_ok(pp, device_cus())) return pvr_gemm_ws(pp, device_cus(), s);
    GemmParams q = p;
    q.tile_cfg = 13;
    return pvr_gemm(&q, s);
  }
  const bool ak = p.a_kcontig, bk = p.b_kcontig;
  if (p.elem8) {
    const int f = p.fmt_a * 2 + p.fmt_b;
    if ((p.N & 3) || !p.scale_a || !p.scale_b) return hipErrorInvalidValue;
    if (!ak && !bk) {
      if (p.epi != EPI_F32_STORE || p.tile_cfg != 14 || p.k_split_len % 128 != 0 || (f != 2 && f != 0) || (p.M & 15) ||
          (p.N & 15) || (p.lda & 15) || (p.ldb & 15))
        return hipErrorInvalidValue;
      if (f == 0) return launch_pp<false, false, true, EPI_F32_STORE, 1, 0, 0>(p, s);
      return launch_pp<false, false, true, EPI_F32_STORE, 1, 1, 0>(p, s);
    }
    if (!ak || !bk || p.K % 128 != 0) return hipErrorInvalidValue;
    if (p.epi == EPI_F32_STORE) {
      if (p.tile_cfg != 14 || p.k_split_len % 128 != 0 || (f != 2 && f != 0)) return hipErrorInvalidValue;
      if (f == 0) return launch_pp<true, true, true, EPI_F32_STORE, 1, 0, 0>(p, s);
      return launch_pp<true, true, true, EPI_F32_STORE, 1, 1, 0>(p, s);
    }
    if (p.k_split_len < p.K) return hipErrorInvalidValue;
    const int ntiles8 = ((p.M + 255) / 256) * ((p.N + 255) / 256);
    const bool pers = g_fp8_persistent > 0 && ntiles8 >= 4 * device_cus() && p.K >= 256 && p.K <= 2048 && !p.epi_staged &&
                      direct_ok(p) && !p.resid;
    switch (p.epi) {
      case EPI_BF16:
        if (pers && f == 0) return launch_ppp<true, EPI_BF16, 1, 0, 0>(p, s);
        if (pers && f == 2) return launch_ppp<true, EPI_BF16, 1, 1, 0>(p, s);
        if (f == 0) return launch_pp<true, true, true, EPI_BF16, 1, 0, 0>(p, s);
        if (f == 2) return launch_pp<true, true, true, EPI_BF16, 1, 1, 0>(p, s);
        break;
      case EPI_GELU:
        if (pers && f == 0) return launch_ppp<true, EPI_GELU, 1, 0, 0>(p, s);
        if (f == 0) return launch_pp<true, true, true, EPI_GELU, 1, 0, 0>(p, s);
        break;
      case EPI_DGELU:
        if (f == 0) return launch_pp<true, true, true, EPI_DGELU, 1, 0, 0>(p, s);
        if (f == 2) return launch_pp<true, true, true, EPI_DGELU, 1, 1, 0>(p, s);
        break;
    }
    return hipErrorInvalidValue;
  }
  switch (p.epi) {
    case EPI_BF16:
      if (ak && bk) return launch_tile<true, true, true, EPI_BF16>(p, s);
      if (ak && !bk) return launch_tile<true, false, true, EPI_BF16>(p, s);
      break;
    case EPI_GELU:
      if (ak && bk) return launch_tile<true, true, true, EPI_GELU>(p, s);
      break;
    case EPI_DGELU:
      if (ak && bk) return launch_tile<true, true, true, EPI_DGELU>(p, s);
      if (ak && !bk) return launch_tile<true, false, true, EPI_DGELU>(p, s);
      break;
    case EPI_F32_ATOMIC:
      if (p.tile_cfg == 14 && ak == bk && p.k_split_len % PP_BK == 0 && (!ak || p.K % PP_BK == 0))
        return ak ? launch_pp<true, true, true, EPI_F32_ATOMIC>(p, s) : launch_pp<false, false, true, EPI_F32_ATOMIC>(p, s);
      if (!ak && !bk) return launch_tile<false, false, false, EPI_F32_ATOMIC>(p, s);
      if (ak && bk) return launch_tile<true, true, false, EPI_F32_ATOMIC>(p, s);
      break;
    case EPI_F32_STORE:
      if (p.tile_cfg == 14 && ak == bk && p.k_split_len % PP_BK == 0 && (!ak || p.K % PP_BK == 0))
        return ak ? launch_pp<true, true, true, EPI_F32_STORE>(p, s) : launch_pp<false, false, true, EPI_F32_STORE>(p, s);
      if (p.split_stride) return hipErrorInvalidValue;
      if (!ak && !bk) return launch_tile<false, false, false, EPI_F32_STORE>(p, s);
      if (ak && bk) return launch_tile<true, true, false, EPI_F32_STORE>(p, s);
      break;
  }
  return hipErrorInvalidValue;
}
```

### pytorch_vit_paper_replication_amd/csrc/kernels.h

```cpp
#pragma once
#include <stdint.h>

#include <hip/hip_runtime_api.h>

#include "gemm_params.h"

namespace pvr {

struct AdamGroup {
  float lr, beta1, beta2, eps, weight_decay;
  float bc1, bc2_sqrt;
  int decoupled;
  float one_minus_beta1, one_minus_beta2;
};
constexpr int ADAM_GROUP_COLS = 10;
static_assert(sizeof(AdamGroup) == ADAM_GROUP_COLS * sizeof(float), "AdamGroup is one float32 [10] row of the group table");

struct AdamEma {
  float* buf = nullptr; const float* pair = nullptr; float decay = 0.f, one_minus_decay = 1.f;
};

constexpr int LAMB_ALWAYS_ADAPT = 2;
constexpr int LAMB_CHUNK = 4096;

struct DropSite {
  const uint64_t* seed = nullptr; uint64_t offset = 0; uint32_t thr = 0; float scale = 1.f;
};


struct Fp8Copy {
  uint8_t* out = nullptr; int64_t ld = 0; const float* scale = nullptr; unsigned* amax = nullptr; int fmt = 0;
};

struct MixRow {
  int partner;
  float lam;
  int bx0, by0, bx1, by1;
  int pad[2];
};
static_assert(sizeof(MixRow) == 32, "MixRow is one int32 [8] row of the plan tensor");

struct EraseRow {
  int x0, y0, x1, y1;
};
static_assert(sizeof(EraseRow) == 16, "EraseRow is one int32 [4] row of the erase table");

constexpr int ERASE_CONST = 0, ERASE_PIXEL = 1;
struct EraseArgs {
  const EraseRow* rows = nullptr; int mode = ERASE_CONST; float value[4] = {0.f, 0.f, 0.f, 0.f};
  const uint64_t* seed = nullptr; uint64_t offset = 0;
};

constexpr int COLOR_NONE = 0, COLOR_GRAY = 1, COLOR_SOLARIZE = 2, COLOR_BLUR = 3;
constexpr int COLOR_TAPS = 13;
constexpr float COLOR_SIGMA_MAX = 2.0f;
constexpr int COLOR_BLOCK_PX = 2048;
struct ColorRow {
  int op, order;
  float fb, fc, fs, sigma;
  float w[COLOR_TAPS];
  float pad;
};
static_assert(sizeof(ColorRow) == 80, "ColorRow is one 20-word row of the plan tensor");

struct LnBwdParams {
  const uint16_t* dy; int64_t dy_stride;
  const uint16_t* x; int64_t x_stride;
  const float* mean; const float* rstd; const float* w;
  const uint16_t* dres; int64_t dres_stride;
  int dres_every;
  uint16_t* dx; int64_t dx_stride;
  float* dw; float* db; float* dsum;
  uint16_t* dz; int64_t dz_stride; DropSite drop; int dz_nostore;
  DropSite dpath; int dp_rows;
  Fp8Copy q;
  int rows, D;
  float* part;
};

struct AttnBwdParams {
  const uint16_t* qkv; int64_t ld;
  const uint16_t* out; int64_t ld_o;
  const uint16_t* dout; int64_t ld_do;
  const float* lse;
  uint16_t* dqkv; int64_t ld_dq;
  float* dq_acc; int dq_rezero;
  float* dbias; float* bpart;
  float* ws;
  int B, N, H, D;
  float scale;
  DropSite drop;
  Fp8Copy q8;
  int q8_only;
};

}

extern "C" {

hipError_t pvr_gemm(const pvr::GemmParams* p, hipStream_t s);
int pvr_gemm_tail_split(int M, int N, int K, int elem_bytes, int max_units);
void pvr_set_fp8_persistent(int mode);
int pvr_gemm_ws_ok(const pvr::GemmParams* p, int cus);
hipError_t pvr_gemm_ws(const pvr::GemmParams* p, int cus, hipStream_t s);
int pvr_gemm_ws_takes(const pvr::GemmParams* p);

hipError_t pvr_layernorm_fwd(const uint16_t* x, int64_t x_stride, const float* w, const float* b, uint16_t* y, int64_t y_stride,
                             float* mean, float* rstd, int rows, int D, float eps, hipStream_t s);
void pvr_set_ln_fwd_q8_grid(int per_cu);
hipError_t pvr_layernorm_fwd_q8(const uint16_t* x, int64_t x_stride, const float* w, const float* b, uint16_t* y, int64_t y_stride,
                                pvr::Fp8Copy q, float* mean, float* rstd, int rows, int D, float eps, hipStream_t s);
int pvr_layernorm_bwd_blocks(int rows, int D);
hipError_t pvr_layernorm_bwd(const pvr::LnBwdParams* p, hipStream_t s);

hipError_t pvr_cast_f32_bf16(const float* in, uint16_t* out, int64_t n, hipStream_t s);
hipError_t pvr_splitk_reduce(const float* ws, int S, int64_t stride, float* out, int64_t n, int ocols, int wcols, int accumulate,
                             hipStream_t s);
hipError_t pvr_splitk_epilogue(const float* ws, int S, int64_t stride, int M, int N, const float* bias, const uint16_t* resid,
                               int64_t ld_resid, int gelu, uint16_t* out, int64_t ldc, hipStream_t s);
hipError_t pvr_pad_cols_bf16(const uint16_t* src, int rows, int cols, uint16_t* dst, int ld_dst, hipStream_t s);
hipError_t pvr_transpose_batched(const uint16_t* src, uint16_t* dst, const int64_t* meta, int nmat, int total_tiles, hipStream_t s);
int pvr_colsum_part_rows(int rows);
hipError_t pvr_colsum(const uint16_t* dy, int64_t ld, int rows, int N, float* db, uint16_t* dz, int64_t ld_dz, pvr::DropSite drop,
                      pvr::Fp8Copy q, float* part, int row_mul, pvr::DropSite dpath, int dp_rows, hipStream_t s);
hipError_t pvr_drop_path_scale(pvr::DropSite dpath, float* s_out, int B, hipStream_t s);
hipError_t pvr_rows_reduce(const float* part, int R, int C, int seg, float* d0, float* d1, float* d2, hipStream_t s);
hipError_t pvr_patch_keep(const uint64_t* seed, uint64_t offset, int B, int np, int n_keep, int* keep, int* inv, hipStream_t s);
hipError_t pvr_pos_gather(const float* pos, const int* keep, float* out, int B, int np, int n_keep, int D, hipStream_t s);
hipError_t pvr_im2col(const float* img, uint16_t* out, int B, int C, int H, int W, int P, int Kp, const pvr::MixRow* mix,
                      const int* keep, int n_keep, pvr::EraseArgs erase, hipStream_t s);
hipError_t pvr_im2col_u8(const uint8_t* img, int64_t sb, int64_t sc, int64_t sy, int64_t sx, const float* mean, const float* stdv,
                         const float* geom, uint16_t* out, int B, int C, int Hs, int Ws, int H, int W, int P, int Kp, int vec,
                         const pvr::MixRow* mix, const int* keep, int n_keep, pvr::EraseArgs erase, hipStream_t s);
hipError_t pvr_erase_noise(const uint64_t* seed, uint64_t offset, float* out, int64_t n, hipStream_t s);
hipError_t pvr_color_u8(const uint8_t* in, int64_t isb, int64_t isc, int64_t isy, int64_t isx, uint8_t* out, int64_t osb, int64_t osc,
                        int64_t osy, int64_t osx, const pvr::ColorRow* rows, uint32_t* sums, int B, int Hs, int Ws, int vec,
                        int any_blur, int any_sum, hipStream_t s);
hipError_t pvr_cls_rows(const float* cls, const float* pos, uint16_t* out, int B, int D, int64_t row_stride, pvr::DropSite drop,
                        hipStream_t s);
hipError_t pvr_patch_bwd(const uint16_t* dE, int B, int ntok, int D, float* ws, float* dpos, float* dcls, uint16_t* dconv,
                         float* dbias, pvr::DropSite drop, const int* inv, int n_keep, hipStream_t s);
int pvr_patch_bwd_groups(int B);
int64_t pvr_patch_bwd_ws_floats(int B, int ntok, int D);

hipError_t pvr_head_fwd(const uint16_t* tok, int64_t ld_tok, int B, int D, const float* gamma, const float* beta, float eps,
                        const float* W, const float* bias, int C, float* xhat, float* rstd, float* logits, hipStream_t s);
hipError_t pvr_head_bwd(const float* dl, const float* xhat, const float* rstd, const float* gamma, const float* beta, const float* W,
                        int B, int C, int D, int ntok, float* dW, float* db, float* dgamma, float* dbeta, float* dy, uint16_t* dtok,
                        float* part, hipStream_t s);
hipError_t pvr_scale_by(const float* x, const float* sc, float* y, int64_t n, hipStream_t s);
hipError_t pvr_mean(const float* x, int n, float* out, hipStream_t s);
hipError_t pvr_metrics_accum(float* sums, const float* loss, const int* correct, int B, hipStream_t s);
hipError_t pvr_rng_next(int64_t* rng, int64_t* seed, hipStream_t s);
hipError_t pvr_zero_f32(float* x, int64_t n, hipStream_t s);
hipError_t pvr_xent(const float* logits, int64_t ld, const int64_t* labels, int B, int C, float* loss_rows, float* dlogits,
                    int* correct, float grad_scale, hipStream_t s);
hipError_t pvr_xent_soft(const float* logits, int64_t ld, const int64_t* ya, const int64_t* yb, const float* lam, float eps, int B,
                         int C, float* loss_rows, float* dlogits, int* correct, float grad_scale, hipStream_t s);

int pvr_norm_partial_blocks();
hipError_t pvr_grad_norm(const float* g, int64_t n, float max_norm, float* workspace, float* out, hipStream_t s);
hipError_t pvr_adam(float* p, const float* g, float* m, float* v, uint16_t* shadow, int64_t n, const int64_t* seg_start,
                    const int* seg_group, int nseg, const pvr::AdamGroup* groups, const pvr::AdamGroup* host_groups, int ngroups,
                    const float* clip, int skip_nonfinite, pvr::AdamEma ema, hipStream_t s);
hipError_t pvr_scale_by_clip(float* g, int64_t n, const float* clip, hipStream_t s);
hipError_t pvr_adam_t(float* p, const float* g, float* m, float* v, uint16_t* shadow, uint16_t* shadow_t, const int64_t* tmeta,
                      int nmat, int ntiles, const int64_t* fmeta, int nflat, int64_t flat4, const pvr::AdamGroup* groups,
                      const pvr::AdamGroup* host_groups, int ngroups, const float* clip, int skip_nonfinite, pvr::AdamEma ema,
                      hipStream_t s);

hipError_t pvr_lamb_moments(const float* p, const float* g, float* m, float* v, int64_t n, const int64_t* chunks, int nchunks,
                            const int* seg_group, int nseg, float* partial, const pvr::AdamGroup* groups,
                            const pvr::AdamGroup* host_groups, int ngroups, const float* clip, int skip_nonfinite, hipStream_t s);
hipError_t pvr_lamb_ratio(const float* partial, int nchunks, const int64_t* seg_chunks, const int* seg_group, int nseg, float* trust,
                          const pvr::AdamGroup* groups, const pvr::AdamGroup* host_groups, int ngroups, const float* clip,
                          int skip_nonfinite, hipStream_t s);
hipError_t pvr_lamb_update(float* p, const float* m, const float* v, uint16_t* shadow, uint16_t* shadow_t, int64_t n,
                           const int64_t* seg_start, const int* seg_group, int nseg, const int64_t* tmeta, int nmat, int ntiles,
                           const int64_t* fmeta, int nflat, int64_t flat4, const float* trust, const pvr::AdamGroup* groups,
                           const pvr::AdamGroup* host_groups, int ngroups, const float* clip, int skip_nonfinite, pvr::AdamEma ema,
                           hipStream_t s);

hipError_t pvr_fp8_quant(const uint16_t* x, int64_t ldx, uint8_t* y, int64_t ldy, int64_t rows, int cols, const float* qscale,
                         unsigned* amax, int fmt, hipStream_t s);
hipError_t pvr_fp8_quant_multi(const int64_t* segs, int nseg, int64_t nchunks, const float* qscale, unsigned* amax, int fmt,
                               int amax_only, hipStream_t s);
hipError_t pvr_fp8_quant_t(const uint16_t* x, int64_t ldx, uint8_t* y, int64_t ldy, int T, int C, const float* qscale, int fmt,
                           hipStream_t s);
hipError_t pvr_fp8_transpose(const uint8_t* x, int64_t ldx, uint8_t* y, int64_t ldy, int T, int C, hipStream_t s);
hipError_t pvr_fp8_dequant(const uint8_t* x, float* y, int64_t n, const float* dscale, int fmt, hipStream_t s);
hipError_t pvr_fp8_scale_update(float* hist, int H, unsigned* amax, float* qscale, float* dscale, const float* fmax, int s0, int s1,
                                float margin_mul, hipStream_t s);

void pvr_set_attn_fwd_qg(int qg);
void pvr_set_attn_fwd_head_qf(int qf);
void pvr_set_attn_prep_xcd(int on);
void pvr_set_attn_dbg(void* p);
int pvr_attn_head_dim_supported(int dh);
hipError_t pvr_attn_fwd(const uint16_t* qkv, int64_t ld, uint16_t* out, int64_t ld_o, float* lse, int B, int N, int H, int D,
                        float scale, pvr::DropSite drop, pvr::Fp8Copy q8, int q8_only, hipStream_t s);
int pvr_attn_dbias_splits(int B, int NQ);
hipError_t pvr_attn_dbias_reduce(const float* part, float* ws, float* dbias, int B, int H, int NQ, int D, hipStream_t s);
int pvr_attn_bwd_waves(int N);
int pvr_attn_bwd_key_blocks(int N);
int pvr_attn_bwd_needs_dq_acc(int N, int dh, int dbias, int drop, int det);
int64_t pvr_attn_bwd_ws_floats(int B, int N, int H, int D, int dbias, int drop, int det);
int pvr_attn_bwd_q8_ok(int N, int drop);
int pvr_attn_bwd_uses_pipe(int B, int N, int H, int D, int64_t ld, int64_t ld_do, int64_t ld_o, int64_t ld_dq, int drop);
int pvr_attn_bwd_part_rows(int B, int N, int H, int D, int64_t ld, int64_t ld_do, int64_t ld_o, int64_t ld_dq, int drop);
hipError_t pvr_attn_bwd(const pvr::AttnBwdParams* p, hipStream_t s);
int pvr_attn_cls_ok(int N, int dh);
hipError_t pvr_attn_cls_fwd(const uint16_t* qkv, int64_t ld, uint16_t* out, int64_t ld_o, float* lse, int B, int N, int H, int D,
                            float scale, hipStream_t s);
hipError_t pvr_attn_cls_bwd(const uint16_t* qkv, int64_t ld, const uint16_t* o, int64_t ld_o, const uint16_t* dout, int64_t ld_do,
                            const float* lse, uint16_t* dqkv, int64_t ld_dq, float* dq0, int B, int N, int H, int D, float scale,
                            hipStream_t s);
hipError_t pvr_attn_cls_dbias(const float* dq0, const uint16_t* dout, int64_t ld_do, float* dbias, int B, int D, hipStream_t s);

}
```

Measured before the change: 7929 images/sec.

## Add lean GEMM template instantiations specialised on epilogue features

Adds compile-time 'lean' variants of the one-tile and persistent bf16 GEMM kernels. Bias, residual, dropout, aux, colsum and split-K tail presence are fixed as template bits, and debug stamps and runtime flag checks are dropped, so the epilogue carries fewer branches and live registers. A host-side chooser picks the lean variant when the parameters match one of the common ViT shapes, with an env switch to turn it off. It also adds a sched_barrier inside the tail-sum loop. The cost is more kernel instantiations and a second dispatch path that has to stay consistent with the general kernel.

New measurement: 8047 images/sec (median of 6 runs). 1.01x the previous value.

```diff
diff --git a/pytorch_vit_paper_replication_amd/_ext.py b/pytorch_vit_paper_replication_amd/_ext.py
--- a/pytorch_vit_paper_replication_amd/_ext.py
+++ b/pytorch_vit_paper_replication_amd/_ext.py
@@ -26,6 +26,11 @@
     return want
 
 
+def _apply_env_switches(mod) -> None:
+    if os.environ.get("PVR_GEMM_LEAN", "1") == "0":
+        mod.set_gemm_lean(False)
+
+
 def load():
     global _C, _ERR, _TRIED
     if _TRIED:
@@ -51,6 +56,7 @@
             from . import _C as mod
 
         _C = mod
+        _apply_env_switches(mod)
     except BaseException as e:
         _ERR = e
         if os.environ.get("PVR_AUTOBUILD", "0") == "1":
@@ -65,6 +71,7 @@
 
                 _C = mod2
                 _ERR = None
+                _apply_env_switches(mod2)
             except BaseException as e2:
                 _ERR = e2
     return _C
diff --git a/pytorch_vit_paper_replication_amd/csrc/bindings.cpp b/pytorch_vit_paper_replication_amd/csrc/bindings.cpp
--- a/pytorch_vit_paper_replication_amd/csrc/bindings.cpp
+++ b/pytorch_vit_paper_replication_amd/csrc/bindings.cpp
@@ -130,6 +130,7 @@
   p.tail_cnt_elems = (int)it->second.cnt.numel();
 }
 void set_gemm_tail(bool on) { g_gemm_tail = on; }
+void set_gemm_lean(bool on) { pvr_set_gemm_lean(on ? 1 : 0); }
 
 constexpr int g_sk_tiles = 4096;
 torch::Tensor& splitk_counters(const torch::Tensor& like) {
@@ -1412,6 +1413,10 @@
   m.def("set_deterministic", &set_deterministic, "deterministic reductions (partial rows + ordered sum) instead of float atomics");
   m.def("deterministic", &deterministic);
   m.def("set_gemm_tail", &set_gemm_tail, "split-K tail of the last dispatch round on (True, default) / off (A/B)");
+  m.def("set_gemm_lean", &set_gemm_lean,
+        "lean GEMM instantiations on (True, default; PVR_GEMM_LEAN=0 at import: off) / off: every launch takes the general kernel");
+  m.def("gemm_lean_last", [] { return (int64_t)pvr_gemm_lean_last(); },
+        "GemmLean bits (csrc/gemm_lean.h) of the kernel the most recent gemm launched; 0: a general kernel");
   m.def("gemm", &gemm,py::arg("A"), py::arg("a_kcontig"), py::arg("B"), py::arg("b_kcontig"), py::arg("C"),
         py::arg("M"), py::arg("N"), py::arg("K"), py::arg("epi"), py::arg("bias"), py::arg("resid"), py::arg("addend"),
         py::arg("addend_period"), py::arg("aux"), py::arg("row_group"), py::arg("row_stride_group"),
diff --git a/pytorch_vit_paper_replication_amd/csrc/gemm.hip b/pytorch_vit_paper_replication_amd/csrc/gemm.hip
--- a/pytorch_vit_paper_replication_amd/csrc/gemm.hip
+++ b/pytorch_vit_paper_replication_amd/csrc/gemm.hip
@@ -1,5 +1,6 @@
 #include "common.h"
 #include "kernels.h"
+#include "gemm_lean.h"
 #include <type_traits>
 
 namespace pvr {
@@ -892,33 +893,32 @@
   pst.type_mark(PT_, 2);
 }
 
-__host__ __device__ inline bool direct_ok(const GemmParams& p) {
-  const int64_t l1 = p.ldc > p.ld_resid ? p.ldc : p.ld_resid;
-  const int64_t ld = l1 > p.ld_aux ? l1 : p.ld_aux;
-  return !p.addend && !p.row_group && (p.N & 7) == 0 && (int64_t)p.M * ld * 2 < (1ll << 31);
-}
-
-template <int EPI, bool RES, bool SCALED = false>
+__host__ __device__ inline bool direct_ok(const GemmParams& p) { return direct_ok_c(p); }
+
+template <int EPI, bool RES, bool SCALED = false, int LN = 0>
 PVR_DEV void epilogue_direct(const GemmParams& p, v4f (&acc)[8][4], char* smem, int mb, int nb, int wm, int wn, int lane) {
   typedef uint32_t v4u __attribute__((ext_vector_type(4)));
   typedef uint32_t v2u_q __attribute__((ext_vector_type(2)));
+  constexpr bool LEAN = LN != 0;
+  static_assert(!LEAN || !SCALED, "lean instantiations: bf16 operands");
+  constexpr bool L_BIAS = (LN & LEAN_BIAS) != 0, L_DROP = (LN & LEAN_DROP) != 0;
   const int li = lane & 15, g = lane >> 4;
   const float deq = SCALED ? (*p.scale_a) * (*p.scale_b) : 1.f;
   const int rows = max(0, min(128, p.M - mb));
   const uint32_t OOB = 0x80000000u;
   const __amdgpu_buffer_rsrc_t crs =
-      make_rsrc((const uint16_t*)p.C + (int64_t)mb * p.ldc, rows && !p.c_skip ? (uint32_t)(((int64_t)(rows - 1) * p.ldc + p.N) * 2) : 0);
+      make_rsrc((const uint16_t*)p.C + (int64_t)mb * p.ldc, rows && (LEAN || !p.c_skip) ? (uint32_t)(((int64_t)(rows - 1) * p.ldc + p.N) * 2) : 0);
   __amdgpu_buffer_rsrc_t xrs = crs;
   int64_t ldx = p.ldc;
   if constexpr (epi_bf16(EPI) && RES) {
     xrs = make_rsrc(p.resid + (int64_t)mb * p.ld_resid, rows ? (uint32_t)(((int64_t)(rows - 1) * p.ld_resid + p.N) * 2) : 0);
     ldx = p.ld_resid;
   } else if constexpr (EPI == EPI_GELU || EPI == EPI_DGELU) {
-    const bool has = p.aux != nullptr;
+    const bool has = (LN & LEAN_AUX) ? true : p.aux != nullptr;
     xrs = make_rsrc(has ? p.aux + (int64_t)mb * p.ld_aux : p.aux, has && rows ? (uint32_t)(((int64_t)(rows - 1) * p.ld_aux + p.N) * 2) : 0);
     ldx = p.ld_aux;
   }
-  const __amdgpu_buffer_rsrc_t brs = make_rsrc(p.bias, p.bias ? (uint32_t)p.N * 4 : 0);
+  const __amdgpu_buffer_rsrc_t brs = make_rsrc(p.bias, (LEAN ? L_BIAS : p.bias != nullptr) ? (uint32_t)p.N * 4 : 0);
   int c0[2];
   uint32_t vc[2], vx[2];
   float bias[2][8];
@@ -930,7 +930,7 @@
     vx[jp] = okc ? (uint32_t)((li * ldx + c0[jp]) * 2) : OOB;
 #pragma unroll
     for (int e = 0; e < 8; ++e) bias[jp][e] = 0.f;
-    if constexpr (epi_bf16(EPI) || EPI == EPI_GELU) {
+    if constexpr ((epi_bf16(EPI) || EPI == EPI_GELU) && (!LEAN || (LN & LEAN_BIAS))) {
       const uint32_t vb = okc ? (uint32_t)(c0[jp] * 4) : OOB;
       const v4f b0 = __builtin_bit_cast(v4f, __builtin_amdgcn_raw_buffer_load_b128(brs, vb, 0, 0));
       const v4f b1 = __builtin_bit_cast(v4f, __builtin_amdgcn_raw_buffer_load_b128(brs, vb + 16, 0, 0));
@@ -938,9 +938,9 @@
       for (int e = 0; e < 4; ++e) { bias[jp][e] = b0[e]; bias[jp][4 + e] = b1[e]; }
     }
   }
-  const uint64_t seed = (p.drop_thr ? *p.seed_ptr : 0ull) + p.seed_offset;
-  const uint32_t key = p.drop_thr ? rng_key(seed) : 0u;
-  const bool idx32 = (uint64_t)p.M * (uint64_t)p.N + 8 <= 0xFFFFFFFFull;
+  const uint64_t seed = ((LEAN ? L_DROP : p.drop_thr != 0) ? *p.seed_ptr : 0ull) + p.seed_offset;
+  const uint32_t key = (LEAN ? L_DROP : p.drop_thr != 0) ? rng_key(seed) : 0u;
+  const bool idx32 = LEAN ? true : (uint64_t)p.M * (uint64_t)p.N + 8 <= 0xFFFFFFFFull;
   DpRowScale dps{};
   if constexpr (EPI == EPI_BF16_DP) dps.init(p, mb);
   float csum[2][8];
@@ -966,7 +966,7 @@
   }
 #pragma unroll
   for (int i = 0; i < 8; ++i) {
-    if (i == 1) stamp(p, 4);
+    if (!LEAN && i == 1) stamp(p, 4);
     const uint32_t so_c = (uint32_t)(i * 16 * (int)p.ldc * 2), so_x = (uint32_t)(i * 16 * (int)ldx * 2);
     const int m = mb + 16 * i + li;
     float rf = 1.f;
@@ -991,7 +991,7 @@
       if constexpr (epi_bf16(EPI) || EPI == EPI_GELU) {
 #pragma unroll
         for (int e = 0; e < 8; ++e) v[e] += bias[jp][e];
-        if (p.drop_thr) {
+        if (LEAN ? L_DROP : p.drop_thr != 0) {
           const uint64_t idx = (uint64_t)m * p.N + c0[jp];
           if (idx32) {
             bool k0[4], k1[4];
@@ -1012,7 +1012,7 @@
           const float zero = rk ? 0.f : -0.f;
 #pragma unroll
           for (int e = 0; e < 8; ++e) v[e] = keep[e] && rk ? v[e] * rf : zero;
-        } else if (p.drop_thr) {
+        } else if (LEAN ? L_DROP : p.drop_thr != 0) {
 #pragma unroll
           for (int e = 0; e < 8; ++e) v[e] = keep[e] ? v[e] * p.drop_scale : 0.f;
         }
@@ -1038,7 +1038,7 @@
           v[2 * q] = g2.x;
           v[2 * q + 1] = g2.y;
         }
-        if (!p.c_skip) {
+        if (LEAN || !p.c_skip) {
 #pragma unroll
           for (int q = 0; q < 4; ++q) out[q] = pack2bf(v[2 * q], v[2 * q + 1]);
         } else {
@@ -1051,9 +1051,18 @@
           v[2 * q] *= bf2f(xin[q] & 0xFFFF);
           v[2 * q + 1] *= bf2f(xin[q] >> 16);
         }
+        if constexpr (LEAN) {
+#pragma unroll
+          for (int q = 0; q < 4; ++q) {
+            v2f t = {v[2 * q], v[2 * q + 1]};
+            asm volatile("" : "+v"(t));
+            v[2 * q] = t.x;
+            v[2 * q + 1] = t.y;
+          }
+        }
 #pragma unroll
         for (int e = 0; e < 8; ++e) csum[jp][e] += v[e];
-        if (!p.c_skip) {
+        if (LEAN || !p.c_skip) {
 #pragma unroll
           for (int q = 0; q < 4; ++q) out[q] = pack2bf(v[2 * q], v[2 * q + 1]);
         } else {
@@ -1074,7 +1083,7 @@
       }
     }
   }
-  stamp(p, 5);
+  if constexpr (!LEAN) stamp(p, 5);
   if constexpr (EPI == EPI_DGELU) {
     {
 #pragma unroll
@@ -1092,7 +1101,8 @@
       asm volatile("s_waitcnt lgkmcnt(0)" ::: "memory");
       __builtin_amdgcn_s_barrier();
       asm volatile("" ::: "memory");
-      const __amdgpu_buffer_rsrc_t srs = make_rsrc(p.colsum, p.colsum ? (uint32_t)p.N * 4 : 0);
+      const bool has_cs = (LN & LEAN_COLSUM) ? true : p.colsum != nullptr;
+      const __amdgpu_buffer_rsrc_t srs = make_rsrc(p.colsum, has_cs ? (uint32_t)p.N * 4 : 0);
       if (li == 0) {
         const int jp = wm;
         const uint32_t vo = c0[jp] < p.N ? (uint32_t)c0[jp] * 4 : OOB;
@@ -1297,7 +1307,7 @@
 PVR_DEV void tail_sum(v4f (&acc)[8][4], __amdgpu_buffer_rsrc_t rs, int tid) {
   constexpr int SLAB_BYTES = 256 * 256 * 4;
 #pragma unroll
-  for (int i = 0; i < 8; ++i)
+  for (int i = 0; i < 8; ++i) {
 #pragma unroll
     for (int j = 0; j < 4; ++j) {
       const uint32_t off = (uint32_t)(((i * 4 + j) * 512 + tid) * 16);
@@ -1307,6 +1317,8 @@
         s += __builtin_bit_cast(v4f, __builtin_amdgcn_raw_buffer_load_b128(rs, off, q * SLAB_BYTES, CPOL_SC1));
       acc[i][j] = s;
     }
+    __builtin_amdgcn_sched_barrier(0);
+  }
 }
 
 PVR_DEV bool tail_gather(const GemmParams& p, v4f (&acc)[8][4], char* smem, int tloc, int tpart) {
@@ -1417,8 +1429,11 @@
   (void)smem;
 }
 
-template <bool AK, bool BKC, bool SWAP, int EPI, int ES = 2, int FA = 0, int FB = 0>
+template <bool AK, bool BKC, bool SWAP, int EPI, int ES = 2, int FA = 0, int FB = 0, int LN = 0>
 __global__ void __launch_bounds__(512, 2) gemm_pp_kernel(GemmParams p) {
+  constexpr bool LEAN = LN != 0;
+  constexpr bool TAIL = !LEAN || (LN & LEAN_TAIL) != 0;
+  static_assert(!LEAN || (ES == 2 && SWAP && AK && BKC && EPI == EPI_BF16), "lean list");
   extern __shared__ __attribute__((aligned(16))) char smem[];
   const int lane = threadIdx.x & 63;
   const int wave = __builtin_amdgcn_readfirstlane(threadIdx.x >> 6);
@@ -1429,17 +1444,23 @@
   PVR_ASSERT(blockDim.x == 512);
   PVR_ASSERT(ES == 2 || (p.K % 128 == 0 && p.scale_a && p.scale_b));
   int tt, kbeg, kend, tloc = 0, tpart = -1;
-  const TailPlan tp{p.tail_from, p.tail_split};
-  PVR_ASSERT((int)blockIdx.x < tail_grid(tp, ntm * ntn));
-  const TailUnit tu = tail_unit_c(tp, ntm * ntn, (int)blockIdx.x);
-  tt = tu.tile;
-  if (tu.part >= 0) {
-    tpart = tu.part;
-    tloc = tt - p.tail_from;
-    const int nkt = p.K / BKE;
-    kbeg = tail_kbeg(tpart, p.tail_split, nkt) * BKE;
-    kend = tail_kbeg(tpart + 1, p.tail_split, nkt) * BKE;
+  if constexpr (TAIL) {
+    const TailPlan tp{p.tail_from, p.tail_split};
+    PVR_ASSERT((int)blockIdx.x < tail_grid(tp, ntm * ntn));
+    const TailUnit tu = tail_unit_c(tp, ntm * ntn, (int)blockIdx.x);
+    tt = tu.tile;
+    if (tu.part >= 0) {
+      tpart = tu.part;
+      tloc = tt - p.tail_from;
+      const int nkt = p.K / BKE;
+      kbeg = tail_kbeg(tpart, p.tail_split, nkt) * BKE;
+      kend = tail_kbeg(tpart + 1, p.tail_split, nkt) * BKE;
+    } else {
+      kbeg = blockIdx.z * p.k_split_len;
+      kend = min(p.K, kbeg + p.k_split_len);
+    }
   } else {
+    tt = xcd_remap_c((int)blockIdx.x, ntm * ntn);
     kbeg = blockIdx.z * p.k_split_len;
     kend = min(p.K, kbeg + p.k_split_len);
   }
@@ -1493,7 +1514,7 @@
   v8s af[4][2], bf[2][2][2];
   PpStamps pst;
 
-  stamp(p, 0);
+  if constexpr (!LEAN) stamp(p, 0);
   pp_issue<0, AK, BKC, ES>(ars, brs, nul, smem, p.lda, p.ldb, 0, nk, wave, lane);
   pp_issue<1, AK, BKC, ES>(ars, brs, nul, smem, p.lda, p.ldb, 0, nk, wave, lane);
   pp_issue<2, AK, BKC, ES>(ars, brs, nul, smem, p.lda, p.ldb, 0, nk, wave, lane);
@@ -1503,7 +1524,7 @@
   asm volatile("s_waitcnt vmcnt(8)" ::: "memory");
   pp_barrier();
   if (wm == 1) pp_barrier();
-  stamp(p, 1);
+  if constexpr (!LEAN) stamp(p, 1);
   pst.begin();
 #ifdef PVR_GEMM_PHASE_STAMPS
   const uint64_t pst0 = pst.last;
@@ -1525,7 +1546,7 @@
   }
   asm volatile("s_waitcnt vmcnt(0)" ::: "memory");
   if (wm == 0) pp_barrier();
-  stamp(p, 2);
+  if constexpr (!LEAN) stamp(p, 2);
 #ifdef PVR_GEMM_PHASE_STAMPS
   pst.acc[7] = __builtin_amdgcn_s_memtime() - pst0;
   if (p.dbg && lane == 0) {
@@ -1534,10 +1555,12 @@
     for (int k = 0; k < 8; ++k) p.dbg[(b * 8 + wave) * 8 + k] = pst.acc[k];
   }
 #endif
-  if constexpr (epi_bf16(EPI) || EPI == EPI_GELU || EPI == EPI_DGELU) {
+  if constexpr (TAIL && (epi_bf16(EPI) || EPI == EPI_GELU || EPI == EPI_DGELU)) {
     if (tpart >= 0 && !tail_gather(p, acc, smem, tloc, tpart)) return;
   }
-  if constexpr (SWAP && (EPI == EPI_F32_ATOMIC || EPI == EPI_F32_STORE)) {
+  if constexpr (LEAN) {
+    epilogue_direct<EPI, (LN & LEAN_RES) != 0, false, LN>(p, acc, smem, m0 + wm * 128, n0 + wn * 64, wm, wn, lane);
+  } else if constexpr (SWAP && (EPI == EPI_F32_ATOMIC || EPI == EPI_F32_STORE)) {
     if ((p.N & 3) == 0 && !p.row_group)
       epilogue_staged<EPI, 128, false>(p, acc, smem, m0, n0, wm, wn, lane);
     else
@@ -1562,8 +1585,10 @@
   } else {
     epilogue<8, 4, SWAP, EPI>(p, acc, m0 + wm * 128, n0 + wn * 64, lane);
   }
-  if (p.dbg) asm volatile("s_waitcnt vmcnt(0)" ::: "memory");
-  stamp(p, 3);
+  if constexpr (!LEAN) {
+    if (p.dbg) asm volatile("s_waitcnt vmcnt(0)" ::: "memory");
+    stamp(p, 3);
+  }
 }
 
 int device_cus() {
@@ -1586,6 +1611,24 @@
                                     q.tail_min_kt > 0 ? q.tail_min_kt : 12);
   q.tail_from = t.from;
   q.tail_split = t.split;
+}
+
+bool g_gemm_lean = true;
+int g_lean_last = 0;
+
+template <bool AK, bool BKC, bool SWAP, int EPI, int ES, int FA, int FB, int LN>
+hipError_t launch_pp_as(const GemmParams& q, int grid, int nsplit, hipStream_t s) {
+  constexpr int SMEM = 2 * PP_BUF;
+  auto kern = gemm_pp_kernel<AK, BKC, SWAP, EPI, ES, FA, FB, LN>;
+  static bool attr_set = false;
+  if (!attr_set) {
+    hipError_t e = hipFuncSetAttribute((const void*)kern, hipFuncAttributeMaxDynamicSharedMemorySize, SMEM);
+    if (e != hipSuccess) return e;
+    attr_set = true;
+  }
+  g_lean_last = LN;
+  hipLaunchKernelGGL(kern, dim3(grid, 1, nsplit), dim3(512), SMEM, s, q);
+  return hipGetLastError();
 }
 
 template <bool AK, bool BKC, bool SWAP, int EPI, int ES = 2, int FA = 0, int FB = 0>
@@ -1607,6 +1650,14 @@
     if (nsplit == 1) {
       plan_tail(q, ntm * ntn, 128 / ES);
       grid = tail_grid(TailPlan{q.tail_from, q.tail_split}, ntm * ntn);
+    }
+  }
+  if constexpr (ES == 2 && SWAP && AK && BKC && EPI == EPI_BF16) {
+    constexpr int RBD = LEAN_ON | LEAN_BIAS | LEAN_RES | LEAN_DROP, T = LEAN_TAIL;
+    switch (g_gemm_lean ? lean_choose(q, LEAN_K_ONE_TILE, q.tail_split > 1) : 0) {
+      case RBD: return launch_pp_as<AK, BKC, SWAP, EPI, ES, FA, FB, RBD>(q, grid, nsplit, s);
+      case RBD | T: return launch_pp_as<AK, BKC, SWAP, EPI, ES, FA, FB, RBD | T>(q, grid, nsplit, s);
+      default: break;
     }
   }
   hipLaunchKernelGGL(kern, dim3(grid, 1, nsplit), dim3(512), SMEM, s, q);
@@ -1731,9 +1782,10 @@
   pp_barrier();
 }
 
-template <bool SWAP, int EPI, bool DIRECT, int ES = 2, int FA = 0, int FB = 0>
+template <bool SWAP, int EPI, bool DIRECT, int ES = 2, int FA = 0, int FB = 0, int LN = 0>
 __global__ void __launch_bounds__(512, 2) gemm_ppp_kernel(GemmParams p) {
   static_assert(ES == 2 || DIRECT, "fp8 persistent GEMM: register-direct epilogue");
+  static_assert(LN == 0 || (ES == 2 && DIRECT && SWAP), "lean list");
   constexpr int INFL = !DIRECT ? 0 : epi_bf16(EPI) ? 16 : EPI == EPI_GELU ? 32 : 24;
   extern __shared__ __attribute__((aligned(16))) char smem[];
   const int lane = threadIdx.x & 63;
@@ -1761,7 +1813,7 @@
     for (int ii = 0; ii < 4; ++ii) pre[ii] = read_frag<256, true>(smem, wm * 128 + 16 * ii, 0, lane);
   }
 
-  const bool dstamp = p.dbg != nullptr;
+  const bool dstamp = LN ? false : p.dbg != nullptr;
   const uint64_t ts0 = dstamp ? __builtin_amdgcn_s_memtime() : 0;
   uint64_t ts_loop = 0, ts_epi = 0, ts_a = 0;
   int ntile_done = 0;
@@ -1800,7 +1852,9 @@
       ts_b = __builtin_amdgcn_s_memtime();
       ts_loop += ts_b - ts_a;
     }
-    if constexpr (DIRECT) {
+    if constexpr (LN != 0) {
+      epilogue_direct<EPI, (LN & LEAN_RES) != 0, false, LN>(p, acc, smem + 2 * PP_BUF, cur.m0 + wm * 128, cur.n0 + wn * 64, wm, wn, lane);
+    } else if constexpr (DIRECT) {
       if (EPI == EPI_BF16_DP || (epi_bf16(EPI) && p.resid))
         epilogue_direct<EPI, epi_bf16(EPI), ES == 1>(p, acc, smem + 2 * PP_BUF, cur.m0 + wm * 128, cur.n0 + wn * 64, wm, wn, lane);
       else
@@ -1853,6 +1907,23 @@
   const int ntiles = ((p.M + 255) / 256) * ((p.N + 255) / 256);
   const int cus = device_cus();
   const int grid = ntiles < cus ? ntiles : cus;
+  if constexpr (ES == 2 && SWAP && (EPI == EPI_BF16 || EPI == EPI_GELU || EPI == EPI_DGELU)) {
+    constexpr int LN = EPI == EPI_BF16 ? (LEAN_ON | LEAN_BIAS)
+                       : EPI == EPI_GELU ? (LEAN_ON | LEAN_BIAS | LEAN_DROP | LEAN_AUX)
+                                         : (LEAN_ON | LEAN_AUX | LEAN_COLSUM);
+    if (g_gemm_lean && direct && lean_choose(p, LEAN_K_PERSISTENT, false) == LN) {
+      auto kl = gemm_ppp_kernel<SWAP, EPI, true, ES, FA, FB, LN>;
+      static bool lean_attr_set = false;
+      if (!lean_attr_set) {
+        hipError_t e = hipFuncSetAttribute((const void*)kl, hipFuncAttributeMaxDynamicSharedMemorySize, SMEM);
+        if (e != hipSuccess) return e;
+        lean_attr_set = true;
+      }
+      g_lean_last = LN;
+      hipLaunchKernelGGL(kl, dim3(grid), dim3(512), SMEM, s, p);
+      return hipGetLastError();
+    }
+  }
   hipLaunchKernelGGL(kern, dim3(grid), dim3(512), SMEM, s, p);
   return hipGetLastError();
 }
@@ -1898,9 +1969,13 @@
 
 extern "C" int pvr_gemm_ws_takes(const pvr::GemmParams* pp) { return pvr_gemm_ws_ok(pp, pvr::device_cus()); }
 
+extern "C" void pvr_set_gemm_lean(int on) { pvr::g_gemm_lean = on != 0; }
+extern "C" int pvr_gemm_lean_last() { return pvr::g_lean_last; }
+
 extern "C" hipError_t pvr_gemm(const pvr::GemmParams* pp, hipStream_t s) {
   using namespace pvr;
   const GemmParams& p = *pp;
+  g_lean_last = 0;
   if (p.M <= 0 || p.N <= 0 || p.K <= 0) return hipSuccess;
   if (p.drop_row_mul && (p.drop_row_mul < 0 || p.tile_cfg != 0 || p.row_group || p.elem8)) return hipErrorInvalidValue;
   if (p.epi < EPI_BF16 || p.epi > EPI_F32_STORE) return hipErrorInvalidValue;
diff --git a/pytorch_vit_paper_replication_amd/csrc/gemm_lean.h b/pytorch_vit_paper_replication_amd/csrc/gemm_lean.h
--- /dev/null
+++ b/pytorch_vit_paper_replication_amd/csrc/gemm_lean.h
@@ -0,0 +1,46 @@
+#pragma once
+#include "gemm_params.h"
+
+namespace pvr {
+
+enum GemmLean : int {
+  LEAN_ON = 1,
+  LEAN_BIAS = 2,
+  LEAN_DROP = 4,
+  LEAN_RES = 8,
+  LEAN_TAIL = 16,
+  LEAN_AUX = 32,
+  LEAN_COLSUM = 64,
+};
+
+enum GemmLeanKernel : int {
+  LEAN_K_ONE_TILE = 0,
+  LEAN_K_PERSISTENT = 1,
+};
+
+constexpr bool direct_ok_c(const GemmParams& p) {
+  const int64_t l1 = p.ldc > p.ld_resid ? p.ldc : p.ld_resid;
+  const int64_t ld = l1 > p.ld_aux ? l1 : p.ld_aux;
+  return !p.addend && !p.row_group && (p.N & 7) == 0 && (int64_t)p.M * ld * 2 < (1ll << 31);
+}
+
+constexpr int lean_choose(const GemmParams& p, int kernel, bool tail) {
+  if (p.dbg || p.elem8 || p.dp_thr || p.drop_row_mul) return 0;
+  if (!p.a_kcontig || !p.b_kcontig || p.epi_staged || p.c_skip || p.q_out || !direct_ok_c(p) || p.k_split_len < p.K) return 0;
+  const bool bias = p.bias != nullptr, res = p.resid != nullptr, aux = p.aux != nullptr, cs = p.colsum != nullptr;
+  const bool drop = p.drop_thr != 0;
+  if (drop && (!p.seed_ptr || (uint64_t)p.M * (uint64_t)p.N + 8 > 0xFFFFFFFFull)) return 0;
+  if (kernel == LEAN_K_ONE_TILE) {
+    if (p.epi != 0) return 0;
+    if (bias && res && drop) return LEAN_ON | LEAN_BIAS | LEAN_RES | LEAN_DROP | (tail ? LEAN_TAIL : 0);
+    return 0;
+  }
+  if (kernel == LEAN_K_PERSISTENT && !tail) {
+    if (p.epi == 0 && bias && !res && !drop) return LEAN_ON | LEAN_BIAS;
+    if (p.epi == 1 && bias && drop && aux) return LEAN_ON | LEAN_BIAS | LEAN_DROP | LEAN_AUX;
+    if (p.epi == 2 && aux && cs) return LEAN_ON | LEAN_AUX | LEAN_COLSUM;
+  }
+  return 0;
+}
+
+}
diff --git a/pytorch_vit_paper_replication_amd/csrc/kernels.h b/pytorch_vit_paper_replication_amd/csrc/kernels.h
--- a/pytorch_vit_paper_replication_amd/csrc/kernels.h
+++ b/pytorch_vit_paper_replication_amd/csrc/kernels.h
@@ -101,6 +101,8 @@
 hipError_t pvr_gemm(const pvr::GemmParams* p, hipStream_t s);
 int pvr_gemm_tail_split(int M, int N, int K, int elem_bytes, int max_units);
 void pvr_set_fp8_persistent(int mode);
+void pvr_set_gemm_lean(int on);
+int pvr_gemm_lean_last();
 int pvr_gemm_ws_ok(const pvr::GemmParams* p, int cus);
 hipError_t pvr_gemm_ws(const pvr::GemmParams* p, int cus, hipStream_t s);
 int pvr_gemm_ws_takes(const pvr::GemmParams* p);
```
